# excamera/alfalfa

Hardware: NVIDIA H100
Metric: decode_throughput (higher is better)
Workload: dtype u8

## Files before the change

alfalfa_b200/csrc/capi.cc:

```cpp
#include <cuda_runtime.h>
#include <stdio.h>
#include <stdlib.h>
#include <string.h>
#include <sys/resource.h>
#include <sys/syscall.h>
#include <unistd.h>

#include <algorithm>
#include <atomic>
#include <condition_variable>
#include <deque>
#include <memory>
#include <mutex>
#include <string>
#include <chrono>
#include <thread>
#include <unordered_map>
#include <vector>

#include "../../include/vp8gpu.h"
#include "engine.hpp"
#include "hostpool.h"
#include "parser.h"
#include "serializer.h"

using vp8::Engine;
using vp8::HostJob;
using vp8::ParsedFrame;
using vp8::State;

struct vp8gpu_parsed;
struct vp8gpu_ctx {
  Engine* engine = nullptr;
  std::string create_error;
  std::atomic<int> next_lane{0};
  std::mutex pool_mu;
  std::vector<vp8gpu_parsed*> pinned_pool;
  double stats[8] = {0, 0, 0, 0, 0, 0, 0, 0};
  std::atomic<int> device_tokens{1};
  std::mutex scratch_mu;
  vp8::TokenRing* scratch_ring = nullptr;
  std::vector<struct ivf_worker_kit*> kit_pool;
  std::mutex tok_mu;
  std::condition_variable tok_cv;
  int tok_permits = 0, tok_capacity = 0;
};
struct TokRelease {
  vp8gpu_ctx* ctx;
  int n;
};
static void CUDART_CB tok_release_cb(void* p) {
  TokRelease* r = static_cast<TokRelease*>(p);
  {
    std::lock_guard<std::mutex> lk(r->ctx->tok_mu);
    r->ctx->tok_permits += r->n;
  }
  r->ctx->tok_cv.notify_all();
  delete r;
}
struct vp8gpu_state {
  State s;
  vp8gpu_state(int w, int h) : s(w, h) {}
  explicit vp8gpu_state(const State& o) : s(o) {}
};
struct vp8gpu_parsed {
  ParsedFrame f;
  uint32_t n_intra = 0, n_filtered = 0;
  cudaEvent_t consumed = nullptr;
  bool busy = false;
  explicit vp8gpu_parsed(const vp8::Allocator& a) : f(a) {}
};
constexpr int kTokSlots = 96;
constexpr int kTokChunk = 32;
constexpr int kTokStreams = 4;
struct ivf_worker_kit {
  vp8::TokenRing* ring = nullptr;
  cudaStream_t copy_stream = nullptr;
  cudaStream_t kstream[kTokStreams] = {};
  int next_kstream = 0;
  vp8gpu_parsed* parsed[kTokSlots] = {};
  cudaEvent_t staged[kTokSlots] = {}, ready[kTokSlots] = {}, finished[kTokSlots] = {};
  bool busy[kTokSlots] = {};
};
struct vp8gpu_resident_batch {
  Engine::Resident* r = nullptr;
};

namespace {

constexpr unsigned kWaitableEvent = cudaEventDisableTiming | cudaEventBlockingSync;

void* pinned_alloc(size_t n) {
  void* p = nullptr;
  return cudaHostAlloc(&p, n, cudaHostAllocDefault) == cudaSuccess ? p : nullptr;
}
void pinned_free(void* p) { cudaFreeHost(p); }
const vp8::Allocator kPinned = {&pinned_alloc, &pinned_free};

size_t ring_bytes_for(size_t n) { return n + n / 4 + 4096; }

void count_mbs(vp8gpu_parsed* p) {
  const vp8gpu_frame_desc& d = p->f.desc;
  const size_t n = (size_t)d.mb_cols * d.mb_rows;
  const vp8gpu_mb* m = p->f.mbs.data();
  uint32_t ni = 0, nf = 0;
  for (size_t i = 0; i < n; i++) {
    ni += m[i].ref_frame == VP8GPU_REF_CURRENT;
    nf += m[i].lf_level != 0;
  }
  p->n_intra = ni;
  p->n_filtered = nf;
}

}

extern "C" {

Engine* vp8gpu_ctx_engine(vp8gpu_ctx* ctx) { return ctx->engine; }
int vp8gpu_ctx_next_lane(vp8gpu_ctx* ctx) { return ctx->next_lane.fetch_add(1) % vp8::kMaxLanes; }
const vp8::ParsedFrame* vp8gpu_parsed_frame(const vp8gpu_parsed* p) { return p ? &p->f : nullptr; }

int vp8gpu_ctx_create(int device, int width, int height, int max_frames, vp8gpu_ctx** out) {
  if (!out) return VP8GPU_ERR_LOGIC;
  *out = nullptr;
  setenv("CUDA_DEVICE_MAX_CONNECTIONS", "32", 0);
  vp8gpu_ctx* c = new vp8gpu_ctx();
  const int rc = Engine::create(device, width, height, max_frames, &c->engine, &c->create_error);
  if (rc != VP8GPU_OK) {
    delete c;
    return rc;
  }
  *out = c;
  return VP8GPU_OK;
}
extern "C" void vp8gpu_encoder_pool_purge(Engine* e);
void vp8gpu_ctx_destroy(vp8gpu_ctx* ctx) {
  if (!ctx) return;
  for (vp8gpu_parsed* p : ctx->pinned_pool) vp8gpu_parsed_destroy(p);
  ctx->engine->sync_all();
  if (ctx->scratch_ring) ctx->engine->token_ring_free(ctx->scratch_ring);
  for (ivf_worker_kit* k : ctx->kit_pool) {
    ctx->engine->token_ring_free(k->ring);
    if (k->copy_stream) cudaStreamDestroy(k->copy_stream);
    for (cudaStream_t st : k->kstream)
      if (st) cudaStreamDestroy(st);
    for (int i = 0; i < kTokSlots; i++) {
      if (k->parsed[i]) vp8gpu_parsed_destroy(k->parsed[i]);
      if (k->staged[i]) cudaEventDestroy(k->staged[i]);
      if (k->ready[i]) cudaEventDestroy(k->ready[i]);
    }
    delete k;
  }
  vp8gpu_encoder_pool_purge(ctx->engine);
  delete ctx->engine;
  delete ctx;
}
const char* vp8gpu_last_error(const vp8gpu_ctx* ctx) { return ctx && ctx->engine ? ctx->engine->last_error() : ""; }

int vp8gpu_frame_alloc(vp8gpu_ctx* ctx, vp8gpu_frame_id* out) { return ctx->engine->frame_alloc(out); }
int vp8gpu_frame_retain(vp8gpu_ctx* ctx, vp8gpu_frame_id id) { return ctx->engine->frame_retain(id); }
int vp8gpu_frame_release(vp8gpu_ctx* ctx, vp8gpu_frame_id id) { return ctx->engine->frame_release(id); }
int vp8gpu_frame_upload(vp8gpu_ctx* ctx, vp8gpu_frame_id id, const uint8_t* y, size_t ys, const uint8_t* u,
                        const uint8_t* v, size_t cs) {
  return ctx->engine->frame_upload(id, y, ys, u, v, cs);
}
int vp8gpu_frame_download(vp8gpu_ctx* ctx, vp8gpu_frame_id id, uint8_t* y, size_t ys, uint8_t* u, uint8_t* v,
                          size_t cs) {
  return ctx->engine->frame_download(id, y, ys, u, v, cs);
}
int vp8gpu_frame_download_display(vp8gpu_ctx* ctx, vp8gpu_frame_id id, uint8_t* dst, size_t dst_size) {
  return ctx->engine->frame_download_display(id, 0, dst, dst_size, true);
}
int vp8gpu_frame_download_display_async(vp8gpu_ctx* ctx, vp8gpu_frame_id id, uint8_t* dst, size_t dst_size) {
  return ctx->engine->frame_download_display(id, 0, dst, dst_size, false);
}
int vp8gpu_frame_hash(vp8gpu_ctx* ctx, vp8gpu_frame_id id, uint64_t* out) { return ctx->engine->frame_hash(id, 0, out); }
int vp8gpu_frame_ssim(vp8gpu_ctx* ctx, vp8gpu_frame_id a, vp8gpu_frame_id b, double* out) {
  if (!ctx || !out) return VP8GPU_ERR_LOGIC;
  return ctx->engine->frames_ssim(a, b, 0, out);
}
size_t vp8gpu_frame_bytes(const vp8gpu_ctx* ctx) { return ctx->engine->geom().frame_bytes; }
int vp8gpu_frame_export(vp8gpu_ctx* ctx, vp8gpu_frame_id id, void* dst, size_t bytes) {
  return ctx->engine->frame_copy_raw(id, dst, bytes, false);
}
int vp8gpu_frame_import(vp8gpu_ctx* ctx, vp8gpu_frame_id id, const void* src, size_t bytes) {
  return ctx->engine->frame_copy_raw(id, const_cast<void*>(src), bytes, true);
}
int vp8gpu_ctx_sync(vp8gpu_ctx* ctx) { return ctx->engine->sync_all(); }
int vp8gpu_host_alloc(void** out, size_t bytes) {
  return cudaHostAlloc(out, bytes, cudaHostAllocDefault) == cudaSuccess ? VP8GPU_OK : VP8GPU_ERR_NOMEM;
}
void vp8gpu_host_free(void* p) {
  if (p) cudaFreeHost(p);
}
uint64_t vp8gpu_launch_count(const vp8gpu_ctx* ctx) { return ctx->engine->launches(); }
int vp8gpu_frames_in_use(const vp8gpu_ctx* ctx) { return ctx->engine->frames_in_use(); }
int vp8gpu_serialize_frame_ex(const vp8gpu_encode_header* hdr, const vp8gpu_encode_features* ft, const vp8gpu_mb* mbs,
                              const vp8gpu_token* tokens, const vp8gpu_split_mvs* split, uint8_t* out, size_t cap,
                              size_t* size) {
  if (!hdr || !mbs || !size) return VP8GPU_ERR_LOGIC;
  vp8::EncodeHeader h;
  h.key_frame = hdr->key_frame;
  h.show_frame = hdr->show_frame;
  h.width = hdr->width;
  h.height = hdr->height;
  h.y_ac_qi = hdr->y_ac_qi;
  h.loop_filter_level = hdr->loop_filter_level;
  h.sharpness = hdr->sharpness;
  h.optimize_token_probs = hdr->optimize_token_probs;
  vp8::EncodeFeatures x;
  if (ft) {
    x.log2_partitions = ft->log2_partitions;
    x.segmentation_enabled = ft->segmentation_enabled;
    x.update_mb_segmentation_map = ft->update_mb_segmentation_map;
    x.update_segment_feature_data = ft->update_segment_feature_data;
    x.segment_feature_absolute = ft->segment_feature_absolute;
    for (int i = 0; i < 4; i++) {
      x.segment_quant[i] = ft->segment_quant[i];
      x.segment_lf[i] = ft->segment_lf[i];
      x.ref_lf_delta[i] = ft->ref_lf_delta[i];
      x.mode_lf_delta[i] = ft->mode_lf_delta[i];
    }
    for (int i = 0; i < 3; i++) x.segment_tree_probs[i] = ft->segment_tree_probs[i];
    x.lf_delta_enabled = ft->lf_delta_enabled;
    x.lf_delta_update = ft->lf_delta_update;
    x.y_dc_delta = ft->y_dc_delta;
    x.y2_dc_delta = ft->y2_dc_delta;
    x.y2_ac_delta = ft->y2_ac_delta;
    x.uv_dc_delta = ft->uv_dc_delta;
    x.uv_ac_delta = ft->uv_ac_delta;
    x.refresh_golden = ft->refresh_golden;
    x.refresh_alternate = ft->refresh_alternate;
    x.refresh_last = ft->refresh_last;
    x.refresh_entropy_probs = ft->refresh_entropy_probs;
    x.copy_to_golden = ft->copy_to_golden;
    x.copy_to_alternate = ft->copy_to_alternate;
    x.sign_bias_golden = ft->sign_bias_golden;
    x.sign_bias_alternate = ft->sign_bias_alternate;
    x.saved_coef_probs = ft->saved_coef_probs;
  }
  const std::vector<uint8_t> bytes = vp8::serialize_frame(h, mbs, tokens, split, ft ? &x : nullptr);
  if (bytes.empty()) return VP8GPU_ERR_UNSUPPORTED;
  *size = bytes.size();
  if (!out || cap < bytes.size()) return VP8GPU_ERR_NOMEM;
  memcpy(out, bytes.data(), bytes.size());
  return VP8GPU_OK;
}
int vp8gpu_serialize_frame(const vp8gpu_encode_header* hdr, const vp8gpu_mb* mbs, const vp8gpu_token* tokens,
                           const vp8gpu_split_mvs* split, uint8_t* out, size_t cap, size_t* size) {
  return vp8gpu_serialize_frame_ex(hdr, nullptr, mbs, tokens, split, out, cap, size);
}
void vp8gpu_decode_ivf_stats(const vp8gpu_ctx* ctx, double out[8]) { memcpy(out, ctx->stats, sizeof(ctx->stats)); }

static HostJob to_host_job(const vp8gpu_job& j) {
  HostJob h;
  h.desc = j.desc;
  h.mbs = j.mbs;
  h.tokens = j.tokens;
  h.split = j.split;
  memcpy(h.refs, j.refs, sizeof(h.refs));
  h.out = j.out;
  return h;
}

int vp8gpu_decode_batch(vp8gpu_ctx* ctx, int lane, const vp8gpu_job* jobs, int n) {
  if (!ctx || !jobs || n < 0) return VP8GPU_ERR_LOGIC;
  std::vector<HostJob> hj;
  hj.reserve(n);
  for (int i = 0; i < n; i++) {
    if (!jobs[i].desc || !jobs[i].mbs) return ctx->engine->fail(VP8GPU_ERR_LOGIC, "decode_batch: null records");
    if (jobs[i].desc->mb_cols != ctx->engine->geom().mb_cols || jobs[i].desc->mb_rows != ctx->engine->geom().mb_rows)
      return ctx->engine->fail(VP8GPU_ERR_LOGIC, "decode_batch: frame size does not match the context");
    hj.push_back(to_host_job(jobs[i]));
  }
  const int rc = ctx->engine->submit(lane, hj.data(), n, nullptr);
  if (rc != VP8GPU_OK) return rc;
  cudaError_t e = cudaStreamSynchronize(ctx->engine->stream(lane));
  return e == cudaSuccess ? VP8GPU_OK : ctx->engine->cuda_fail(e, "decode_batch sync");
}

int vp8gpu_decode_parsed(vp8gpu_ctx* ctx, int lane, const vp8gpu_frame_desc* desc, const vp8gpu_mb* mbs,
                         const vp8gpu_token* tokens, const vp8gpu_split_mvs* split, const vp8gpu_frame_id refs[3],
                         vp8gpu_frame_id out) {
  vp8gpu_job j;
  j.desc = desc;
  j.mbs = mbs;
  j.tokens = tokens;
  j.split = split;
  for (int i = 0; i < 3; i++) j.refs[i] = refs ? refs[i] : -1;
  j.out = out;
  return vp8gpu_decode_batch(ctx, lane, &j, 1);
}

int vp8gpu_batch_upload(vp8gpu_ctx* ctx, const vp8gpu_job* jobs, int n, vp8gpu_resident_batch** out) {
  std::vector<HostJob> hj;
  for (int i = 0; i < n; i++) hj.push_back(to_host_job(jobs[i]));
  vp8gpu_resident_batch* b = new vp8gpu_resident_batch();
  const int rc = ctx->engine->resident_upload(hj.data(), n, &b->r);
  if (rc != VP8GPU_OK) {
    delete b;
    return rc;
  }
// ... 502 lines not shown
    j.n_intra = (int)ps[i]->n_intra;
    j.n_filtered = (int)ps[i]->n_filtered;
    j.consumed = ps[i]->consumed;
    jobs.push_back(j);
    which.push_back(i);
  }
  const int rc = e->submit(lane < 0 ? ds[0]->lane : lane, jobs.data(), (int)jobs.size(), nullptr);
  for (size_t k = 0; k < jobs.size(); k++) {
    const int i = which[k];
    if (rc == VP8GPU_OK) {
      ps[i]->busy = true;
      copy_to_references(ds[i], *jobs[k].desc, jobs[k].out);
    } else {
      rcs[i] = rc;
    }
    e->frame_release(jobs[k].out);
  }
  for (int i = 0; i < n; i++)
    if (rcs[i] != VP8GPU_OK) return rcs[i];
  return VP8GPU_OK;
}

int vp8gpu_decoder_decode_parsed(vp8gpu_decoder* d, const vp8gpu_parsed* parsed, int* shown, vp8gpu_frame_id* out) {
  if (!d || !parsed) return VP8GPU_ERR_LOGIC;
  cudaSetDevice(d->ctx->engine->device());
  return decode_parsed_impl(d, const_cast<vp8gpu_parsed*>(parsed), false, shown, out);
}

vp8gpu_state* vp8gpu_decoder_state(vp8gpu_decoder* d) { return &d->state; }
int vp8gpu_decoder_references(const vp8gpu_decoder* d, vp8gpu_frame_id refs[3]) {
  memcpy(refs, d->refs, sizeof(d->refs));
  return VP8GPU_OK;
}
int vp8gpu_decoder_lane(const vp8gpu_decoder* d) { return d->lane; }

int vp8gpu_decoder_hash(vp8gpu_decoder* d, uint64_t* out) {
  if (!d || !out) return VP8GPU_ERR_LOGIC;
  uint64_t h = d->state.s.hash();
  for (int i = 0; i < 3; i++) {
    uint64_t r = 0;
    const int rc = d->ctx->engine->frame_hash(d->refs[i], d->lane, &r);
    if (rc != VP8GPU_OK) return rc;
    h = (h ^ r) * 0x9E3779B97F4A7C15ull + (h >> 29) + i;
  }
  *out = h;
  return VP8GPU_OK;
}

int vp8gpu_decoder_equal(vp8gpu_decoder* a, vp8gpu_decoder* b, int* equal) {
  if (!a || !b || !equal || a->ctx != b->ctx) return VP8GPU_ERR_LOGIC;
  *equal = 0;
  if (!(a->state.s == b->state.s)) return VP8GPU_OK;
  for (int i = 0; i < 3; i++) {
    int eq = 0;
    const int rc = a->ctx->engine->frames_equal(a->refs[i], b->refs[i], a->lane, &eq);
    if (rc != VP8GPU_OK) return rc;
    if (!eq) return VP8GPU_OK;
  }
  *equal = 1;
  return VP8GPU_OK;
}

struct CachedFirstPartition {
  vp8gpu_frame_desc desc;
  std::vector<vp8gpu_mb> mbs;
  std::vector<vp8gpu_split_mvs> split;
  vp8::TokenWork tw;
  size_t bits_delta = 0;
};
std::mutex g_parse_cache_mu;
std::unordered_map<uint64_t, std::shared_ptr<CachedFirstPartition>> g_parse_cache;
uint64_t frame_key(const uint8_t* p, size_t n) {
  uint64_t h = 1469598103934665603ull ^ n;
  auto mix = [&](const uint8_t* q, size_t k) {
    for (size_t i = 0; i < k; i++) h = (h ^ q[i]) * 1099511628211ull;
  };
  mix(p, n < 64 ? n : 64);
  if (n > 64) mix(p + n - 64, 64);
  return h;
}
int parse_first_partition_cached(vp8::State& state, const uint8_t* data, size_t len, vp8::ParsedFrame& out) {
  const uint64_t key = frame_key(data, len);
  std::shared_ptr<CachedFirstPartition> c;
  {
    std::lock_guard<std::mutex> lk(g_parse_cache_mu);
    auto it = g_parse_cache.find(key);
    if (it != g_parse_cache.end()) c = it->second;
  }
  if (!c) {
    const int rc = vp8::parse_frame(state, data, len, out, true);
    if (rc != VP8GPU_OK) return rc;
    c = std::make_shared<CachedFirstPartition>();
    c->desc = out.desc;
    const size_t n = (size_t)out.desc.mb_cols * out.desc.mb_rows;
    c->mbs.assign(out.mbs.data(), out.mbs.data() + n);
    c->split.assign(out.split.data(), out.split.data() + out.desc.n_split);
    c->tw = out.tw;
    c->bits_delta = (size_t)(out.tw.bits - data);
    std::lock_guard<std::mutex> lk(g_parse_cache_mu);
    g_parse_cache[key] = c;
    return VP8GPU_OK;
  }
  out.desc = c->desc;
  if (!out.mbs.reserve(c->mbs.size(), 0) || !out.split.reserve(c->split.size() + 1, 0)) return VP8GPU_ERR_NOMEM;
  memcpy(out.mbs.data(), c->mbs.data(), c->mbs.size() * sizeof(vp8gpu_mb));
  if (!c->split.empty()) memcpy(out.split.data(), c->split.data(), c->split.size() * sizeof(vp8gpu_split_mvs));
  out.tw = c->tw;
  out.tw.bits = data + c->bits_delta;
  return VP8GPU_OK;
}

struct IvfKnobs {
  int tok_slots = -1;
  int tok_chunk = -1;
  int tok_inflight = -1;
  int tok_arena = -1;
  int dispatchers = -1;
  int worker_nice = -1;
  bool trace = false;
  bool parse_cache = false;
  static int num(const char* name) {
    const char* v = getenv(name);
    return v ? atoi(v) : -1;
  }
  IvfKnobs()
      : tok_slots(num("VP8GPU_TOK_SLOTS")), tok_chunk(num("VP8GPU_TOK_CHUNK")), tok_inflight(num("VP8GPU_TOK_INFLIGHT")),
        tok_arena(num("VP8GPU_TOK_ARENA")), dispatchers(num("VP8GPU_DISPATCHERS")), worker_nice(num("VP8GPU_WORKER_NICE")),
        trace(getenv("VP8GPU_TRACE") != nullptr), parse_cache(getenv("VP8GPU_PARSE_CACHE") != nullptr) {}
};

class IvfDecode {
 public:
  IvfDecode(vp8gpu_ctx* ctx_, const uint8_t* ivf_, size_t len_, int threads_, uint8_t* dst_, size_t dst_size_)
      : ctx(ctx_), e(ctx_->engine), ivf(ivf_), len(len_), threads(threads_), dst(dst_), dst_size(dst_size_) {}
  int parse_container();
  void plan();
  int run(uint32_t* n_decoded, uint32_t* n_shown);

 private:
  struct Item {
    const uint8_t* p;
    uint32_t n;
    int64_t out_off;
  };
  static constexpr int kSlots = 4;
  enum SlotState { kFree = 0, kQueued = 1 };
  struct Pending {
    vp8gpu_parsed* slot;
    int refs[3];
    int out;
    int64_t out_off;
    int* slot_state;
    int tid = 0;
    const vp8::TokenRing* ring = nullptr;
    int ring_slot = 0;
    cudaEvent_t ready = nullptr;
    cudaEvent_t* finished = nullptr;
  };

  vp8gpu_ctx* const ctx;
  Engine* const e;
  const IvfKnobs knobs;
  const uint8_t* const ivf;
  const size_t len;
  int threads;
  uint8_t* const dst;
  const size_t dst_size;
  int w = 0, h = 0;
  std::vector<Item> items;
  std::vector<uint32_t> gop_start;
  uint32_t shown_total = 0, max_frame_bytes = 0;
  int n_gops = 0;
  int tok_slots = 0, tok_chunk = 1, n_disp = 1, worker_nice = 5;
  size_t arena_tokens = 0;
  bool device_tokens = false;
  std::mutex mu;
  std::vector<std::condition_variable> cv_worker, cv_disp;
  std::vector<std::deque<Pending>> queues;
  std::vector<int> running;
  std::atomic<int> next_gop{0};
  std::atomic<int> first_error{VP8GPU_OK};
  std::mutex stats_mu;
  double st_parse = 0, st_wait_slot = 0, st_wait_dma = 0, st_submit = 0, st_download = 0, st_disp_idle = 0;
  double st_batches = 0, st_jobs = 0;

  void set_error(int rc) {
    int ok = VP8GPU_OK;
    first_error.compare_exchange_strong(ok, rc);
  }
  static double now() { return std::chrono::duration<double>(std::chrono::steady_clock::now().time_since_epoch()).count(); }
  static void advance_refs(Engine* e, int refs[3], const vp8gpu_frame_desc& desc, int out) {
    if (desc.key_frame) {
      set_ref(e, &refs[0], out);
      set_ref(e, &refs[1], out);
      set_ref(e, &refs[2], out);
    } else {
      if (desc.copy_to_alternate == 1) set_ref(e, &refs[2], refs[0]);
      else if (desc.copy_to_alternate == 2) set_ref(e, &refs[2], refs[1]);
      if (desc.copy_to_golden == 1) set_ref(e, &refs[1], refs[0]);
      else if (desc.copy_to_golden == 2) set_ref(e, &refs[1], refs[2]);
      if (desc.refresh_golden) set_ref(e, &refs[1], out);
      if (desc.refresh_alternate) set_ref(e, &refs[2], out);
      if (desc.refresh_last) set_ref(e, &refs[0], out);
    }
  }
  void worker_host(int tid);
  ivf_worker_kit* acquire_kit();
  void worker_device(int tid);
  void dispatcher(int di);
};

int IvfDecode::parse_container() {
  if (len < 32 || memcmp(ivf, "DKIF", 4) != 0) return e->fail(VP8GPU_ERR_INVALID, "missing IVF file header");
  if ((ivf[4] | (ivf[5] << 8)) != 0) return e->fail(VP8GPU_ERR_UNSUPPORTED, "not an IVF version 0 file");
  if ((ivf[6] | (ivf[7] << 8)) != 32) return e->fail(VP8GPU_ERR_UNSUPPORTED, "unsupported IVF header length");
  if (memcmp(ivf + 8, "VP80", 4) != 0) return e->fail(VP8GPU_ERR_UNSUPPORTED, "not a VP8 file");
  w = ivf[12] | (ivf[13] << 8), h = ivf[14] | (ivf[15] << 8);
  if (w != e->width() || h != e->height()) return e->fail(VP8GPU_ERR_UNSUPPORTED, "IVF size does not match the context");
  const uint32_t count = ivf[24] | (ivf[25] << 8) | (ivf[26] << 16) | ((uint32_t)ivf[27] << 24);
  const size_t frame_bytes = (size_t)w * h + 2 * (size_t)((w + 1) / 2) * ((h + 1) / 2);
  size_t pos = 32, out_off = 0;
  for (uint32_t i = 0; i < count; i++) {
    if (pos + 12 > len) return e->fail(VP8GPU_ERR_INVALID, "IVF file truncated");
    const uint32_t n = ivf[pos] | (ivf[pos + 1] << 8) | (ivf[pos + 2] << 16) | ((uint32_t)ivf[pos + 3] << 24);
    if (pos + 12 + n > len) return e->fail(VP8GPU_ERR_INVALID, "IVF file truncated");
    const uint8_t* p = ivf + pos + 12;
    pos += 12 + n;
    const bool key = n > 0 && !(p[0] & 1);
    if (items.empty() && !key) continue;
    if (key) gop_start.push_back((uint32_t)items.size());
    const bool shown = n > 0 && ((p[0] >> 4) & 1);
    Item it = {p, n, shown ? (int64_t)out_off : -1};
    if (shown) {
      out_off += frame_bytes;
      shown_total++;
    }
    items.push_back(it);
  }
  if (dst && dst_size < out_off) return e->fail(VP8GPU_ERR_LOGIC, "decode_ivf: destination too small");
  gop_start.push_back((uint32_t)items.size());
  n_gops = (int)gop_start.size() - 1;
  for (const Item& it : items) max_frame_bytes = it.n > max_frame_bytes ? it.n : max_frame_bytes;
  return VP8GPU_OK;
}

void IvfDecode::plan() {
  if (threads < 1) threads = 1;
  if (threads > 512) threads = 512;
  if (threads > n_gops) threads = n_gops > 0 ? n_gops : 1;
  if (ctx->device_tokens.load()) {
    tok_slots = e->frames_free() / threads - 4;
    size_t free_mem = 0, total_mem = (size_t)80 << 30;
    if (cudaSetDevice(e->device()) != cudaSuccess || cudaMemGetInfo(&free_mem, &total_mem) != cudaSuccess) total_mem = (size_t)80 << 30;
    const size_t ring_budget = total_mem / 2;
    const size_t worst = e->token_cap_for(max_frame_bytes), worst_bytes = worst * sizeof(vp8gpu_token);
    const size_t stride = e->token_ring_layout(ring_bytes_for(max_frame_bytes), true).stride;
    const size_t per_worker = ring_budget / (size_t)threads;
    int want = per_worker > 2 * worst_bytes ? (int)std::min<size_t>((per_worker - 2 * worst_bytes) / (stride + worst_bytes / 2), kTokSlots) : 0;
    if (knobs.tok_slots >= 0) want = knobs.tok_slots;
    if (want > kTokSlots) want = kTokSlots;
    if (tok_slots > want) tok_slots = want;
    if (tok_slots < 4) tok_slots = 0;
    if (tok_slots > 0) {
      const size_t room = per_worker > (size_t)tok_slots * stride ? (per_worker - (size_t)tok_slots * stride) / sizeof(vp8gpu_token) : 0;
      arena_tokens = std::max(std::min(room, (size_t)tok_slots * worst), (size_t)(tok_slots / 2 + 2) * worst);
      if (knobs.tok_arena >= 0) arena_tokens = std::max((size_t)knobs.tok_arena * worst, (size_t)(tok_slots / 2 + 2) * worst);
    }
  }
  device_tokens = tok_slots > 0;
  if (!device_tokens) {
    const int fit = e->frames_free() / 8;
    if (threads > fit) threads = fit > 0 ? fit : 1;
  }
  if (device_tokens) {
    int sms = 132;
    cudaDeviceGetAttribute(&sms, cudaDevAttrMultiProcessorCount, e->device());
    int cap = 0;
    (void)sms;
    if (knobs.tok_inflight >= 0) cap = knobs.tok_inflight;
    std::lock_guard<std::mutex> lk(ctx->tok_mu);
    ctx->tok_capacity = cap;
    ctx->tok_permits = cap;
  }
  tok_chunk = tok_slots / 3 > kTokChunk ? kTokChunk : (tok_slots / 3 > 0 ? tok_slots / 3 : 1);
  if (knobs.tok_chunk >= 0) {
    const int c = knobs.tok_chunk;
    if (c >= 1 && c <= tok_slots / 2) tok_chunk = c;
  }
  n_disp = device_tokens ? (threads >= 32 ? 4 : (threads >= 8 ? 2 : 1)) : 1;
  if (knobs.dispatchers >= 0) {
    const int n = knobs.dispatchers;
    if (n >= 1 && n <= 16 && n <= threads) n_disp = n;
  }
  if (knobs.worker_nice >= 0) worker_nice = knobs.worker_nice;
  cv_worker = std::vector<std::condition_variable>(threads);
  cv_disp = std::vector<std::condition_variable>(n_disp);
  queues.assign(threads, {});
  running.assign(n_disp, 0);
  for (int t = 0; t < threads; t++) running[t % n_disp]++;
}

void IvfDecode::worker_host(int tid) {
  cudaSetDevice(e->device());
  double t_parse = 0, t_slot = 0, t_dma = 0;
  State state(w, h);
  int refs[3] = {-1, -1, -1};
  vp8gpu_parsed* slots[kSlots] = {};
  int slot_state[kSlots] = {};
  int next_slot = 0;
  int rc = VP8GPU_OK;
  for (;;) {
    const int g = next_gop.fetch_add(1);
    if (g >= n_gops || first_error.load() != VP8GPU_OK) break;
    for (uint32_t i = gop_start[g]; i < gop_start[g + 1] && rc == VP8GPU_OK; i++) {
      const int si = next_slot;
      next_slot = (next_slot + 1) % kSlots;
      if (!slots[si]) {
        {
          std::lock_guard<std::mutex> lk(ctx->pool_mu);
          if (!ctx->pinned_pool.empty()) {
            slots[si] = ctx->pinned_pool.back();
            ctx->pinned_pool.pop_back();
          }
        }
        if (!slots[si]) {
          slots[si] = new vp8gpu_parsed(kPinned);
          cudaEventCreateWithFlags(&slots[si]->consumed, kWaitableEvent);
          const size_t n_mbs = (size_t)e->geom().mb_cols * e->geom().mb_rows;
          slots[si]->f.mbs.reserve(n_mbs, 0);
          slots[si]->f.tokens.reserve(n_mbs * 32 + 1024, 0);
          slots[si]->f.split.reserve(256, 0);
        }
      }
      vp8gpu_parsed* p = slots[si];
      const double t0 = now();
      {
        std::unique_lock<std::mutex> lk(mu);
        cv_worker[tid].wait(lk, [&] { return slot_state[si] == kFree; });
      }
      const double t1 = now();
      if (p->busy) {
        cudaEventSynchronize(p->consumed);
        p->busy = false;
      }
      const double t2 = now();
      rc = vp8::parse_frame(state, items[i].p, items[i].n, p->f);
      if (rc != VP8GPU_OK) break;
      count_mbs(p);
      t_slot += t1 - t0;
      t_dma += t2 - t1;
      t_parse += now() - t2;
      const vp8gpu_frame_desc& desc = p->f.desc;
      Pending job;
      job.slot = p;
      job.slot_state = &slot_state[si];
      job.out_off = (dst && desc.show_frame) ? items[i].out_off : -1;
      rc = e->frame_alloc(&job.out);
      if (rc != VP8GPU_OK) break;
      for (int k = 0; k < 3; k++) {
        job.refs[k] = desc.key_frame ? -1 : refs[k];
        if (job.refs[k] >= 0) e->frame_retain(job.refs[k]);
      }
      advance_refs(e, refs, desc, job.out);
      {
        std::lock_guard<std::mutex> lk(mu);
        slot_state[si] = kQueued;
        job.tid = tid;
        queues[tid].push_back(job);
      }
      cv_disp[tid % n_disp].notify_one();
    }
    if (rc != VP8GPU_OK) {
      set_error(rc);
      break;
    }
  }
  {
    std::unique_lock<std::mutex> lk(mu);
    cv_worker[tid].wait(lk, [&] {
      for (int k = 0; k < kSlots; k++)
        if (slot_state[k] != kFree) return false;
      return true;
    });
    running[tid % n_disp]--;
  }
  cv_disp[tid % n_disp].notify_one();
  {
    std::lock_guard<std::mutex> lk(stats_mu);
    st_parse += t_parse;
    st_wait_slot += t_slot;
    st_wait_dma += t_dma;
  }
  for (int k = 0; k < 3; k++)
    if (refs[k] >= 0) e->frame_release(refs[k]);
  for (auto* p : slots)
    if (p) {
      if (p->busy) {
        cudaEventSynchronize(p->consumed);
        p->busy = false;
      }
      std::lock_guard<std::mutex> lk(ctx->pool_mu);
      ctx->pinned_pool.push_back(p);
    }
}

ivf_worker_kit* IvfDecode::acquire_kit() {
  ivf_worker_kit* k = nullptr;
  {
    std::lock_guard<std::mutex> lk(ctx->pool_mu);
    for (size_t i = 0; i < ctx->kit_pool.size(); i++)
      if (ctx->kit_pool[i]->ring->bits_cap >= max_frame_bytes + 16 && ctx->kit_pool[i]->ring->nslots >= tok_slots &&
          ctx->kit_pool[i]->ring->arena_cap >= arena_tokens) {
        k = ctx->kit_pool[i];
        ctx->kit_pool.erase(ctx->kit_pool.begin() + i);
        break;
      }
  }
  if (k) return k;
  k = new ivf_worker_kit();
  bool ok = e->token_ring_create(tok_slots, ring_bytes_for(max_frame_bytes), &k->ring, arena_tokens) == VP8GPU_OK &&
            cudaStreamCreateWithFlags(&k->copy_stream, cudaStreamNonBlocking) == cudaSuccess;
  for (cudaStream_t& st : k->kstream) ok = ok && cudaStreamCreateWithFlags(&st, cudaStreamNonBlocking) == cudaSuccess;
  if (!ok) {
    if (k->ring) e->token_ring_free(k->ring);
    if (k->copy_stream) cudaStreamDestroy(k->copy_stream);
    for (cudaStream_t st : k->kstream)
      if (st) cudaStreamDestroy(st);
    delete k;
    return nullptr;
  }
  const size_t n_mbs = (size_t)e->geom().mb_cols * e->geom().mb_rows;
  for (int i = 0; i < tok_slots; i++) {
    k->parsed[i] = new vp8gpu_parsed(kPinned);
    k->parsed[i]->f.mbs.reserve(n_mbs, 0);
    k->parsed[i]->f.split.reserve(256, 0);
    cudaEventCreateWithFlags(&k->staged[i], cudaEventDisableTiming);
    cudaEventCreateWithFlags(&k->ready[i], cudaEventDisableTiming);
  }
  return k;
}

void IvfDecode::worker_device(int tid) {
  if (worker_nice > 0) setpriority(PRIO_PROCESS, (id_t)syscall(SYS_gettid), worker_nice);
  cudaSetDevice(e->device());
  double t_parse = 0, t_slot = 0, t_dma = 0;
  State state(w, h);
  int refs[3] = {-1, -1, -1};
  int slot_state[kTokSlots] = {};
  int next_slot = 0;
  int launches_done = 0;
  int rc = VP8GPU_OK;
  ivf_worker_kit* kit = acquire_kit();
  if (!kit) rc = e->fail(VP8GPU_ERR_NOMEM, "decode_ivf: token ring allocation failed");
  std::deque<int> live;
  size_t head = 0, a_start[kTokSlots] = {};
  bool held[kTokSlots] = {};
  long n_takes = 0, n_wraps = 0, n_waits = 0;
  struct ChunkTrace {
    cudaEvent_t ev[3];
    int frames;
  };
  std::vector<ChunkTrace> chunk_trace;
  auto arena_take = [&](int si, size_t need, auto in_chunk, vp8gpu_token** out) {
    const size_t cap = arena_tokens;
    if (held[si]) {
      live.erase(std::find(live.begin(), live.end(), si));
      held[si] = false;
    }
    for (;;) {
      size_t at = SIZE_MAX;
      if (live.empty()) {
        at = need <= cap ? 0 : SIZE_MAX;
      } else {
        const size_t tail = a_start[live.front()];
        if (head > tail) {
          if (cap - head >= need) at = head;
          else if (tail >= need) at = 0;
        } else if (tail - head >= need) {
          at = head;
        }
      }
      if (at != SIZE_MAX) {
        n_takes++;
        if (at == 0 && head > 0) n_wraps++;
        a_start[si] = at;
        head = at + need;
        held[si] = true;
        live.push_back(si);
        *out = kit->ring->arena + at;
        return VP8GPU_OK;
      }
      if (live.empty() || in_chunk(live.front())) return e->fail(VP8GPU_ERR_LOGIC, "decode_ivf: token arena too small");
      const int s = live.front();
      n_waits++;
      {
        std::unique_lock<std::mutex> lk(mu);
        cv_worker[tid].wait(lk, [&] { return slot_state[s] == kFree; });
      }
      if (kit->busy[s]) {
        if (kit->finished[s]) cudaEventSynchronize(kit->finished[s]);
        kit->busy[s] = false;
      }
      live.pop_front();
      held[s] = false;
    }
  };
  while (rc == VP8GPU_OK) {
    const int g = next_gop.fetch_add(1);
    if (g >= n_gops || first_error.load() != VP8GPU_OK) break;
    uint32_t i = gop_start[g];
    while (i < gop_start[g + 1] && rc == VP8GPU_OK) {
      const uint32_t left = gop_start[g + 1] - i;
      int want = tok_chunk;
      if (launches_done < 3 && (2 << launches_done) < want) want = 2 << launches_done;
      launches_done++;
      const int n = (int)left < want ? (int)left : want;
      const int first_slot = next_slot;
      int staged = 0, permits_taken = 0;
      for (int c = 0; c < n && rc == VP8GPU_OK; c++) {
        const int si = (first_slot + c) % tok_slots;
        const double t0 = now();
        {
          std::unique_lock<std::mutex> lk(mu);
          cv_worker[tid].wait(lk, [&] { return slot_state[si] == kFree; });
        }
        const double t1 = now();
        if (kit->busy[si]) {
          if (kit->finished[si]) cudaEventSynchronize(kit->finished[si]);
          kit->busy[si] = false;
        }
        const double t2 = now();
        vp8gpu_parsed* p = kit->parsed[si];
        rc = knobs.parse_cache ? parse_first_partition_cached(state, items[i + c].p, items[i + c].n, p->f)
                               : vp8::parse_frame(state, items[i + c].p, items[i + c].n, p->f, true);
        if (rc != VP8GPU_OK) break;
        count_mbs(p);
        vp8gpu_token* tokens = nullptr;
        rc = arena_take(si, e->token_cap_for(p->f.tw.bits_len), [&](int s) {
          return (s - first_slot + tok_slots) % tok_slots < c;
        }, &tokens);
        if (rc != VP8GPU_OK) break;
        rc = e->token_ring_stage(kit->ring, si, p->f, kit->copy_stream, tokens);
        if (rc != VP8GPU_OK) break;
        staged++;
        t_slot += t1 - t0;
        t_dma += t2 - t1;
        t_parse += now() - t2;
      }
      if (rc != VP8GPU_OK) break;
      cudaStream_t ks = kit->kstream[kit->next_kstream];
      kit->next_kstream = (kit->next_kstream + 1) % kTokStreams;
      cudaEventRecord(kit->staged[first_slot], kit->copy_stream);
      cudaStreamWaitEvent(ks, kit->staged[first_slot], 0);
      ChunkTrace ctr{{nullptr, nullptr, nullptr}, staged};
      if (knobs.trace) {
        for (cudaEvent_t& ev : ctr.ev) cudaEventCreate(&ev);
        cudaEventRecord(ctr.ev[0], kit->copy_stream);
        cudaEventRecord(ctr.ev[1], ks);
      }
      if (ctx->tok_capacity > 0) {
        std::unique_lock<std::mutex> lk(ctx->tok_mu);
        const int need = staged < ctx->tok_capacity ? staged : ctx->tok_capacity;
        ctx->tok_cv.wait(lk, [&] { return ctx->tok_permits >= need; });
        ctx->tok_permits -= need;
        permits_taken = need;
      }
      const int until_wrap = tok_slots - first_slot;
      rc = e->token_ring_launch(kit->ring, first_slot, staged < until_wrap ? staged : until_wrap, ks);
      if (rc == VP8GPU_OK && staged > until_wrap) rc = e->token_ring_launch(kit->ring, 0, staged - until_wrap, ks);
      if (rc == VP8GPU_OK)
        cudaEventRecord(kit->ready[first_slot], ks);
      if (knobs.trace) {
        cudaEventRecord(ctr.ev[2], ks);
        chunk_trace.push_back(ctr);
      }
      if (permits_taken && cudaLaunchHostFunc(ks, tok_release_cb, new TokRelease{ctx, permits_taken}) != cudaSuccess) {
        std::lock_guard<std::mutex> lk(ctx->tok_mu);
        ctx->tok_permits += permits_taken;
      }
      if (rc != VP8GPU_OK) break;
      for (int c = 0; c < staged && rc == VP8GPU_OK; c++) {
        const int si = (first_slot + c) % tok_slots;
        vp8gpu_parsed* p = kit->parsed[si];
        const vp8gpu_frame_desc& desc = p->f.desc;
        Pending job;
        job.slot = p;
        job.slot_state = &slot_state[si];
        job.out_off = (dst && desc.show_frame) ? items[i + c].out_off : -1;
        job.ring = kit->ring;
        job.ring_slot = si;
        job.ready = kit->ready[first_slot];
        job.finished = &kit->finished[si];
        rc = e->frame_alloc(&job.out);
        if (rc != VP8GPU_OK) break;
        for (int k = 0; k < 3; k++) {
          job.refs[k] = desc.key_frame ? -1 : refs[k];
          if (job.refs[k] >= 0) e->frame_retain(job.refs[k]);
        }
        advance_refs(e, refs, desc, job.out);
        kit->busy[si] = true;
        {
          std::lock_guard<std::mutex> lk(mu);
          slot_state[si] = kQueued;
          job.tid = tid;
        queues[tid].push_back(job);
        }
        cv_disp[tid % n_disp].notify_one();
      }
      next_slot = (first_slot + staged) % tok_slots;
      i += (uint32_t)staged;
    }
    if (rc != VP8GPU_OK) break;
  }
  if (rc != VP8GPU_OK) set_error(rc);
  {
    std::unique_lock<std::mutex> lk(mu);
    cv_worker[tid].wait(lk, [&] {
      for (int k = 0; k < kTokSlots; k++)
        if (slot_state[k] != kFree) return false;
      return true;
    });
    running[tid % n_disp]--;
  }
  cv_disp[tid % n_disp].notify_one();
  {
    std::lock_guard<std::mutex> lk(stats_mu);
    st_parse += t_parse;
    st_wait_slot += t_slot;
    st_wait_dma += t_dma;
  }
  for (int k = 0; k < 3; k++)
    if (refs[k] >= 0) e->frame_release(refs[k]);
  if (kit) {
    for (int k = 0; k < kTokSlots; k++)
      if (kit->busy[k]) {
        if (kit->finished[k]) cudaEventSynchronize(kit->finished[k]);
        kit->busy[k] = false;
      }
    cudaStreamSynchronize(kit->copy_stream);
    for (cudaStream_t st : kit->kstream) cudaStreamSynchronize(st);
    uint32_t res[kTokSlots][2];
    if (cudaMemcpy2D(res, 8, kit->ring->dev + kit->ring->result_off, kit->ring->stride, 8, (size_t)kit->ring->nslots,
                     cudaMemcpyDeviceToHost) == cudaSuccess) {
      bool cleared = false;
      for (int k = 0; k < kit->ring->nslots && k < tok_slots; k++)
        if (res[k][1]) {
          set_error(e->fail(VP8GPU_ERR_LOGIC, "device token pool overflow"));
          cleared = e->token_ring_clear_result(kit->ring, k, kit->copy_stream) == VP8GPU_OK || cleared;
        }
      if (cleared) cudaStreamSynchronize(kit->copy_stream);
    }
    if (knobs.trace) {
      fprintf(stderr, "decode_ivf arena: worker %d takes %ld wraps %ld waits %ld cap %zu slots %d chunk %d\n", tid, n_takes, n_wraps,
              n_waits, arena_tokens, tok_slots, tok_chunk);
      std::vector<float> lat, kern;
      long frames = 0;
      for (ChunkTrace& c : chunk_trace) {
        float ms = 0;
        if (cudaEventElapsedTime(&ms, c.ev[0], c.ev[2]) == cudaSuccess) lat.push_back(ms);
        if (cudaEventElapsedTime(&ms, c.ev[1], c.ev[2]) == cudaSuccess) kern.push_back(ms);
        frames += c.frames;
        for (cudaEvent_t ev : c.ev) cudaEventDestroy(ev);
      }
      auto pct = [](std::vector<float>& v, double q) {
        if (v.empty()) return 0.0;
        std::sort(v.begin(), v.end());
        return (double)v[std::min(v.size() - 1, (size_t)(q * (v.size() - 1) + 0.5))];
      };
      fprintf(stderr, "[trace] worker %d chunks: %zu (%ld frames); staged -> ready ms p10 %.2f p50 %.2f p90 %.2f max %.2f; "
              "k_tokens start -> ready ms p50 %.2f p90 %.2f max %.2f\n", tid, chunk_trace.size(), frames, pct(lat, 0.1), pct(lat, 0.5),
              pct(lat, 0.9), pct(lat, 1.0), pct(kern, 0.5), pct(kern, 0.9), pct(kern, 1.0));
    }
    std::lock_guard<std::mutex> lk(ctx->pool_mu);
    ctx->kit_pool.push_back(kit);
  }
}

void IvfDecode::dispatcher(int di) {
  cudaSetDevice(e->device());
  std::vector<Pending> batch;
  std::vector<HostJob> hj;
  std::vector<int> dl_ids;
  std::vector<uint8_t*> dl_dst;
  int round = 0;
  double t_idle = 0, t_submit = 0, t_download = 0, n_batches = 0, n_jobs = 0;
  struct Trace {
    cudaEvent_t a, b;
    int lane, n;
    double host_t;
    cudaEvent_t mid[4] = {nullptr, nullptr, nullptr, nullptr};
  };
  std::vector<Trace> trace;
  const bool tracing = knobs.trace;
  for (;;) {
    batch.clear();
    const double ti = now();
    {
      std::unique_lock<std::mutex> lk(mu);
      auto eligible = [&](std::deque<Pending>& q) {
        if (q.empty()) return false;
        Pending& f = q.front();
        if (!f.ready) return true;
        if (cudaEventQuery(f.ready) != cudaSuccess) return false;
        const cudaEvent_t fired = f.ready;
        for (Pending& p : q) {
          if (p.ready != fired) break;
          p.ready = nullptr;
        }
        return true;
      };
      auto ready = [&] {
        int n = 0;
        for (int t = di; t < threads; t += n_disp) n += eligible(queues[t]);
        return n;
      };
      auto queued = [&] {
        for (int t = di; t < threads; t += n_disp)
          if (!queues[t].empty()) return true;
        return false;
      };
      while (!(running[di] == 0 && !queued()) && ready() == 0) {
        if (queued()) cv_disp[di].wait_for(lk, std::chrono::microseconds(100));
        else cv_disp[di].wait(lk);
      }
      const auto deadline = std::chrono::steady_clock::now() + std::chrono::microseconds(1500);
      while (running[di] > 0 && ready() < (running[di] * 3 + 3) / 4) {
        if (device_tokens) {
          if (std::chrono::steady_clock::now() >= deadline) break;
          cv_disp[di].wait_for(lk, std::chrono::microseconds(100));
        } else if (cv_disp[di].wait_until(lk, deadline) == std::cv_status::timeout) {
          break;
        }
      }
      for (int t = di; t < threads; t += n_disp)
        if (eligible(queues[t])) {
          batch.push_back(queues[t].front());
          queues[t].pop_front();
        }
      if (batch.empty() && running[di] == 0 && !queued()) break;
    }
    if (batch.empty()) continue;
    const double ts = now();
    t_idle += ts - ti;
    n_batches += 1;
    n_jobs += batch.size();
    const int lane = 2 * di + (round++ & 1);
    hj.clear();
    for (const Pending& b : batch) {
      HostJob j;
      j.desc = &b.slot->f.desc;
      j.mbs = b.slot->f.mbs.data();
      j.tokens = b.slot->f.tokens.data();
      j.split = b.slot->f.split.data();
      memcpy(j.refs, b.refs, sizeof(j.refs));
      j.out = b.out;
      j.n_intra = (int)b.slot->n_intra;
      j.n_filtered = (int)b.slot->n_filtered;
      j.consumed = b.slot->consumed;
      if (b.ring) {
        j.ring = b.ring;
        j.ring_slot = b.ring_slot;
        j.ready = nullptr;
        j.finished = b.finished;
        j.consumed = nullptr;
      }
      hj.push_back(j);
    }
    Trace tr{nullptr, nullptr, lane, (int)batch.size(), ts};
    if (tracing) {
      e->ensure_lane(lane);
      cudaEventCreate(&tr.a);
      cudaEventCreate(&tr.b);
      for (cudaEvent_t& m : tr.mid) cudaEventCreate(&m);
      cudaEventRecord(tr.a, e->stream(lane));
    }
    int rc = e->submit(lane, hj.data(), (int)hj.size(), nullptr, tracing ? tr.mid + 1 : nullptr);
    if (tracing) {
      cudaEventRecord(tr.b, e->stream(lane));
      trace.push_back(tr);
    }
    const double td = now();
    t_submit += td - ts;
    if (rc == VP8GPU_OK) {
      dl_ids.clear();
      dl_dst.clear();
      for (const Pending& b : batch) {
        if (!b.ring) b.slot->busy = true;
        if (b.out_off >= 0) {
          dl_ids.push_back(b.out);
          dl_dst.push_back(dst + b.out_off);
        }
      }
      if (!dl_ids.empty()) rc = e->frames_download_display(dl_ids.data(), dl_dst.data(), (int)dl_ids.size(), lane);
    }
    for (const Pending& b : batch) {
      for (int k = 0; k < 3; k++)
        if (b.refs[k] >= 0) e->frame_release(b.refs[k]);
      e->frame_release(b.out);
    }
    if (rc != VP8GPU_OK) set_error(rc);
    t_download += now() - td;
    {
      std::lock_guard<std::mutex> lk(mu);
      for (const Pending& b : batch) *b.slot_state = kFree;
    }
    for (const Pending& b : batch) cv_worker[b.tid].notify_one();
  }
  e->sync_lane(2 * di);
  e->sync_lane(2 * di + 1);
  if (tracing && !trace.empty()) {
    double sum_ms = 0, sum_gap = 0, first_host = trace.front().host_t, last_host = trace.back().host_t;
    double sum_intra = 0, sum_lf = 0, sum_inter = 0, sum_pre = 0, sum_turn = 0;
    float ms = 0;
    for (size_t i = 0; i < trace.size(); i++) {
      if (cudaEventElapsedTime(&ms, trace[i].mid[3], trace[i].mid[1]) == cudaSuccess) sum_inter += ms;
      if (cudaEventElapsedTime(&ms, trace[i].a, trace[i].mid[3]) == cudaSuccess) sum_pre += ms;
      if (cudaEventElapsedTime(&ms, trace[i].mid[1], trace[i].mid[2]) == cudaSuccess) sum_intra += ms;
      if (cudaEventElapsedTime(&ms, trace[i].mid[2], trace[i].b) == cudaSuccess) sum_lf += ms;
      cudaEventElapsedTime(&ms, trace[i].a, trace[i].b);
      sum_ms += ms;
      if (i) {
        cudaEventElapsedTime(&ms, trace[i - 1].b, trace[i].b);
        sum_gap += ms;
        if (cudaEventElapsedTime(&ms, trace[i - 1].b, trace[i].mid[3]) == cudaSuccess) sum_turn += ms;
      }
    }
    fprintf(stderr, "[trace] dispatcher %d: %zu batches, avg %.2f frames, device %.3f ms per batch, end-to-end period %.3f ms, "
            "host span %.1f ms; per batch: waits + upload %.3f ms, k_inter %.3f ms, k_intra %.3f ms, k_loopfilter %.3f ms, turn-around %.3f ms\n", di,
            trace.size(), n_jobs / n_batches, sum_ms / trace.size(), trace.size() > 1 ? sum_gap / (trace.size() - 1) : 0.0,
            (last_host - first_host) * 1e3, sum_pre / trace.size(), sum_inter / trace.size(), sum_intra / trace.size(),
            sum_lf / trace.size(), trace.size() > 1 ? sum_turn / (trace.size() - 1) : 0.0);
    for (Trace& t : trace) {
      cudaEventDestroy(t.a);
      cudaEventDestroy(t.b);
      for (cudaEvent_t m : t.mid)
        if (m) cudaEventDestroy(m);
    }
  }
  std::lock_guard<std::mutex> lk(stats_mu);
  st_disp_idle += t_idle;
  st_submit += t_submit;
  st_download += t_download;
  st_batches += n_batches;
  st_jobs += n_jobs;
}

int IvfDecode::run(uint32_t* n_decoded, uint32_t* n_shown) {
  std::vector<std::thread> pool;
  for (int t = 0; t < threads; t++) {
    if (device_tokens) pool.emplace_back(&IvfDecode::worker_device, this, t);
    else pool.emplace_back(&IvfDecode::worker_host, this, t);
  }
  std::vector<std::thread> dispatchers;
  for (int d = 1; d < n_disp; d++) dispatchers.emplace_back(&IvfDecode::dispatcher, this, d);
  dispatcher(0);
  for (auto& t : dispatchers) t.join();
  for (auto& t : pool) t.join();
  ctx->stats[0] = st_parse;
  ctx->stats[1] = st_wait_slot;
  ctx->stats[2] = st_wait_dma;
  ctx->stats[3] = st_submit;
  ctx->stats[4] = st_download;
  ctx->stats[5] = st_disp_idle;
  ctx->stats[6] = st_batches;
  ctx->stats[7] = st_jobs;
  if (n_decoded) *n_decoded = (uint32_t)items.size();
  if (n_shown) *n_shown = shown_total;
  return first_error.load();
}

int vp8gpu_decode_ivf(vp8gpu_ctx* ctx, const uint8_t* ivf, size_t len, int threads, uint8_t* dst, size_t dst_size,
                      uint32_t* n_decoded, uint32_t* n_shown) {
  if (!ctx || !ivf) return VP8GPU_ERR_LOGIC;
  IvfDecode job(ctx, ivf, len, threads, dst, dst_size);
  const int rc = job.parse_container();
  if (rc != VP8GPU_OK) return rc;
  job.plan();
  return job.run(n_decoded, n_shown);
}

}
```

alfalfa_b200/csrc/engine.cu:

```cuda
#include "engine.hpp"

#include <cuda.h>
#include <stdlib.h>
#include <string.h>

namespace vp8 {

int launch_compare(const uint8_t* a, const uint8_t* b, const Geom& g, int* d_flag, void* stream);
int launch_hash(const uint8_t* a, const Geom& g, unsigned long long* d_out, void* stream);

namespace {
inline size_t align_up(size_t v, size_t a) { return (v + a - 1) / a * a; }

std::mutex g_tmap_mu;
struct TmapChunk {
  uint8_t* base;
  size_t used, cap;
};
std::vector<TmapChunk> g_tmap_chunks[64];
uint8_t* tmap_arena_alloc(int device, size_t bytes) {
  std::lock_guard<std::mutex> lk(g_tmap_mu);
  if (device < 0 || device >= 64) return nullptr;
  auto& chunks = g_tmap_chunks[device];
  if (chunks.empty() || chunks.back().used + bytes > chunks.back().cap) {
// ... 362 lines not shown
    if (!cmp_scratch_) CU(cudaMalloc(&cmp_scratch_, 1024));
    flag = reinterpret_cast<int*>(cmp_scratch_ + 640 + 4 * lane);
    if (int rc = wait_for(frames_[a], lane, s, false)) return rc;
    if (int rc = wait_for(frames_[b], lane, s, false)) return rc;
    CU(cudaMemsetAsync(flag, 0, sizeof(int), s));
    if (int e = launch_compare(frames_[a].dev, frames_[b].dev, g_, flag, s)) return cuda_fail((cudaError_t)e, "compare");
    launches_++;
    if (int rc = touch(frames_[a], lane, false)) return rc;
    if (int rc = touch(frames_[b], lane, false)) return rc;
  }
  int h = 0;
  CU(cudaMemcpyAsync(&h, flag, sizeof(int), cudaMemcpyDeviceToHost, s));
  CU(cudaStreamSynchronize(s));
  *equal = h == 0;
  return VP8GPU_OK;
}

int Engine::frames_ssim(int a, int b, int lane, double* out) {
  if (int rc = ensure_lane(lane)) return rc;
  cudaStream_t s = lanes_[lane];
  const int n = (g_.W / 4 - 1) * (g_.H / 4 - 1);
  if (n <= 0) {
    *out = 0.0;
    return VP8GPU_OK;
  }
  {
    std::lock_guard<std::mutex> lk(mu_);
    for (int id : {a, b})
      if (id < 0 || id >= (int)frames_.size() || frames_[id].refcnt <= 0) return fail(VP8GPU_ERR_LOGIC, "ssim: bad frame id");
    if (!ssim_dev_[lane]) {
      CU(cudaSetDevice(device_));
      CU(cudaMalloc(&ssim_dev_[lane], (size_t)n * sizeof(float)));
      CU(cudaHostAlloc(&ssim_host_[lane], (size_t)n * sizeof(float), cudaHostAllocDefault));
    }
    if (int rc = wait_for(frames_[a], lane, s, false)) return rc;
    if (int rc = wait_for(frames_[b], lane, s, false)) return rc;
    if (int e = launch_ssim(frames_[a].dev, frames_[b].dev, g_, ssim_dev_[lane], s)) return cuda_fail((cudaError_t)e, "ssim");
    launches_++;
    if (int rc = touch(frames_[a], lane, false)) return rc;
    if (int rc = touch(frames_[b], lane, false)) return rc;
  }
  CU(cudaMemcpyAsync(ssim_host_[lane], ssim_dev_[lane], (size_t)n * sizeof(float), cudaMemcpyDeviceToHost, s));
  CU(cudaStreamSynchronize(s));
  float total = 0.0f;
  const float* v = ssim_host_[lane];
  for (int i = 0; i < n; i++) total += v[i];
  *out = total / n;
  return VP8GPU_OK;
}

int Engine::frame_hash(int id, int lane, uint64_t* out) {
  if (int rc = ensure_lane(lane)) return rc;
  unsigned long long* d;
  cudaStream_t s = lanes_[lane];
  {
    std::lock_guard<std::mutex> lk(mu_);
    if (id < 0 || id >= (int)frames_.size() || frames_[id].refcnt <= 0) return fail(VP8GPU_ERR_LOGIC, "hash: bad frame id");
    if (!cmp_scratch_) CU(cudaMalloc(&cmp_scratch_, 1024));
    d = reinterpret_cast<unsigned long long*>(cmp_scratch_ + 64 + 8 * lane);
    if (int rc = wait_for(frames_[id], lane, s, false)) return rc;
    CU(cudaMemsetAsync(d, 0, sizeof(unsigned long long), s));
    if (int e = launch_hash(frames_[id].dev, g_, d, s)) return cuda_fail((cudaError_t)e, "hash");
    launches_++;
    if (int rc = touch(frames_[id], lane, false)) return rc;
  }
  unsigned long long h = 0;
  CU(cudaMemcpyAsync(&h, d, sizeof(h), cudaMemcpyDeviceToHost, s));
  CU(cudaStreamSynchronize(s));
  *out = h;
  return VP8GPU_OK;
}

int Engine::count_jobs(const HostJob& j, uint32_t* n_intra, uint32_t* n_inter, uint32_t* n_filtered) const {
  const size_t n = (size_t)g_.mb_cols * g_.mb_rows;
  uint32_t ni = 0, nf = 0;
  if (j.n_intra >= 0 && j.n_filtered >= 0) {
    ni = (uint32_t)j.n_intra;
    nf = (uint32_t)j.n_filtered;
  } else {
    for (size_t i = 0; i < n; i++) {
      ni += j.mbs[i].ref_frame == VP8GPU_REF_CURRENT;
      nf += j.mbs[i].lf_level != 0;
    }
  }
  *n_intra = ni;
  *n_inter = (uint32_t)n - ni;
  *n_filtered = j.desc->loop_filter_level ? nf : 0;
  return VP8GPU_OK;
}

namespace {
struct Layout {
  size_t jobs_off, sync_off, sync_bytes, total;
  std::vector<size_t> mbs_off, tok_off, split_off;
};
Layout plan(const Geom& g, const HostJob* jobs, int n) {
  Layout L;
  L.jobs_off = 0;
  L.sync_off = align_up(sizeof(DevJob) * n, 256);
  L.sync_bytes = sizeof(int) * (kSyncHeaderInts + (size_t)n * 2 * g.mb_rows);
  size_t off = align_up(L.sync_off + L.sync_bytes, 256);
  const size_t n_mbs = (size_t)g.mb_cols * g.mb_rows;
  for (int i = 0; i < n; i++) {
    if (jobs[i].ring) {
      L.mbs_off.push_back(0);
      L.tok_off.push_back(0);
      L.split_off.push_back(0);
      continue;
    }
    L.mbs_off.push_back(off);
    off = align_up(off + n_mbs * sizeof(vp8gpu_mb), 256);
    L.tok_off.push_back(off);
    off = align_up(off + (size_t)jobs[i].desc->n_tokens * sizeof(vp8gpu_token) + 4, 256);
    L.split_off.push_back(off);
    off = align_up(off + (size_t)jobs[i].desc->n_split * sizeof(vp8gpu_split_mvs) + 4, 256);
  }
  L.total = off;
  return L;
}
}

int Engine::build_and_launch(int lane, const DevJob* d_jobs, int* d_sync, int n, bool any_inter, bool any_intra,
                             bool any_lf, cudaEvent_t* between) {
  cudaStream_t s = lanes_[lane];
  if (between) CU(cudaEventRecord(between[2], s));
  if (any_inter) {
    if (int e = launch_inter(d_jobs, n, g_, s)) return cuda_fail((cudaError_t)e, "k_inter launch");
    launches_++;
  }
  if (between) CU(cudaEventRecord(between[0], s));
  if (any_intra) {
    if (int e = launch_intra(d_jobs, n, g_, d_sync + 0, next_epoch(1), s)) return cuda_fail((cudaError_t)e, "k_intra launch");
    launches_++;
  }
  if (between) CU(cudaEventRecord(between[1], s));
  if (any_lf) {
    if (int e = launch_loopfilter(d_jobs, n, g_, d_sync + 32, next_epoch(2), lf_band(), s)) return cuda_fail((cudaError_t)e, "k_loopfilter launch");
    launches_++;
  }
  return VP8GPU_OK;
}

uint32_t Engine::token_cap_for(size_t bits) const {
  const size_t by_bytes = align_up(bits + 16, 256) * 9 + 1024, by_blocks = (size_t)g_.mb_cols * g_.mb_rows * 400;
  return (uint32_t)(by_bytes < by_blocks ? by_bytes : by_blocks);
}

TokenRing Engine::token_ring_layout(size_t max_frame_bytes, bool arena) const {
  const size_t n_mbs = (size_t)g_.mb_cols * g_.mb_rows;
  TokenRing r;
  r.bits_cap = (uint32_t)align_up(max_frame_bytes + 16, 256);
  r.split_cap = (uint32_t)n_mbs;
  r.tok_cap = token_cap_for(max_frame_bytes);
  size_t off = 256;
  r.probs_off = off;
  off += 1280;
  r.info_off = off;
  off = align_up(off + 4 * ((n_mbs + 15) / 16 + 1), 256);
  r.bits_off = off;
  off = align_up(off + r.bits_cap, 256);
  r.host_stride = off;
  r.result_off = off;
  off += 256;
  r.above_off = off;
  off = align_up(off + 2 * (size_t)g_.mb_cols, 256);
  r.mbs_off = off;
  off = align_up(off + n_mbs * sizeof(vp8gpu_mb), 256);
  r.split_off = off;
  off = align_up(off + (size_t)r.split_cap * sizeof(vp8gpu_split_mvs), 256);
  r.tok_off = off;
  if (!arena) off = align_up(off + (size_t)r.tok_cap * sizeof(vp8gpu_token), 256);
  r.stride = off;
  return r;
}

int Engine::token_ring_create(int nslots, size_t max_frame_bytes, TokenRing** out, size_t arena_tokens) {
  CU(cudaSetDevice(device_));
  TokenRing* r = new TokenRing(token_ring_layout(max_frame_bytes, arena_tokens > 0));
  r->nslots = nslots;
  r->slot_tokens.assign(nslots, nullptr);
  r->arena_cap = arena_tokens;
  if (cudaMalloc(&r->dev, r->stride * nslots) != cudaSuccess ||
      (arena_tokens && cudaMalloc(&r->arena, arena_tokens * sizeof(vp8gpu_token)) != cudaSuccess) ||
      cudaHostAlloc(&r->host, r->host_stride * nslots, cudaHostAllocDefault) != cudaSuccess) {
    token_ring_free(r);
    return fail(VP8GPU_ERR_NOMEM, "token ring allocation failed");
  }
  CU(cudaMemset2D(r->dev + r->result_off, r->stride, 0, 8, (size_t)nslots));
  *out = r;
  return VP8GPU_OK;
}

void Engine::token_ring_free(TokenRing* r) {
  if (!r) return;
  cudaSetDevice(device_);
  if (r->dev) cudaFree(r->dev);
  if (r->arena) cudaFree(r->arena);
  if (r->host) cudaFreeHost(r->host);
  delete r;
}

int Engine::token_ring_stage(TokenRing* r, int slot, const ParsedFrame& f, cudaStream_t s, vp8gpu_token* tokens) {
  const TokenWork& tw = f.tw;
  if (!tw.deferred) return fail(VP8GPU_ERR_LOGIC, "token_ring_stage: frame was not parsed with defer_tokens");
  if (tw.bits_len > r->bits_cap || f.desc.n_split > r->split_cap)
    return fail(VP8GPU_ERR_NOMEM, "token_ring_stage: frame larger than the ring was sized for");
  if ((r->arena != nullptr) != (tokens != nullptr)) return fail(VP8GPU_ERR_LOGIC, "token_ring_stage: token area");
  uint8_t* h = r->host_slot(slot);
  uint8_t* d = r->dev_slot(slot);
  TokJob* j = reinterpret_cast<TokJob*>(h);
  j->mbs = reinterpret_cast<vp8gpu_mb*>(d + r->mbs_off);
  j->tokens = tokens ? tokens : reinterpret_cast<vp8gpu_token*>(d + r->tok_off);
  r->slot_tokens[slot] = j->tokens;
  j->bits = d + r->bits_off;
  j->coef_probs = d + r->probs_off;
  j->result = reinterpret_cast<uint32_t*>(d + r->result_off);
  j->above = reinterpret_cast<uint16_t*>(d + r->above_off);
  j->mbinfo = reinterpret_cast<const uint32_t*>(d + r->info_off);
  memcpy(j->part_off, tw.part_off, sizeof(j->part_off));
  memcpy(j->part_len, tw.part_len, sizeof(j->part_len));
  j->nparts = tw.nparts;
  j->tok_cap = tokens ? token_cap_for(tw.bits_len) : r->tok_cap;
  memcpy(h + r->probs_off, tw.coef_probs, 1056);
  memcpy(h + r->bits_off, tw.bits, tw.bits_len);
  const size_t n_mbs = (size_t)g_.mb_cols * g_.mb_rows;
  {
    uint32_t* info = reinterpret_cast<uint32_t*>(h + r->info_off);
    const vp8gpu_mb* m = f.mbs.data();
    for (size_t w = 0; w < (n_mbs + 15) / 16; w++) {
      uint32_t v = 0;
      const size_t n = n_mbs - 16 * w < 16 ? n_mbs - 16 * w : 16;
      for (size_t k = 0; k < n; k++) v |= (uint32_t)(m[16 * w + k].flags & 3u) << (2 * k);
      info[w] = v;
    }
  }
  CU(cudaMemcpyAsync(d, h, r->bits_off + align_up(tw.bits_len, 16), cudaMemcpyHostToDevice, s));
  CU(cudaMemcpyAsync(d + r->mbs_off, f.mbs.data(), n_mbs * sizeof(vp8gpu_mb), cudaMemcpyHostToDevice, s));
  if (f.desc.n_split)
    CU(cudaMemcpyAsync(d + r->split_off, f.split.data(), (size_t)f.desc.n_split * sizeof(vp8gpu_split_mvs),
                       cudaMemcpyHostToDevice, s));
  return VP8GPU_OK;
}

int Engine::token_ring_launch(TokenRing* r, int first, int count, cudaStream_t s) {
  if (count <= 0) return VP8GPU_OK;
  if (int e = launch_tokens(r->dev, r->stride, first, count, r->nslots, g_, s)) return cuda_fail((cudaError_t)e, "k_tokens launch");
  launches_++;
  return VP8GPU_OK;
}

int Engine::token_ring_clear_result(TokenRing* r, int slot, cudaStream_t s) {
  CU(cudaMemsetAsync(r->dev_slot(slot) + r->result_off, 0, 8, s));
  return VP8GPU_OK;
}

int Engine::token_ring_result(TokenRing* r, int slot, cudaStream_t s, uint32_t result[2]) {
  CU(cudaMemcpyAsync(result, r->dev_slot(slot) + r->result_off, 8, cudaMemcpyDeviceToHost, s));
  CU(cudaStreamSynchronize(s));
  return VP8GPU_OK;
}

int Engine::submit(int lane, const HostJob* jobs, int n, cudaEvent_t consumed, cudaEvent_t* between) {
  if (n <= 0) return VP8GPU_OK;
  if (int rc = ensure_lane(lane)) return rc;
  CU(cudaSetDevice(device_));
  cudaStream_t s = lanes_[lane];
  const Layout L = plan(g_, jobs, n);
  Staging& st = staging_[lane][staging_next_[lane]];
  staging_next_[lane] = (staging_next_[lane] + 1) % kStagingDepth;
  if (st.in_flight) {
    CU(cudaEventSynchronize(st.done));
    st.in_flight = false;
  }
  if (!st.done) CU(cudaEventCreateWithFlags(&st.done, cudaEventDisableTiming | cudaEventBlockingSync));
  const size_t hdr_bytes = align_up(L.sync_off + L.sync_bytes, 256);
  if (st.host_cap < hdr_bytes) {
    if (st.host) CU(cudaFreeHost(st.host));
    st.host_cap = hdr_bytes * 2;
    CU(cudaHostAlloc(&st.host, st.host_cap, cudaHostAllocMapped));
    CU(cudaHostGetDevicePointer(reinterpret_cast<void**>(&st.host_dev), st.host, 0));
  }
  if (st.dev_cap < L.total) {
    if (st.dev) CU(cudaFree(st.dev));
    st.dev_cap = L.total + L.total / 2;
    CU(cudaMalloc(&st.dev, st.dev_cap));
  }
  memset(st.host, 0, hdr_bytes);
  DevJob* hj = reinterpret_cast<DevJob*>(st.host);
  int* d_sync = reinterpret_cast<int*>(st.dev + L.sync_off);
  bool any_inter = false, any_intra = false, any_lf = false;
  std::vector<cudaEvent_t> waits;
  {
    std::lock_guard<std::mutex> lk(mu_);
    for (int i = 0; i < n; i++) {
      const HostJob& j = jobs[i];
      if (j.out < 0 || j.out >= (int)frames_.size() || frames_[j.out].refcnt <= 0)
        return fail(VP8GPU_ERR_LOGIC, "submit: bad output frame");
      DevJob& d = hj[i];
      if (j.ring) {
        const uint8_t* slot = j.ring->dev_slot(j.ring_slot);
        d.mbs = reinterpret_cast<const vp8gpu_mb*>(slot + j.ring->mbs_off);
        d.tokens = j.ring->slot_tokens[j.ring_slot];
        d.split = reinterpret_cast<const vp8gpu_split_mvs*>(slot + j.ring->split_off);
      } else {
        d.mbs = reinterpret_cast<const vp8gpu_mb*>(st.dev + L.mbs_off[i]);
        d.tokens = reinterpret_cast<const vp8gpu_token*>(st.dev + L.tok_off[i]);
        d.split = reinterpret_cast<const vp8gpu_split_mvs*>(st.dev + L.split_off[i]);
      }
      d.out = frames_[j.out].dev;
      for (int r = 0; r < 3; r++) {
        d.ref[r] = nullptr;
        d.ref_tmap[r] = nullptr;
        if (!j.desc->key_frame) {
          if (j.refs[r] < 0 || j.refs[r] >= (int)frames_.size() || frames_[j.refs[r]].refcnt <= 0)
            return fail(VP8GPU_ERR_LOGIC, "submit: bad reference frame");
          d.ref[r] = frames_[j.refs[r]].dev;
          d.ref_tmap[r] = frame_tmaps(j.refs[r]);
        }
      }
      d.intra_progress = d_sync + kSyncHeaderInts + (size_t)(2 * i) * g_.mb_rows;
      d.lf_progress = d_sync + kSyncHeaderInts + (size_t)(2 * i + 1) * g_.mb_rows;
      memcpy(d.quant, j.desc->quant, sizeof(d.quant));
      d.key_frame = j.desc->key_frame;
      d.sharpness = j.desc->sharpness;
      uint32_t n_filtered;
      count_jobs(j, &d.n_intra, &d.n_inter, &n_filtered);
      d.lf_enabled = n_filtered != 0;
      any_inter |= d.n_inter != 0;
      any_intra |= d.n_intra != 0;
      any_lf |= d.lf_enabled != 0;
    }
    for (int i = 0; i < n; i++) {
      collect_waits(frames_[jobs[i].out], lane, true, waits);
      if (!jobs[i].desc->key_frame)
        for (int r = 0; r < 3; r++) collect_waits(frames_[jobs[i].refs[r]], lane, false, waits);
    }
  }
  for (cudaEvent_t ev : waits) CU(cudaStreamWaitEvent(s, ev, 0));
  if (int ce = launch_fetch_header(st.dev, st.host_dev, hdr_bytes, s)) return cuda_fail((cudaError_t)ce, "header fetch");
  launches_++;
  const size_t n_mbs = (size_t)g_.mb_cols * g_.mb_rows;
  for (int i = 0; i < n; i++) {
    const HostJob& j = jobs[i];
    if (j.ring) {
      if (j.ready) CU(cudaStreamWaitEvent(s, j.ready, 0));
      continue;
    }
    CU(cudaMemcpyAsync(st.dev + L.mbs_off[i], j.mbs, n_mbs * sizeof(vp8gpu_mb), cudaMemcpyHostToDevice, s));
    if (j.desc->n_tokens)
      CU(cudaMemcpyAsync(st.dev + L.tok_off[i], j.tokens, (size_t)j.desc->n_tokens * sizeof(vp8gpu_token),
                         cudaMemcpyHostToDevice, s));
    if (j.desc->n_split)
      CU(cudaMemcpyAsync(st.dev + L.split_off[i], j.split, (size_t)j.desc->n_split * sizeof(vp8gpu_split_mvs),
                         cudaMemcpyHostToDevice, s));
    if (j.consumed) CU(cudaEventRecord(j.consumed, s));
  }
  if (consumed) CU(cudaEventRecord(consumed, s));
  if (int rc = build_and_launch(lane, reinterpret_cast<const DevJob*>(st.dev), d_sync, n, any_inter, any_intra, any_lf, between))
    return rc;
  {
    std::lock_guard<std::mutex> lk(mu_);
    cudaEvent_t ev = next_event(lane);
    if (!ev) return fail(VP8GPU_ERR_CUDA, "event creation failed");
    CU(cudaEventRecord(ev, s));
    for (int i = 0; i < n; i++) {
      touch(frames_[jobs[i].out], lane, true, ev);
      if (!jobs[i].desc->key_frame)
        for (int r = 0; r < 3; r++) touch(frames_[jobs[i].refs[r]], lane, false, ev);
      if (jobs[i].finished) *jobs[i].finished = ev;
    }
  }
  CU(cudaEventRecord(st.done, s));
  st.in_flight = true;
  return VP8GPU_OK;
}

struct Engine::Resident {
  uint8_t* dev = nullptr;
  size_t sync_off = 0, sync_bytes = 0;
  int n = 0;
  bool any_inter = false, any_intra = false, any_lf = false;
  std::vector<int> outs, refs;
  cudaEvent_t t0 = nullptr, t1 = nullptr;
};

int Engine::resident_upload(const HostJob* jobs, int n, Resident** out) {
  if (n <= 0) return fail(VP8GPU_ERR_LOGIC, "empty batch");
  if (int rc = ensure_lane(0)) return rc;
  CU(cudaSetDevice(device_));
  const Layout L = plan(g_, jobs, n);
  Resident* r = new Resident();
  r->n = n;
  r->sync_off = L.sync_off;
  r->sync_bytes = L.sync_bytes;
  cudaError_t e = cudaMalloc(&r->dev, L.total);
  if (e != cudaSuccess) {
    delete r;
    return cuda_fail(e, "cudaMalloc(resident batch)");
  }
  std::vector<uint8_t> hdr(align_up(L.sync_off + L.sync_bytes, 256), 0);
  DevJob* hj = reinterpret_cast<DevJob*>(hdr.data());
  int* d_sync = reinterpret_cast<int*>(r->dev + L.sync_off);
  {
    std::lock_guard<std::mutex> lk(mu_);
    for (int i = 0; i < n; i++) {
      const HostJob& j = jobs[i];
      DevJob& d = hj[i];
      d.mbs = reinterpret_cast<const vp8gpu_mb*>(r->dev + L.mbs_off[i]);
      d.tokens = reinterpret_cast<const vp8gpu_token*>(r->dev + L.tok_off[i]);
      d.split = reinterpret_cast<const vp8gpu_split_mvs*>(r->dev + L.split_off[i]);
      if (j.out < 0 || j.out >= (int)frames_.size() || frames_[j.out].refcnt <= 0) {
        cudaFree(r->dev);
        delete r;
        return fail(VP8GPU_ERR_LOGIC, "resident: bad output frame");
      }
      d.out = frames_[j.out].dev;
      r->outs.push_back(j.out);
      for (int k = 0; k < 3; k++) {
        d.ref[k] = nullptr;
        d.ref_tmap[k] = nullptr;
        if (!j.desc->key_frame) {
          if (j.refs[k] < 0 || j.refs[k] >= (int)frames_.size() || frames_[j.refs[k]].refcnt <= 0) {
            cudaFree(r->dev);
            delete r;
            return fail(VP8GPU_ERR_LOGIC, "resident: bad reference frame");
          }
          d.ref[k] = frames_[j.refs[k]].dev;
          d.ref_tmap[k] = frame_tmaps(j.refs[k]);
          r->refs.push_back(j.refs[k]);
        }
      }
      d.intra_progress = d_sync + kSyncHeaderInts + (size_t)(2 * i) * g_.mb_rows;
      d.lf_progress = d_sync + kSyncHeaderInts + (size_t)(2 * i + 1) * g_.mb_rows;
      memcpy(d.quant, j.desc->quant, sizeof(d.quant));
      d.key_frame = j.desc->key_frame;
      d.sharpness = j.desc->sharpness;
      uint32_t n_filtered;
      count_jobs(j, &d.n_intra, &d.n_inter, &n_filtered);
      d.lf_enabled = n_filtered != 0;
      r->any_inter |= d.n_inter != 0;
      r->any_intra |= d.n_intra != 0;
      r->any_lf |= d.lf_enabled != 0;
    }
  }
  const size_t n_mbs = (size_t)g_.mb_cols * g_.mb_rows;
  CU(cudaMemcpy(r->dev, hdr.data(), hdr.size(), cudaMemcpyHostToDevice));
  for (int i = 0; i < n; i++) {
    CU(cudaMemcpy(r->dev + L.mbs_off[i], jobs[i].mbs, n_mbs * sizeof(vp8gpu_mb), cudaMemcpyHostToDevice));
    if (jobs[i].desc->n_tokens)
      CU(cudaMemcpy(r->dev + L.tok_off[i], jobs[i].tokens, (size_t)jobs[i].desc->n_tokens * 4, cudaMemcpyHostToDevice));
    if (jobs[i].desc->n_split)
      CU(cudaMemcpy(r->dev + L.split_off[i], jobs[i].split, (size_t)jobs[i].desc->n_split * 64, cudaMemcpyHostToDevice));
  }
  CU(cudaEventCreate(&r->t0));
  CU(cudaEventCreate(&r->t1));
  *out = r;
  return VP8GPU_OK;
}

int Engine::resident_run(int lane, Resident* r, float* ms) {
  if (int rc = ensure_lane(lane)) return rc;
  CU(cudaSetDevice(device_));
  cudaStream_t s = lanes_[lane];
  {
    std::lock_guard<std::mutex> lk(mu_);
    for (int id : r->outs) {
      if (int rc = wait_for(frames_[id], lane, s)) return rc;
    }
    for (int id : r->refs)
      if (int rc = wait_for(frames_[id], lane, s)) return rc;
  }
  CU(cudaMemsetAsync(r->dev + r->sync_off, 0, r->sync_bytes, s));
  if (ms) CU(cudaEventRecord(r->t0, s));
  if (int rc = build_and_launch(lane, reinterpret_cast<const DevJob*>(r->dev), reinterpret_cast<int*>(r->dev + r->sync_off),
                                r->n, r->any_inter, r->any_intra, r->any_lf))
    return rc;
  if (ms) CU(cudaEventRecord(r->t1, s));
  {
    std::lock_guard<std::mutex> lk(mu_);
    cudaEvent_t ev = next_event(lane);
    if (!ev) return fail(VP8GPU_ERR_CUDA, "event creation failed");
    CU(cudaEventRecord(ev, s));
    for (int id : r->refs) touch(frames_[id], lane, false, ev);
    for (int id : r->outs) touch(frames_[id], lane, true, ev);
  }
  if (ms) {
    CU(cudaEventSynchronize(r->t1));
    CU(cudaEventElapsedTime(ms, r->t0, r->t1));
  }
  return VP8GPU_OK;
}

int Engine::resident_run_many(int lane, Resident* const* rs, int n, float* total_ms) {
  if (n <= 0) return VP8GPU_OK;
  if (int rc = ensure_lane(lane)) return rc;
  cudaStream_t s = lanes_[lane];
  if (total_ms) CU(cudaEventRecord(rs[0]->t0, s));
  for (int i = 0; i < n; i++)
    if (int rc = resident_run(lane, rs[i], nullptr)) return rc;
  if (total_ms) {
// ... 84 lines not shown
```

alfalfa_b200/csrc/engine.h:

```cpp
#pragma once
#include <stdint.h>

#include "../../include/vp8gpu.h"

#ifdef VP8GPU_SIMT_EMUL
#define VP8_LAUNCH(kern, grid, block, smem, stream) ::simt::make_launch((grid), (block), (smem), [](auto... a_) { kern(a_...); })
#else
#define VP8_LAUNCH(kern, grid, block, smem, stream) kern<<<(grid), (block), (smem), (stream)>>>
#endif

namespace vp8 {

struct Geom {
  int mb_cols, mb_rows;
  int W, H;
  int y_pitch, c_pitch;
  uint32_t u_off, v_off;
  uint32_t frame_bytes;
  uint32_t msg_lf_off, msg_intra_off;
  uint32_t alloc_bytes;
};

struct DevJob {
  const vp8gpu_mb* mbs;
  const vp8gpu_token* tokens;
  const vp8gpu_split_mvs* split;
  uint8_t* out;
  const uint8_t* ref[3];
  const void* ref_tmap[3];
  int* intra_progress;
  int* lf_progress;
  vp8gpu_quant quant[4];
  uint8_t key_frame, sharpness, lf_enabled;
  uint8_t lf_force;
  uint32_t n_intra;
  uint32_t n_inter;
  uint32_t pad2;
};

struct EncTables;
struct TrellisTables;
struct EncJob {
  const uint8_t* src;
  const uint8_t* ref;
  uint8_t* out;
  vp8gpu_mb* mbs;
  vp8gpu_token* tokens;
  uint32_t* tok_counter;
  uint32_t tok_cap;
  int* progress;
  const EncTables* tab;
  vp8gpu_quant q;
  uint32_t rate_mult, dist_mult;
  uint16_t cols, rows;
  uint8_t sub;
  uint8_t key_frame, lf_level;
  uint8_t sad_per_bit;
  uint8_t realtime;
  uint8_t mv_costs_zero;
  uint8_t mv_sad_zero;
  uint8_t pad[1];
  const TrellisTables* trellis;
  const uint8_t* y2_prev;
};

struct ReencJob {
  const uint8_t* target;
  uint8_t* recon;
  const vp8gpu_mb* mbs_in;
  vp8gpu_mb* mbs_out;
  vp8gpu_token* tokens;
  uint32_t* tok_counter;
  uint32_t tok_cap;
  int* progress;
  vp8gpu_quant q;
  uint16_t cols, rows;
};

struct TokJob {
  vp8gpu_mb* mbs;
  vp8gpu_token* tokens;
  const uint8_t* bits;
  const uint8_t* coef_probs;
  uint32_t* result;
  uint16_t* above;
  const uint32_t* mbinfo;
  uint32_t part_off[8], part_len[8];
  uint32_t nparts;
  uint32_t tok_cap;
};

int launch_inter(const DevJob* jobs, int njobs, const Geom& g, void* stream);
int launch_enc_rd_trellis(const EncJob* job, int rows, const Geom& g, int* ticket, void* stream);
int launch_reenc_inter(const ReencJob* jobs, int njobs, int n_mbs, const Geom& g, void* stream);
int launch_reenc_intra(const ReencJob* jobs, int njobs, int rows, const Geom& g, int* ticket, void* stream);
int launch_intra(const DevJob* jobs, int njobs, const Geom& g, int* ticket, uint32_t epoch, void* stream);
int launch_loopfilter(const DevJob* jobs, int njobs, const Geom& g, int* ticket, uint32_t epoch, bool band, void* stream);
int launch_tokens(const uint8_t* ring, size_t stride, int first, int count, int nslots, const Geom& g, void* stream);
int launch_fetch_header(void* dst, const void* src_host_devptr, size_t bytes, void* stream);
int launch_ssim(const uint8_t* a, const uint8_t* b, const Geom& g, float* d_windows, void* stream);
int launch_enc_rd(const EncJob* jobs, int njobs, int rows, const Geom& g, int* ticket, void* stream);

}
```

alfalfa_b200/csrc/engine.hpp:

```cpp
#pragma once
#include <cuda_runtime.h>
#include <stdint.h>

#include <atomic>
#include <mutex>
#include <string>
#include <vector>

#include "engine.h"
#include "parser.h"

namespace vp8 {

constexpr int kMaxLanes = 32;
constexpr int kStagingDepth = 3;

struct TokenRing {
  int nslots = 0;
  uint8_t* dev = nullptr;
  uint8_t* host = nullptr;
  size_t stride = 0, host_stride = 0;
  size_t probs_off = 0, info_off = 0, bits_off = 0, result_off = 0, above_off = 0, mbs_off = 0, split_off = 0, tok_off = 0;
  uint32_t bits_cap = 0, split_cap = 0, tok_cap = 0;
  vp8gpu_token* arena = nullptr;
  size_t arena_cap = 0;
  std::vector<vp8gpu_token*> slot_tokens;
  uint8_t* dev_slot(int i) const { return dev + (size_t)i * stride; }
  uint8_t* host_slot(int i) const { return host + (size_t)i * host_stride; }
};

struct HostJob {
  const vp8gpu_frame_desc* desc;
  const vp8gpu_mb* mbs;
  const vp8gpu_token* tokens;
  const vp8gpu_split_mvs* split;
  int refs[3];
  int out;
  int n_intra = -1;
  int n_filtered = -1;
  cudaEvent_t consumed = nullptr;
  const TokenRing* ring = nullptr;
  int ring_slot = 0;
  cudaEvent_t ready = nullptr;
  cudaEvent_t* finished = nullptr;
};

class Engine {
 public:
  static int create(int device, int width, int height, int max_frames, Engine** out, std::string* err);
  ~Engine();

  const Geom& geom() const { return g_; }
  int width() const { return width_; }
  int height() const { return height_; }
  int device() const { return device_; }

  int frame_alloc(int* id);
  int frame_retain(int id);
  int frame_release(int id);
  int frames_free();
  int frames_in_use() {
    std::lock_guard<std::mutex> lk(mu_);
    int n = 0;
    for (const Frame& f : frames_) n += f.refcnt > 0;
    return n;
  }
  uint32_t next_epoch(int kernel_bit = 3) {
    if (!(ll_mask_ & kernel_bit)) return 0;
    uint32_t e = ++epoch_;
    if (e == 0) e = ++epoch_;
    return e;
  }
  bool lf_band() const { return ll_mask_ & 4; }
  int frame_upload(int id, const uint8_t* y, size_t ys, const uint8_t* u, const uint8_t* v, size_t cs);
  int frame_download(int id, uint8_t* y, size_t ys, uint8_t* u, uint8_t* v, size_t cs);
  int frame_download_display(int id, int lane, uint8_t* dst, size_t dst_size, bool wait);
  int frames_download_display(const int* ids, uint8_t* const* dsts, int n, int lane);
  int frame_clear(int id, int lane);
  int frame_copy(int dst, int src, int lane);
  int frame_copy_raw(int id, void* buf, size_t bytes, bool into_frame);
  int frames_equal(int a, int b, int lane, int* equal);
  int frame_hash(int id, int lane, uint64_t* out);
  int frames_ssim(int a, int b, int lane, double* out);

  int submit(int lane, const HostJob* jobs, int n, cudaEvent_t consumed, cudaEvent_t* between = nullptr);

  TokenRing token_ring_layout(size_t max_frame_bytes, bool arena = false) const;
  uint32_t token_cap_for(size_t bits) const;
  int token_ring_create(int nslots, size_t max_frame_bytes, TokenRing** out, size_t arena_tokens = 0);
  void token_ring_free(TokenRing* r);
  int token_ring_stage(TokenRing* r, int slot, const ParsedFrame& f, cudaStream_t s, vp8gpu_token* tokens = nullptr);
  int token_ring_launch(TokenRing* r, int first, int count, cudaStream_t s);
  int token_ring_clear_result(TokenRing* r, int slot, cudaStream_t s);
  int token_ring_result(TokenRing* r, int slot, cudaStream_t s, uint32_t result[2]);

  struct Resident;
  int resident_upload(const HostJob* jobs, int n, Resident** out);
  int resident_run(int lane, Resident* r, float* ms);
  int resident_run_many(int lane, Resident* const* rs, int n, float* total_ms);
  int resident_run_timed(int lane, Resident* r, float ms[3]);
  void resident_free(Resident* r);

  uint8_t* frame_dev(int id) { return frames_[id].dev; }
  const void* frame_tmaps(int id) const { return tmaps_ ? tmaps_ + (size_t)id * 384 : nullptr; }
  int acquire_frames(int lane, const int* ids, int n, uint32_t write_mask = ~0u);
  int mark_frames(int lane, const int* ids, int n, uint32_t write_mask = ~0u);
  void count_launches(int n) { launches_ += n; }

  int ensure_lane(int lane);
  int sync_all();
  int sync_lane(int lane);
  cudaStream_t stream(int lane) const { return lanes_[lane]; }
  uint64_t launches() const { return launches_.load(); }
  const char* last_error() const { return err_.c_str(); }
  int fail(int code, const std::string& what);
  int cuda_fail(cudaError_t e, const char* what);
  static std::string& thread_error();

 private:
  Engine() = default;
  struct Frame {
    uint8_t* dev = nullptr;
    int refcnt = 0;
    uint64_t pending = 0;
    cudaEvent_t ev[2 * kMaxLanes] = {};
    int wslot = -1;
    cudaEvent_t wev = nullptr;
  };
  struct Staging {
    uint8_t* dev = nullptr;
    size_t dev_cap = 0;
    uint8_t* host = nullptr;
    uint8_t* host_dev = nullptr;
    size_t host_cap = 0;
    cudaEvent_t done = nullptr;
    bool in_flight = false;
  };
  static constexpr int kEventRing = 2048;
  cudaEvent_t next_event(int slot);
  int touch(Frame& f, int slot, bool write = true, cudaEvent_t shared = nullptr);
  void collect_waits(const Frame& f, int slot, bool write, std::vector<cudaEvent_t>& out) const;
  int wait_for(Frame& f, int slot, cudaStream_t s, bool write = true);
  int build_and_launch(int lane, const DevJob* d_jobs, int* d_sync, int n, bool any_inter, bool any_intra,
                       bool any_lf, cudaEvent_t* between = nullptr);
  int count_jobs(const HostJob& j, uint32_t* n_intra, uint32_t* n_inter, uint32_t* n_filtered) const;

  int device_ = 0, width_ = 0, height_ = 0;
  Geom g_{};
  std::mutex mu_;
  std::vector<Frame> frames_;
  std::vector<int> free_;
  cudaStream_t lanes_[2 * kMaxLanes] = {};
  cudaEvent_t ring_[2 * kMaxLanes][kEventRing] = {};
  int ring_next_[2 * kMaxLanes] = {};
  Staging staging_[kMaxLanes][kStagingDepth];
  int staging_next_[kMaxLanes] = {};
  uint8_t* cmp_scratch_ = nullptr;
  float* ssim_dev_[kMaxLanes] = {};
  float* ssim_host_[kMaxLanes] = {};
  uint8_t* tmaps_ = nullptr;
  int make_tensor_maps(int id);
  std::atomic<uint64_t> launches_{0};
  std::string err_;
  std::mutex err_mu_;
  std::atomic<uint32_t> epoch_{0};
  int ll_mask_ = 1 | 4;
};

}
```

alfalfa_b200/csrc/kernels.cu:

```cuda
#include <cuda_runtime.h>
#include <stdint.h>

#include "enc_costs.h"
#include "engine.h"
#include "vp8_math.cuh"

namespace vp8 {
namespace {

#define VP8_LUT_QUALIFIER __device__ const
#include "bpred_lut.inc"

__constant__ int16_t c_sixtap[8][6] = {{0, 0, 128, 0, 0, 0},     {0, -6, 123, 12, -1, 0}, {2, -11, 108, 36, -8, 1},
                                      {0, -9, 93, 50, -6, 0},   {3, -16, 77, 77, -16, 3}, {0, -6, 50, 93, -9, 0},
                                      {1, -8, 36, 108, -11, 2}, {0, -1, 12, 123, -6, 0}};

#ifdef VP8_PROFILE
__device__ unsigned long long g_prof[32];
#define PROF_DECL unsigned long long prof_t = clock64(), prof_acc[8] = {0, 0, 0, 0, 0, 0, 0, 0}; unsigned prof_n = 0
#define PROF(i)                                  \
  do {                                           \
    const unsigned long long now_ = clock64();   \
    prof_acc[i] += now_ - prof_t;                \
    prof_t = now_;                               \
// ... 264 lines not shown
  const uint32_t nz = __ballot_sync(0xffffffffu, nonzero);
  __syncwarp();
  return nz;
}

__device__ __forceinline__ void store_mb(const uint8_t* pix, uint8_t* frame, const Geom& g, int col, int row,
                                         int lane) {
  if (lane < 16) {
    const uint4 v = *reinterpret_cast<const uint4*>(pix + lane * 16);
    *reinterpret_cast<uint4*>(frame + (size_t)(16 * row + lane) * g.y_pitch + 16 * col) = v;
  } else {
    const int plane = (lane - 16) >> 3, y = (lane - 16) & 7;
    const uint2 v = *reinterpret_cast<const uint2*>(pix + 256 + plane * 64 + y * 8);
    uint8_t* base = frame + (plane ? g.v_off : g.u_off);
    *reinterpret_cast<uint2*>(base + (size_t)(8 * row + y) * g.c_pitch + 8 * col) = v;
  }
}

constexpr int INTER_WARPS = 4;
constexpr int TSY = 48, TSC = 32;
constexpr uint32_t TILE_Y_BYTES = 21 * TSY, TILE_C_BYTES = 13 * TSC;

__constant__ uint32_t c_taps03[8] = {0x00800000u, 0x0c7bfa00u, 0x246cf502u, 0x325df700u, 0x4d4df003u, 0x5d32fa00u, 0x6c24f801u, 0x7b0cff00u};
__constant__ uint32_t c_taps45[8] = {0x0000u, 0x00ffu, 0x01f8u, 0x00fau, 0x03f0u, 0x00f7u, 0x02f5u, 0x00fau};

struct __align__(128) InterSmem {
  union {
    struct {
      uint8_t y[1024];
      uint8_t u[512];
      uint8_t v[512];
      uint8_t mid_y[21 * 16];
      uint8_t mid_c[2][13 * 8];
    } n;
    struct {
      uint8_t win[24][9][12];
      uint8_t mid[24][9][4];
    } s;
  };
  uint8_t pix[384];
  int16_t coef[COEF_I16];
  unsigned long long bar;
  uint8_t nzlist[24];
};

#ifndef VP8GPU_SIMT_EMUL
__device__ __forceinline__ uint32_t smem_u32(const void* p) { return (uint32_t)__cvta_generic_to_shared(p); }
__device__ __forceinline__ void mbar_init(unsigned long long* bar, int count) {
  asm volatile("mbarrier.init.shared::cta.b64 [%0], %1;" ::"r"(smem_u32(bar)), "r"(count) : "memory");
  asm volatile("fence.mbarrier_init.release.cluster;" ::: "memory");
  asm volatile("fence.proxy.async.shared::cta;" ::: "memory");
}
__device__ __forceinline__ void mbar_expect_tx(unsigned long long* bar, uint32_t bytes) {
  asm volatile("mbarrier.arrive.expect_tx.shared::cta.b64 _, [%0], %1;" ::"r"(smem_u32(bar)), "r"(bytes) : "memory");
}
__device__ __forceinline__ void tma_load_2d(void* dst, const void* tmap, int x, int y, unsigned long long* bar) {
  asm volatile("cp.async.bulk.tensor.2d.shared::cluster.global.tile.mbarrier::complete_tx::bytes [%0], [%1, {%2, %3}], [%4];" ::"r"(
                   smem_u32(dst)),
               "l"(tmap), "r"(x), "r"(y), "r"(smem_u32(bar))
               : "memory");
}
__device__ __forceinline__ void tmap_acquire(const void* tmap) {
#ifdef VP8_TMAP_FENCE
  asm volatile("fence.proxy.tensormap::generic.acquire.sys [%0], 128;" ::"l"(tmap) : "memory");
#else
  (void)tmap;
#endif
}
__device__ __forceinline__ void mbar_wait(unsigned long long* bar, uint32_t parity) {
  uint32_t done;
  do {
    asm volatile(
        "{\n"
        ".reg .pred p;\n"
        "mbarrier.try_wait.parity.shared::cta.b64 p, [%1], %2;\n"
        "selp.u32 %0, 1, 0, p;\n"
        "}"
        : "=r"(done)
        : "r"(smem_u32(bar)), "r"(parity)
        : "memory");
  } while (!done);
}
#else
__device__ __forceinline__ void mbar_init(unsigned long long* bar, int) { *bar = 0; }
__device__ __forceinline__ void mbar_expect_tx(unsigned long long* bar, uint32_t bytes) { *bar = bytes; }
__device__ __forceinline__ void tma_load_2d(void* dst, const void* tmap, int x, int y, unsigned long long* bar) {
  *bar -= simt::tma_copy_2d(dst, tmap, x, y);
  if (*bar == 0) *bar = 1ull << 63;
}
__device__ __forceinline__ void tmap_acquire(const void*) {}
__device__ __forceinline__ void mbar_wait(unsigned long long* bar, uint32_t) {
  while (!(*bar >> 63)) simt::yield();
}
#endif

template <int TS>
__device__ __forceinline__ void stage_clamped(uint8_t* tile, const uint8_t* __restrict__ ref, int pitch, int PW, int PH, int wx,
                                              int wy, int wcols, int wrows, int lane) {
  for (int i = lane; i < wrows * wcols; i += 32) {
    const int r = i / wcols, c = i - r * wcols;
    tile[r * TS + c] = __ldg(ref + (size_t)clampi(wy + r, 0, PH - 1) * pitch + clampi(wx + c, 0, PW - 1));
  }
}

template <int N, int TS, int OS>
__device__ __forceinline__ void hpass2(const uint8_t* tile, int o, int nrows, int mx, uint8_t* out, int lane) {
  constexpr int G = N / 4;
  const uint32_t t03 = c_taps03[mx], t45 = c_taps45[mx];
  const int sh = 8 * (o & 3);
  for (int i = lane; i < nrows * G; i += 32) {
    const int r = i / G, g = i - r * G;
    const uint32_t* w = reinterpret_cast<const uint32_t*>(tile + r * TS) + (o >> 2) + g;
    const uint32_t w0 = w[0], w1 = w[1], w2 = w[2], w3 = w[3];
    *reinterpret_cast<uint32_t*>(out + r * OS + 4 * g) =
        vp8m::sixtap_h4(vp8m::bytes_at(w0, w1, sh), vp8m::bytes_at(w1, w2, sh), vp8m::bytes_at(w2, w3, sh), t03, t45);
  }
}
template <int N, int TS, int OS>
__device__ __forceinline__ void hcopy(const uint8_t* tile, int o, int nrows, uint8_t* out, int lane) {
  constexpr int G = N / 4;
  const int sh = 8 * (o & 3);
  for (int i = lane; i < nrows * G; i += 32) {
    const int r = i / G, g = i - r * G;
    const uint32_t* w = reinterpret_cast<const uint32_t*>(tile + r * TS) + (o >> 2) + g;
    *reinterpret_cast<uint32_t*>(out + r * OS + 4 * g) = vp8m::bytes_at(w[0], w[1], sh);
  }
}
template <int R>
__device__ __forceinline__ void vitem(const uint8_t* s, int ss, const int16_t* t, uint8_t* d, int ds) {
  uint32_t p[R + 5];
#pragma unroll
  for (int k = 0; k < R + 5; k++) p[k] = vp8m::pair_of(*reinterpret_cast<const uint16_t*>(s + k * ss));
#pragma unroll
  for (int j = 0; j < R; j++)
    *reinterpret_cast<uint16_t*>(d + j * ds) = (uint16_t)vp8m::sixtap_v2(p[j], p[j + 1], p[j + 2], p[j + 3], p[j + 4], p[j + 5], t);
}

__device__ __forceinline__ void add_residuals(uint8_t* pix, const int16_t* coef, uint32_t nz, uint8_t* nzlist, int lane) {
  if ((nz >> lane) & 1) nzlist[__popc(nz & ((1u << lane) - 1))] = (uint8_t)lane;
  __syncwarp();
  const int n = 4 * __popc(nz);
  for (int i = lane; i < n; i += 32) {
    const int blk = nzlist[i >> 2], ry = i & 3;
    int off;
    if (blk < 16) off = ((blk >> 2) * 4 + ry) * 16 + (blk & 3) * 4;
    else off = 256 + ((blk - 16) >> 2) * 64 + (((blk >> 1) & 1) * 4 + ry) * 8 + (blk & 1) * 4;
    const uint2 r = *reinterpret_cast<const uint2*>(coef + blk * CS + ry * 4);
    uint32_t* p = reinterpret_cast<uint32_t*>(pix + off);
    *p = vp8m::add_residual4(*p, r.x, r.y);
  }
  __syncwarp();
}

__global__ void __launch_bounds__(INTER_WARPS * 32, 10) k_inter(const DevJob* __restrict__ jobs, Geom g) {
  __shared__ InterSmem s_all[INTER_WARPS];
  const int warp = threadIdx.x >> 5, lane = threadIdx.x & 31;
  const DevJob& J = jobs[blockIdx.y];
  const int mbi = blockIdx.x * INTER_WARPS + warp;
  if (mbi >= g.mb_cols * g.mb_rows) return;
  const MbFields f = load_mb(J.mbs + mbi);
  if (f.ref == VP8GPU_REF_CURRENT) return;
  const int row = mbi / g.mb_cols, col = mbi - row * g.mb_cols;
  InterSmem& S = s_all[warp];
  uint8_t* const pix = S.pix;
  const uint8_t* ref = J.ref[f.ref - 1];
  const uint8_t* refU = ref + g.u_off;
  const uint8_t* refV = ref + g.v_off;
  const int CW = g.W >> 1, CH = g.H >> 1;
  uint32_t nz = 0;

  if (f.y_mode != VP8GPU_SPLITMV) {
    const int mx = f.mv_x & 7, my = f.mv_y & 7;
    const int X = 16 * col + (f.mv_x >> 3) - (mx ? 2 : 0), Y = 16 * row + (f.mv_y >> 3) - (my ? 2 : 0);
    const int ncols = 16 + (mx ? 5 : 0), nrows = 16 + (my ? 5 : 0);
    const bool fastY = X >= 0 && Y >= 0 && X + ncols <= g.W && Y + nrows <= g.H;
    const int cmvx = chroma_component(4 * f.mv_x), cmvy = chroma_component(4 * f.mv_y);
    const int cmx = cmvx & 7, cmy = cmvy & 7;
    const int CX = 8 * col + (cmvx >> 3) - (cmx ? 2 : 0), CY = 8 * row + (cmvy >> 3) - (cmy ? 2 : 0);
    const int cncols = 8 + (cmx ? 5 : 0), cnrows = 8 + (cmy ? 5 : 0);
    const bool fastC = CX >= 0 && CY >= 0 && CX + cncols <= CW && CY + cnrows <= CH;
    const uint32_t tx = (fastY ? TILE_Y_BYTES : 0u) + (fastC ? 2 * TILE_C_BYTES : 0u);
    const int oY = fastY ? (X & 15) : 0, oC = fastC ? (CX & 15) : 0;
    if (lane == 0) mbar_init(&S.bar, 1);
    __syncwarp();
    if (lane == 0 && tx) {
      const uint8_t* maps = static_cast<const uint8_t*>(J.ref_tmap[f.ref - 1]);
      mbar_expect_tx(&S.bar, tx);
      if (fastY) {
        tmap_acquire(maps);
        tma_load_2d(S.n.y, maps, X & ~15, Y, &S.bar);
      }
      if (fastC) {
        tmap_acquire(maps + 128);
        tmap_acquire(maps + 256);
        tma_load_2d(S.n.u, maps + 128, CX & ~15, CY, &S.bar);
        tma_load_2d(S.n.v, maps + 256, CX & ~15, CY, &S.bar);
      }
    }
    if (f.tok_cnt) nz = build_residuals(J, f, S.coef, lane);
    if (!fastY) stage_clamped<TSY>(S.n.y, ref, g.y_pitch, g.W, g.H, X, Y, ncols, nrows, lane);
    if (!fastC) {
      stage_clamped<TSC>(S.n.u, refU, g.c_pitch, CW, CH, CX, CY, cncols, cnrows, lane);
      stage_clamped<TSC>(S.n.v, refV, g.c_pitch, CW, CH, CX, CY, cncols, cnrows, lane);
    }
    if (tx) mbar_wait(&S.bar, 0);
    __syncwarp();

    if (my == 0) {
      if (mx) hpass2<16, TSY, 16>(S.n.y, oY, 16, mx, pix, lane);
      else hcopy<16, TSY, 16>(S.n.y, oY, 16, pix, lane);
    } else {
      if (mx) hpass2<16, TSY, 16>(S.n.y, oY, 21, mx, S.n.mid_y, lane);
      else hcopy<16, TSY, 16>(S.n.y, oY, 21, S.n.mid_y, lane);
      __syncwarp();
      const int cp = lane & 7, rg = lane >> 3;
      vitem<4>(S.n.mid_y + (4 * rg) * 16 + 2 * cp, 16, c_sixtap[my], pix + (4 * rg) * 16 + 2 * cp, 16);
    }
    if (cmy == 0) {
      if (cmx) {
        hpass2<8, TSC, 8>(S.n.u, oC, 8, cmx, pix + 256, lane);
        hpass2<8, TSC, 8>(S.n.v, oC, 8, cmx, pix + 320, lane);
      } else {
        hcopy<8, TSC, 8>(lane < 16 ? S.n.u : S.n.v, oC, 8, pix + (lane < 16 ? 256 : 320), lane & 15);
      }
    } else {
      if (cmx) {
        hpass2<8, TSC, 8>(S.n.u, oC, 13, cmx, S.n.mid_c[0], lane);
        hpass2<8, TSC, 8>(S.n.v, oC, 13, cmx, S.n.mid_c[1], lane);
      } else {
        hcopy<8, TSC, 8>(S.n.u, oC, 13, S.n.mid_c[0], lane);
        hcopy<8, TSC, 8>(S.n.v, oC, 13, S.n.mid_c[1], lane);
      }
      __syncwarp();
      const int plane = lane >> 4, cp = lane & 3, rg = (lane >> 2) & 3;
      vitem<2>(S.n.mid_c[plane] + (2 * rg) * 8 + 2 * cp, 8, c_sixtap[cmy], pix + 256 + 64 * plane + (2 * rg) * 8 + 2 * cp, 8);
    }
    __syncwarp();
  } else {
    if (f.tok_cnt) nz = build_residuals(J, f, S.coef, lane);
    int lmx = 0, lmy = 0;
    if (lane < 16) {
      const uint32_t v = __ldg(reinterpret_cast<const uint32_t*>(J.split + f.split_idx) + lane);
      lmx = (int16_t)(v & 0xFFFF);
      lmy = (int16_t)(v >> 16);
    }
    const int qa = ((lane >> 1) & 1) * 8 + (lane & 1) * 2;
    const int sx = __shfl_sync(0xffffffffu, lmx, qa) + __shfl_sync(0xffffffffu, lmx, qa + 1) + __shfl_sync(0xffffffffu, lmx, qa + 4) +
                   __shfl_sync(0xffffffffu, lmx, qa + 5);
    const int sy = __shfl_sync(0xffffffffu, lmy, qa) + __shfl_sync(0xffffffffu, lmy, qa + 1) + __shfl_sync(0xffffffffu, lmy, qa + 4) +
                   __shfl_sync(0xffffffffu, lmy, qa + 5);
    int bmvx = lmx, bmvy = lmy, bx0 = 16 * col + 4 * (lane & 3), by0 = 16 * row + 4 * ((lane >> 2) & 3);
    if (lane >= 16) {
      bmvx = chroma_component(sx), bmvy = chroma_component(sy);
      bx0 = 8 * col + 4 * (lane & 1), by0 = 8 * row + 4 * ((lane >> 1) & 1);
    }
    const int bX = bx0 + (bmvx >> 3) - 2, bY = by0 + (bmvy >> 3) - 2;
    const int bfx = bmvx & 7, bfy = bmvy & 7;
    for (int it = 0; it < 7; it++) {
      const int i = it * 32 + lane, b = min(i / 9, 23), r = i - 9 * (i / 9);
      const int wx = __shfl_sync(0xffffffffu, bX, b), wy = __shfl_sync(0xffffffffu, bY, b);
      if (i < 216) {
        const uint8_t* plane = b < 16 ? ref : (b < 20 ? refU : refV);
        const int pitch = b < 16 ? g.y_pitch : g.c_pitch, PW = b < 16 ? g.W : CW, PH = b < 16 ? g.H : CH;
        const uint8_t* rowp = plane + (size_t)clampi(wy + r, 0, PH - 1) * pitch;
        uint32_t a0, a1, a2;
        if (wx >= 0 && wx + 9 <= PW) {
          const int o = wx & 3;
          const uint32_t* wp = reinterpret_cast<const uint32_t*>(rowp + (wx - o));
          const uint32_t w0 = __ldg(wp), w1 = __ldg(wp + 1), w2 = __ldg(wp + 2);
          a0 = vp8m::bytes_at(w0, w1, 8 * o), a1 = vp8m::bytes_at(w1, w2, 8 * o), a2 = w2 >> (8 * o);
        } else {
          uint32_t px[9];
#pragma unroll
          for (int k = 0; k < 9; k++) px[k] = __ldg(rowp + clampi(wx + k, 0, PW - 1));
          a0 = px[0] | (px[1] << 8) | (px[2] << 16) | (px[3] << 24);
          a1 = px[4] | (px[5] << 8) | (px[6] << 16) | (px[7] << 24);
          a2 = px[8];
        }
        uint32_t* d = reinterpret_cast<uint32_t*>(S.s.win[b][r]);
        d[0] = a0, d[1] = a1, d[2] = a2;
      }
    }
    __syncwarp();
    for (int it = 0; it < 7; it++) {
      const int i = it * 32 + lane, b = min(i / 9, 23), r = i - 9 * (i / 9);
      const int fx = __shfl_sync(0xffffffffu, bfx, b);
      if (i < 216) {
        const uint32_t* w = reinterpret_cast<const uint32_t*>(S.s.win[b][r]);
        *reinterpret_cast<uint32_t*>(S.s.mid[b][r]) =
            fx ? vp8m::sixtap_h4(w[0], w[1], w[2], c_taps03[fx], c_taps45[fx]) : vp8m::bytes_at(w[0], w[1], 16);
      }
    }
    __syncwarp();
    for (int it = 0; it < 2; it++) {
      const int i = it * 32 + lane, b = min(i >> 1, 23), cp = i & 1;
      const int fy = __shfl_sync(0xffffffffu, bfy, b);
      if (i < 48) {
        uint8_t* d;
        int ds;
        if (b < 16) d = pix + ((b >> 2) * 4) * 16 + (b & 3) * 4 + 2 * cp, ds = 16;
        else d = pix + 256 + 64 * ((b - 16) >> 2) + (((b >> 1) & 1) * 4) * 8 + (b & 1) * 4 + 2 * cp, ds = 8;
        const uint8_t* m = &S.s.mid[b][0][2 * cp];
        if (fy) {
          vitem<4>(m, 4, c_sixtap[fy], d, ds);
        } else {
#pragma unroll
          for (int j = 0; j < 4; j++) *reinterpret_cast<uint16_t*>(d + j * ds) = *reinterpret_cast<const uint16_t*>(m + (j + 2) * 4);
        }
      }
    }
    __syncwarp();
  }

  if (nz) add_residuals(pix, S.coef, nz, S.nzlist, lane);
  store_mb(pix, J.out, g, col, row, lane);
}

#ifndef VP8GPU_SIMT_EMUL
__device__ __forceinline__ int ld_progress(const int* p) {
  int v;
  asm volatile("ld.acquire.gpu.global.s32 %0, [%1];" : "=r"(v) : "l"(p) : "memory");
  return v;
}
__device__ __forceinline__ void st_progress(int* p, int v) {
  asm volatile("st.release.gpu.global.s32 [%0], %1;" ::"l"(p), "r"(v) : "memory");
}
#else
__device__ __forceinline__ int ld_progress(const int* p) {
  simt::yield();
  return *reinterpret_cast<const volatile int*>(p);
}
__device__ __forceinline__ void st_progress(int* p, int v) { *reinterpret_cast<volatile int*>(p) = v; }
#endif
#ifndef VP8GPU_SIMT_EMUL
__device__ __forceinline__ int ld_flag_cta(const int* p) {
  int v;
  asm volatile("ld.acquire.cta.shared::cta.s32 %0, [%1];" : "=r"(v) : "r"((unsigned)__cvta_generic_to_shared(p)) : "memory");
  return v;
}
__device__ __forceinline__ void st_flag_cta(int* p, int v) {
  asm volatile("st.release.cta.shared::cta.s32 [%0], %1;" ::"r"((unsigned)__cvta_generic_to_shared(p)), "r"(v) : "memory");
}
#else
__device__ __forceinline__ int ld_flag_cta(const int* p) {
  simt::yield();
  return *reinterpret_cast<const volatile int*>(p);
}
__device__ __forceinline__ void st_flag_cta(int* p, int v) { *reinterpret_cast<volatile int*>(p) = v; }
#endif
#ifndef VP8GPU_SIMT_EMUL
__device__ __forceinline__ int lane_here() {
  int l;
  asm volatile("mov.u32 %0, %%laneid;" : "=r"(l));
  return l;
}
#else
__device__ __forceinline__ int lane_here() { return threadIdx.x & 31; }
#endif
__device__ __forceinline__ void wait_flag_cta(const int* flag, int need, int lane) {
  if (lane == 0)
    while (ld_flag_cta(flag) < need) __nanosleep(20);
  __syncwarp();
}
__device__ __forceinline__ void wait_row(const int* progress_above, int need, int lane) {
  if (lane == 0) {
    unsigned ns = 20;
    while (ld_progress(progress_above) < need) {
      __nanosleep(ns);
      if (ns < 160) ns += ns;
    }
  }
  __syncwarp();
}
__device__ __forceinline__ void publish_row(int* progress, int value, int lane) {
  __syncwarp();
  if (lane == 0) st_progress(progress, value);
}
__device__ __forceinline__ uint8_t ldcg_u8(const uint8_t* p) { return __ldcg(p); }

__device__ __forceinline__ int next_marked(uint32_t my_word, int from, int nwords) {
  for (int w = from >> 5; w < nwords; w++) {
    uint32_t bits = __shfl_sync(0xffffffffu, my_word, w);
    if (w == (from >> 5)) bits &= 0xffffffffu << (from & 31);
    if (bits) return w * 32 + __ffs(bits) - 1;
  }
  return -1;
}

constexpr int WS = 48;

__device__ __forceinline__ void add_residuals_intra(uint8_t* W, uint8_t* pixc, const int16_t* coef, int lane,
                                                    bool luma_too) {
  for (int g4 = (luma_too ? lane : 64 + lane); g4 < 96; g4 += 32) {
    int blk, ry;
    uint8_t* p;
    if (g4 < 64) {
      const int y = g4 >> 2, x4 = (g4 & 3) * 4;
      blk = (y >> 2) * 4 + (x4 >> 2);
      ry = y & 3;
      p = W + (y + 1) * WS + 16 + x4;
    } else {
      const int c = g4 - 64, plane = c >> 4, cc = c & 15;
      const int y = cc >> 1, x4 = (cc & 1) * 4;
      blk = 16 + plane * 4 + (y >> 2) * 2 + (x4 >> 2);
      ry = y & 3;
      p = pixc + plane * 64 + y * 8 + x4;
    }
    const int16_t* r = coef + blk * CS + ry * 4;
    const uint32_t v = *reinterpret_cast<uint32_t*>(p);
    uint32_t o = 0;
#pragma unroll
    for (int k = 0; k < 4; k++) o |= (uint32_t)vp8m::clamp255((int)((v >> (8 * k)) & 0xFF) + r[k]) << (8 * k);
    *reinterpret_cast<uint32_t*>(p) = o;
  }
  __syncwarp();
}

constexpr int WF_WARPS = 2;

__global__ void __launch_bounds__(32 * WF_WARPS, 24) k_intra(const DevJob* __restrict__ jobs, int njobs, Geom g, int* ticket) {
  __shared__ __align__(16) uint8_t s_W[WF_WARPS][17 * WS];
  __shared__ __align__(16) uint8_t s_pixc[WF_WARPS][128];
  __shared__ __align__(16) int16_t s_coef[WF_WARPS][COEF_I16];
  __shared__ uint8_t s_aboveC[WF_WARPS][2][12];
  __shared__ uint8_t s_leftC[WF_WARPS][2][8];
  __shared__ uint16_t s_lut[WF_WARPS][128];
  const int lane = threadIdx.x & 31, warp = threadIdx.x >> 5;
  uint8_t* const W = s_W[warp];
  uint8_t* const pixc = s_pixc[warp];
  int16_t* const coef = s_coef[warp];
  uint8_t (*const aboveC)[12] = s_aboveC[warp];
  uint8_t (*const leftC)[8] = s_leftC[warp];
  uint16_t* const lut = s_lut[warp];
  for (int i = lane; i < 128; i += 32) lut[i] = k_bpred_lut[i];
  int t = 0;
  if (lane == 0) t = atomicAdd(ticket, 1);
  t = __shfl_sync(0xffffffffu, t, 0);
  const int row = t / njobs, job = t - row * njobs;
  if (row >= g.mb_rows) return;
  const DevJob& J = jobs[job];
  if (J.n_intra == 0) return;
  const int cols = g.mb_cols;
  const vp8gpu_mb* row_mbs = J.mbs + (size_t)row * cols;

  const int nwords = (cols + 31) >> 5;
  uint32_t my_word = 0;
  for (int w = 0; w < nwords; w++) {
    const int c = w * 32 + lane;
    const bool intra = c < cols && (__ldg(reinterpret_cast<const uint32_t*>(row_mbs + c) + 2) & 0xFF) == VP8GPU_REF_CURRENT;
    const uint32_t bits = __ballot_sync(0xffffffffu, intra);
    if (lane == w) my_word = bits;
  }
  uint32_t above_word = 0;
  if (row > 0)
    for (int w = 0; w < nwords; w++) {
      const int c = w * 32 + lane;
      const bool intra = c < cols && (__ldg(reinterpret_cast<const uint32_t*>(row_mbs - cols + c) + 2) & 0xFF) == VP8GPU_REF_CURRENT;
      const uint32_t bits = __ballot_sync(0xffffffffu, intra);
      if (lane == w) above_word = bits;
    }
  int col = next_marked(my_word, 0, nwords);
  int* progress = J.intra_progress + row;
  publish_row(progress, col < 0 ? cols : col, lane);

  uint8_t* const Y = J.out;
  uint8_t* const U = J.out + g.u_off;
  uint8_t* const V = J.out + g.v_off;

  PROF_DECL;
  while (col >= 0) {
    PROF(7);
    const MbFields f = load_mb(row_mbs + col);
    const bool has_res = f.tok_cnt != 0;
    PROF(0);
    if (has_res) build_residuals(J, f, coef, lane);
    PROF(1);
    if (row > 0) {
      int dep = -1;
#pragma unroll
      for (int d = -1; d <= 1; d++) {
        const int c = col + d;
        const uint32_t word = __shfl_sync(0xffffffffu, above_word, (c >> 5) & 31);
        if (c >= 0 && c < cols && ((word >> (c & 31)) & 1)) dep = c;
      }
      if (dep >= 0) wait_row(progress - 1, dep + 1, lane);
    }
    PROF(2);

    {
      const int outside_above = row == 0 ? 127 : 129;
      const uint8_t* pa = Y;
      bool va = false;
      if (lane < 21 && row > 0 && !(lane == 0 && col == 0)) {
        const int x = (lane >= 17 && col == cols - 1) ? 15 : lane - 1;
        pa = Y + (size_t)(16 * row - 1) * g.y_pitch + 16 * col + x;
        va = true;
      }
      const uint8_t* pb = Y;
      if (col > 0) {
        if (lane < 16) pb = Y + (size_t)(16 * row + lane) * g.y_pitch + 16 * col - 1;
        else pb = ((lane & 8) ? V : U) + (size_t)(8 * row + (lane & 7)) * g.c_pitch + 8 * col - 1;
      }
      const uint8_t* pc = Y;
      bool vc = false;
      const int cpl = lane >= 9, ck = lane - 9 * cpl;
      if (lane < 18 && row > 0 && !(ck == 0 && col == 0)) {
        pc = (cpl ? V : U) + (size_t)(8 * row - 1) * g.c_pitch + 8 * col + ck - 1;
        vc = true;
      }
      const int a = va ? (int)ldcg_u8(pa) : outside_above;
      const int b = col > 0 ? (int)ldcg_u8(pb) : 129;
      const int c = vc ? (int)ldcg_u8(pc) : outside_above;
      if (lane < 21) W[15 + lane] = (uint8_t)a;
      if (lane < 16) W[(lane + 1) * WS + 15] = (uint8_t)b;
      else leftC[(lane >> 3) & 1][lane & 7] = (uint8_t)b;
      if (lane < 18) aboveC[cpl][ck] = (uint8_t)c;
    }
    __syncwarp();
    PROF(3);

    {
      const int plane = lane >> 4, y = (lane >> 1) & 7, x4 = (lane & 1) * 4;
      const uint8_t* A = aboveC[plane] + 1;
      const uint8_t* L = leftC[plane];
      uint32_t word;
      if (f.uv_mode == VP8GPU_DC_PRED) {
        int s = 0, n = 0;
        if (row > 0) { for (int k = 0; k < 8; k++) s += A[k]; n += 8; }
        if (col > 0) { for (int k = 0; k < 8; k++) s += L[k]; n += 8; }
        word = (uint32_t)(n == 16 ? (s + 8) >> 4 : (n == 8 ? (s + 4) >> 3 : 128)) * 0x01010101u;
      } else if (f.uv_mode == VP8GPU_V_PRED) {
        word = (uint32_t)A[x4] | ((uint32_t)A[x4 + 1] << 8) | ((uint32_t)A[x4 + 2] << 16) | ((uint32_t)A[x4 + 3] << 24);
      } else if (f.uv_mode == VP8GPU_H_PRED) {
        word = (uint32_t)L[y] * 0x01010101u;
      } else {
        const int base = L[y] - A[-1];
        word = 0;
#pragma unroll
        for (int k = 0; k < 4; k++) word |= (uint32_t)vp8m::clamp255(base + A[x4 + k]) << (8 * k);
      }
      *reinterpret_cast<uint32_t*>(pixc + plane * 64 + y * 8 + x4) = word;
    }

    if (f.y_mode != VP8GPU_B_PRED) {
      const int y = lane >> 1, x8 = (lane & 1) * 8;
      const uint8_t* A = W + 16;
      const int left = W[(y + 1) * WS + 15];
      uint32_t w0, w1;
      if (f.y_mode == VP8GPU_DC_PRED) {
        int s = 0, n = 0;
        if (row > 0) { for (int k = 0; k < 16; k++) s += A[k]; n += 16; }
        if (col > 0) { for (int k = 0; k < 16; k++) s += W[(k + 1) * WS + 15]; n += 16; }
        w0 = w1 = (uint32_t)(n == 32 ? (s + 16) >> 5 : (n == 16 ? (s + 8) >> 4 : 128)) * 0x01010101u;
      } else if (f.y_mode == VP8GPU_V_PRED) {
        w0 = *reinterpret_cast<const uint32_t*>(A + x8);
        w1 = *reinterpret_cast<const uint32_t*>(A + x8 + 4);
      } else if (f.y_mode == VP8GPU_H_PRED) {
        w0 = w1 = (uint32_t)left * 0x01010101u;
      } else {
        const int base = left - W[15];
        w0 = w1 = 0;
#pragma unroll
        for (int k = 0; k < 4; k++) {
          w0 |= (uint32_t)vp8m::clamp255(base + A[x8 + k]) << (8 * k);
          w1 |= (uint32_t)vp8m::clamp255(base + A[x8 + 4 + k]) << (8 * k);
        }
      }
      __syncwarp();
      *reinterpret_cast<uint32_t*>(W + (y + 1) * WS + 16 + x8) = w0;
      *reinterpret_cast<uint32_t*>(W + (y + 1) * WS + 20 + x8) = w1;
      __syncwarp();
      if (has_res) add_residuals_intra(W, pixc, coef, lane, true);
    } else {
      if (lane < 12) W[(4 + 4 * (lane >> 2)) * WS + 32 + (lane & 3)] = W[32 + (lane & 3)];
      __syncwarp();
      if (has_res) add_residuals_intra(W, pixc, coef, lane, false);
      const uint64_t modes = ((uint64_t)f.bm_hi << 32) | f.bm_lo;
      const int x = lane & 3, y = (lane >> 2) & 3;
#pragma unroll
      for (int b = 0; b < 16; b++) {
        const int bx = b & 3, by = b >> 2;
        const int mode = (int)((modes >> (4 * b)) & 15);
        const uint8_t* e0 = W + (4 * by) * WS + 15 + 4 * bx;
        if (lane < 16) {
          int v;
          if (mode == VP8GPU_B_DC_PRED) {
            int s4 = 4;
#pragma unroll
            for (int k = 0; k < 4; k++) s4 += e0[1 + k] + e0[(1 + k) * WS];
            v = s4 >> 3;
          } else if (mode == VP8GPU_B_TM_PRED) {
            v = vp8m::clamp255(e0[(1 + y) * WS] + e0[1 + x] - e0[0]);
          } else {
            const unsigned entry = lut[(mode - 2) * 16 + lane];
            const int ia = entry & 15, ib = (entry >> 4) & 15, ic = (entry >> 8) & 15;
            const int pa = e0[ia < 4 ? (4 - ia) * WS : ia - 4];
            const int pb = e0[ib < 4 ? (4 - ib) * WS : ib - 4];
            const int pc = e0[ic < 4 ? (4 - ic) * WS : ic - 4];
            v = (entry & 0x1000) ? ((pa + 2 * pb + pc + 2) >> 2) : ((pa + pb + 1) >> 1);
          }
          if (has_res) v = vp8m::clamp255(v + coef[b * CS + lane]);
          W[(4 * by + y + 1) * WS + 16 + 4 * bx + x] = (uint8_t)v;
        }
        __syncwarp();
      }
    }
    __syncwarp();
    PROF(4);
    if (lane < 16) {
      *reinterpret_cast<uint4*>(Y + (size_t)(16 * row + lane) * g.y_pitch + 16 * col) =
          *reinterpret_cast<const uint4*>(W + (lane + 1) * WS + 16);
    } else {
      const int plane = (lane - 16) >> 3, yy = lane & 7;
      *reinterpret_cast<uint2*>((plane ? V : U) + (size_t)(8 * row + yy) * g.c_pitch + 8 * col) =
          *reinterpret_cast<const uint2*>(pixc + plane * 64 + yy * 8);
    }
    const int next = next_marked(my_word, col + 1, nwords);
    PROF(5);
    publish_row(progress, next < 0 ? cols : next, lane);
    PROF(6);
    PROF_COUNT();
    col = next;
  }
  PROF_FLUSH(0);
}

__device__ __forceinline__ void filter_edge_at(int* px, int q, const vp8m::LfParams& lp, bool mb_edge) {
  const int mask = vp8m::lf_mask(lp.interior, mb_edge ? lp.mb_edge : lp.sub_edge, px[q - 4], px[q - 3], px[q - 2],
                                 px[q - 1], px[q], px[q + 1], px[q + 2], px[q + 3]);
  if (!mask) return;
  const int hev = vp8m::lf_hev(lp.hev, px[q - 2], px[q - 1], px[q], px[q + 1]);
  if (mb_edge) vp8m::lf_mbedge(mask, hev, px[q - 3], px[q - 2], px[q - 1], px[q], px[q + 1], px[q + 2]);
  else vp8m::lf_inner(mask, hev, px[q - 2], px[q - 1], px[q], px[q + 1]);
}
__device__ __forceinline__ void filter_line(int* px, bool luma, bool do_mb_edge, bool do_inner,
                                            const vp8m::LfParams& lp) {
  if (do_mb_edge) filter_edge_at(px, 4, lp, true);
  if (do_inner) {
    filter_edge_at(px, 8, lp, false);
    if (luma) {
      filter_edge_at(px, 12, lp, false);
      filter_edge_at(px, 16, lp, false);
    }
  }
}

__device__ __forceinline__ void filter_region(uint8_t* ry, uint8_t (*rc)[12 * 12], const DevJob& J, const MbFields& f,
                                              bool left_edge, bool top_edge, int lane) {
  constexpr int YS = 20, CSZ = 12;
  const vp8m::LfParams lp = vp8m::lf_params(J.lf_force ? J.lf_force : f.lf_level, J.sharpness, J.key_frame);
  const bool do_inner = !((f.flags & VP8GPU_MB_HAS_Y2) && f.tok_cnt == 0);
  const bool luma = lane < 16;
  uint8_t* const plane_base = luma ? ry : rc[(lane - 16) >> 3];
  const int stride = luma ? YS : CSZ, idx = luma ? lane : (lane & 7), len = luma ? 20 : 12;
  int px[20];

  {
    const uint32_t* rw = reinterpret_cast<const uint32_t*>(plane_base + (4 + idx) * stride);
#pragma unroll
    for (int k = 0; k < 5; k++) {
      const uint32_t v = (k < 3 || luma) ? rw[k] : 0u;
      px[4 * k] = v & 0xFF, px[4 * k + 1] = (v >> 8) & 0xFF, px[4 * k + 2] = (v >> 16) & 0xFF, px[4 * k + 3] = v >> 24;
    }
    filter_line(px, luma, left_edge, do_inner, lp);
    uint32_t* ww = reinterpret_cast<uint32_t*>(plane_base + (4 + idx) * stride);
#pragma unroll
    for (int k = 0; k < 5; k++)
      if (k < 3 || luma) ww[k] = (uint32_t)px[4 * k] | ((uint32_t)px[4 * k + 1] << 8) | ((uint32_t)px[4 * k + 2] << 16) | ((uint32_t)px[4 * k + 3] << 24);
  }
  __syncwarp();
  {
    uint8_t* cp = plane_base + 4 + idx;
#pragma unroll
    for (int k = 0; k < 20; k++) px[k] = k < len ? cp[k * stride] : 0;
    filter_line(px, luma, top_edge, do_inner, lp);
#pragma unroll
    for (int k = 1; k < 19; k++)
      if (k < len - 1) cp[k * stride] = (uint8_t)px[k];
  }
  __syncwarp();
}

__global__ void __launch_bounds__(32 * WF_WARPS, 16) k_loopfilter(const DevJob* __restrict__ jobs, int njobs, Geom g, int* ticket) {
  constexpr int YS = 20, CSZ = 12;
  __shared__ __align__(16) uint8_t s_ry[WF_WARPS][20 * YS];
  __shared__ __align__(16) uint8_t s_rc[WF_WARPS][2][12 * CSZ];
  const int lane = threadIdx.x & 31, warp = threadIdx.x >> 5;
  uint8_t* const ry = s_ry[warp];
  uint8_t (*const rc)[12 * CSZ] = s_rc[warp];
  int t = 0;
  if (lane == 0) t = atomicAdd(ticket, 1);
  t = __shfl_sync(0xffffffffu, t, 0);
  const int row = t / njobs, job = t - row * njobs;
  if (row >= g.mb_rows) return;
  const DevJob& J = jobs[job];
  if (!J.lf_enabled) return;
  const int cols = g.mb_cols;
  const vp8gpu_mb* row_mbs = J.mbs + (size_t)row * cols;

  const int nwords = (cols + 31) >> 5;
  uint32_t my_word = 0;
  for (int w = 0; w < nwords; w++) {
    const int c = w * 32 + lane;
    const bool filtered = c < cols && (J.lf_force || ((__ldg(reinterpret_cast<const uint32_t*>(row_mbs + c) + 2) >> 16) & 0xFF) != 0);
    const uint32_t bits = __ballot_sync(0xffffffffu, filtered);
    if (lane == w) my_word = bits;
  }
  int col = next_marked(my_word, 0, nwords);
  int* progress = J.lf_progress + row;
  publish_row(progress, col < 0 ? cols : col, lane);

  uint8_t* const Y = J.out;
  uint8_t* const U = J.out + g.u_off;
  uint8_t* const V = J.out + g.v_off;
  const int y_lo = row > 0 ? 0 : 4;

  auto own_ptr = [&](int k, int c, const uint8_t*& gp, uint8_t*& sp) {
    const int w = lane + 32 * k;
    if (w < 64) {
      const int r = w >> 2, wx = w & 3;
      gp = Y + (size_t)(16 * row + r) * g.y_pitch + 16 * c + 4 * wx;
      sp = ry + (4 + r) * YS + 4 + 4 * wx;
    } else {
      const int cw = w - 64, plane = cw >> 4, k2 = cw & 15, r = k2 >> 1, wx = k2 & 1;
      gp = (plane ? V : U) + (size_t)(8 * row + r) * g.c_pitch + 8 * c + 4 * wx;
      sp = rc[plane] + (4 + r) * CSZ + 4 + 4 * wx;
    }
  };
  uint32_t own[3];
  auto prefetch_own = [&](int c) {
#pragma unroll
    for (int k = 0; k < 3; k++) {
      const uint8_t* gp;
      uint8_t* sp;
      own_ptr(k, c, gp, sp);
      own[k] = __ldcg(reinterpret_cast<const uint32_t*>(gp));
    }
  };
  if (col >= 0) prefetch_own(col);
  int prev = -2;

  PROF_DECL;
  while (col >= 0) {
    PROF(7);
    const MbFields f = load_mb(row_mbs + col);
    const bool have_left = prev == col - 1;
    PROF(0);
    if (row > 0) wait_row(progress - 1, min(col + 2, cols), lane);
    PROF(1);

    uint32_t top = 0;
    if (row > 0) {
      if (lane < 16) {
        const int r = lane >> 2, wx = lane & 3;
        top = __ldcg(reinterpret_cast<const uint32_t*>(Y + (size_t)(16 * row - 4 + r) * g.y_pitch + 16 * col + 4 * wx));
      } else {
        const int cw = lane - 16, plane = cw >> 3, k2 = cw & 7, r = k2 >> 1, wx = k2 & 1;
        top = __ldcg(reinterpret_cast<const uint32_t*>((plane ? V : U) + (size_t)(8 * row - 4 + r) * g.c_pitch + 8 * col + 4 * wx));
      }
    }
    uint32_t left0 = 0, left1 = 0;
    if (col > 0) {
      if (have_left) {
        if (lane < 20) left0 = *reinterpret_cast<const uint32_t*>(ry + lane * YS + 16);
        if (lane < 24) left1 = *reinterpret_cast<const uint32_t*>(rc[lane / 12] + (lane % 12) * CSZ + 8);
      } else {
        if (lane < 20 && lane >= y_lo)
          left0 = __ldcg(reinterpret_cast<const uint32_t*>(Y + (size_t)(16 * row - 4 + lane) * g.y_pitch + 16 * col - 4));
        if (lane < 24 && (lane % 12) >= y_lo)
          left1 = __ldcg(reinterpret_cast<const uint32_t*>((lane / 12 ? V : U) + (size_t)(8 * row - 4 + lane % 12) * g.c_pitch + 8 * col - 4));
      }
    }
    __syncwarp();
    if (col > 0) {
      if (lane < 20) *reinterpret_cast<uint32_t*>(ry + lane * YS) = left0;
      if (lane < 24) *reinterpret_cast<uint32_t*>(rc[lane / 12] + (lane % 12) * CSZ) = left1;
    }
    if (row > 0) {
      if (lane < 16) *reinterpret_cast<uint32_t*>(ry + (lane >> 2) * YS + 4 + 4 * (lane & 3)) = top;
      else {
        const int cw = lane - 16, plane = cw >> 3, k2 = cw & 7;
        *reinterpret_cast<uint32_t*>(rc[plane] + (k2 >> 1) * CSZ + 4 + 4 * (k2 & 1)) = top;
      }
    }
#pragma unroll
    for (int k = 0; k < 3; k++) {
      const uint8_t* gp;
      uint8_t* sp;
      own_ptr(k, col, gp, sp);
      *reinterpret_cast<uint32_t*>(sp) = own[k];
    }
    __syncwarp();
    PROF(2);
    const int next = next_marked(my_word, col + 1, nwords);
    if (next >= 0) prefetch_own(next);

    filter_region(ry, rc, J, f, col > 0, row > 0, lane);

    PROF(3);
    const int x_lo = col > 0 ? 0 : 1;
    const bool flush_right = next != col + 1;
    {
      uint8_t* const gy = Y + (size_t)(16 * row - 4) * g.y_pitch + 16 * col - 4;
#pragma unroll
      for (int k = 0; k < 3; k++) {
        const int w = lane + 32 * k, r = w >> 2, wx = w & 3;
        if (w < 80 && r >= y_lo && wx >= x_lo)
          *reinterpret_cast<uint32_t*>(gy + (size_t)r * g.y_pitch + 4 * wx) = *reinterpret_cast<const uint32_t*>(ry + r * YS + 4 * wx);
      }
#pragma unroll
      for (int k = 0; k < 2; k++) {
        const int w = lane + 32 * k, plane = w >= 24, kk = w - 24 * plane, r = kk >> 1, wx = kk & 1;
        if (w < 48 && r >= y_lo && wx >= x_lo)
          *reinterpret_cast<uint32_t*>((plane ? V : U) + (size_t)(8 * row - 4 + r) * g.c_pitch + 8 * col - 4 + 4 * wx) =
              *reinterpret_cast<const uint32_t*>(rc[plane] + r * CSZ + 4 * wx);
      }
      if (flush_right) {
        if (lane < 20 && lane >= y_lo)
          *reinterpret_cast<uint32_t*>(gy + (size_t)lane * g.y_pitch + 16) = *reinterpret_cast<const uint32_t*>(ry + lane * YS + 16);
        if (lane < 24) {
          const int plane = lane >= 12, r = lane - 12 * plane;
          if (r >= y_lo)
            *reinterpret_cast<uint32_t*>((plane ? V : U) + (size_t)(8 * row - 4 + r) * g.c_pitch + 8 * col + 4) =
                *reinterpret_cast<const uint32_t*>(rc[plane] + r * CSZ + 8);
        }
      }
    }
    PROF(4);
    publish_row(progress, next < 0 ? cols : next, lane);
    PROF(5);
    PROF_COUNT();
    prev = col;
    col = next;
  }
  PROF_FLUSH(16);
}

constexpr int LF_BAND = 4, LF_RING = 8;

__global__ void __launch_bounds__(32 * LF_BAND, 32 / LF_BAND) k_loopfilter_band(const DevJob* __restrict__ jobs, int njobs, Geom g, int* ticket) {
  constexpr int YS = 20, CSZ = 12;
  struct Row {
    uint8_t ry[20 * YS];
    uint8_t rc[2][12 * CSZ];
    uint32_t ring[LF_RING][32];
    int done;
    int free;
    int pad[2];
  };
  __shared__ __align__(16) Row s_rows[LF_BAND];
  __shared__ int s_ticket;
  const int lane = threadIdx.x & 31, warp = threadIdx.x >> 5;
  if (threadIdx.x == 0) s_ticket = atomicAdd(ticket, 1);
  if (threadIdx.x < LF_BAND) s_rows[threadIdx.x].done = 0, s_rows[threadIdx.x].free = 0;
  __syncthreads();
  const int band = s_ticket / njobs, job = s_ticket - band * njobs;
  const int row = band * LF_BAND + warp;
  if (row >= g.mb_rows) return;
  const DevJob& J = jobs[job];
  if (!J.lf_enabled) return;
  const int cols = g.mb_cols;
  const vp8gpu_mb* row_mbs = J.mbs + (size_t)row * cols;
  Row* const S = s_rows + warp;
  uint8_t* const ry = S->ry;
  uint8_t (*const rc)[12 * CSZ] = S->rc;
  const bool ring_in = warp > 0;
  const bool ring_out = warp < LF_BAND - 1 && row + 1 < g.mb_rows;

  const int nwords = (cols + 31) >> 5;
  uint32_t my_word = 0, above_word = 0;
  for (int w = 0; w < nwords; w++) {
    const int c = w * 32 + lane;
    const bool filtered = c < cols && (J.lf_force || ((__ldg(reinterpret_cast<const uint32_t*>(row_mbs + c) + 2) >> 16) & 0xFF) != 0);
    const uint32_t bits = __ballot_sync(0xffffffffu, filtered);
    if (lane == w) my_word = bits;
    if (ring_in) {
      const bool fa = c < cols && (J.lf_force || ((__ldg(reinterpret_cast<const uint32_t*>(row_mbs - cols + c) + 2) >> 16) & 0xFF) != 0);
      const uint32_t bits_above = __ballot_sync(0xffffffffu, fa);
      if (lane == w) above_word = bits_above;
    }
  }
  int* const progress = J.lf_progress + row;
  auto publish = [&](int done, int free) {
    __syncwarp();
    if (lane == 0) {
      if (warp == LF_BAND - 1) st_progress(progress, done);
      else st_flag_cta(&S->done, done);
      if (ring_in) st_flag_cta(&S->free, free);
    }
  };
  int col = next_marked(my_word, 0, nwords);
  publish(col < 0 ? cols : col, col < 0 ? cols : col - 1);

  uint8_t* const Y = J.out;
  uint8_t* const U = J.out + g.u_off;
  uint8_t* const V = J.out + g.v_off;
  const int y_lo = row > 0 ? 0 : 4;

  auto own_ptr = [&](int k, int c, const uint8_t*& gp, uint8_t*& sp) {
    const int w = lane_here() + 32 * k;
    if (w < 64) {
      const int r = w >> 2, wx = w & 3;
      gp = Y + (size_t)(16 * row + r) * g.y_pitch + 16 * c + 4 * wx;
      sp = ry + (4 + r) * YS + 4 + 4 * wx;
    } else {
      const int cw = w - 64, plane = cw >> 4, k2 = cw & 15, r = k2 >> 1, wx = k2 & 1;
      gp = (plane ? V : U) + (size_t)(8 * row + r) * g.c_pitch + 8 * c + 4 * wx;
      sp = rc[plane] + (4 + r) * CSZ + 4 + 4 * wx;
    }
  };
  uint32_t own[3];
  auto prefetch_own = [&](int c) {
#pragma unroll
    for (int k = 0; k < 3; k++) {
      const uint8_t* gp;
      uint8_t* sp;
      own_ptr(k, c, gp, sp);
      own[k] = __ldcg(reinterpret_cast<const uint32_t*>(gp));
    }
  };
  if (col >= 0) prefetch_own(col);
  int prev = -2;

  PROF_DECL;
  while (col >= 0) {
    PROF(7);
    const MbFields f = load_mb(row_mbs + col);
    const bool have_left = prev == col - 1;
    uint32_t abits = 0;
    if (ring_in) {
#pragma unroll
      for (int d = -1; d <= 1; d++) {
        const int c = col + d;
        const uint32_t word = __shfl_sync(0xffffffffu, above_word, (c >> 5) & 31);
        if (c >= 0 && c < cols && ((word >> (c & 31)) & 1)) abits |= 1u << (d + 1);
      }
    }
    PROF(0);
    if (ring_in) wait_flag_cta(&S[-1].done, min(col + 2, cols), lane);
    PROF(1);
    if (!ring_in && row > 0) wait_row(progress - 1, min(col + 2, cols), lane);
    PROF(2);

    const int lane = lane_here();
    uint32_t top = 0;
    if (row > 0) {
      const uint8_t* tp;
      bool right;
      if (lane < 16) {
        const int r = lane >> 2, wx = lane & 3;
        tp = Y + (size_t)(16 * row - 4 + r) * g.y_pitch + 16 * col + 4 * wx;
        right = wx == 3;
      } else {
        const int cw = lane - 16, plane = cw >> 3, k2 = cw & 7, r = k2 >> 1, wx = k2 & 1;
        tp = (plane ? V : U) + (size_t)(8 * row - 4 + r) * g.c_pitch + 8 * col + 4 * wx;
        right = wx == 1;
      }
      const bool in_ring = (abits & 2) || (right && (abits & 4));
      top = in_ring ? S[-1].ring[col & (LF_RING - 1)][lane] : __ldcg(reinterpret_cast<const uint32_t*>(tp));
    }
    uint32_t left0 = 0, left1 = 0;
    if (col > 0) {
      if (have_left) {
        if (lane < 20) left0 = *reinterpret_cast<const uint32_t*>(ry + lane * YS + 16);
        if (lane < 24) left1 = *reinterpret_cast<const uint32_t*>(rc[lane / 12] + (lane % 12) * CSZ + 8);
      } else {
        const uint32_t* const corner = S[-1].ring[(col - 1) & (LF_RING - 1)];
        const bool corner_in_ring = (abits & 3) != 0;
        if (lane < 20 && lane >= y_lo)
          left0 = corner_in_ring && lane < 4
                      ? corner[4 * lane + 3]
                      : __ldcg(reinterpret_cast<const uint32_t*>(Y + (size_t)(16 * row - 4 + lane) * g.y_pitch + 16 * col - 4));
        if (lane < 24 && (lane % 12) >= y_lo)
          left1 = corner_in_ring && lane % 12 < 4
                      ? corner[16 + 8 * (lane / 12) + 2 * (lane % 12) + 1]
                      : __ldcg(reinterpret_cast<const uint32_t*>((lane / 12 ? V : U) + (size_t)(8 * row - 4 + lane % 12) * g.c_pitch + 8 * col - 4));
      }
    }
    __syncwarp();
    if (col > 0) {
      if (lane < 20) *reinterpret_cast<uint32_t*>(ry + lane * YS) = left0;
      if (lane < 24) *reinterpret_cast<uint32_t*>(rc[lane / 12] + (lane % 12) * CSZ) = left1;
    }
    if (row > 0) {
      if (lane < 16) *reinterpret_cast<uint32_t*>(ry + (lane >> 2) * YS + 4 + 4 * (lane & 3)) = top;
      else {
        const int cw = lane - 16, plane = cw >> 3, k2 = cw & 7;
        *reinterpret_cast<uint32_t*>(rc[plane] + (k2 >> 1) * CSZ + 4 + 4 * (k2 & 1)) = top;
      }
    }
#pragma unroll
    for (int k = 0; k < 3; k++) {
      const uint8_t* gp;
      uint8_t* sp;
      own_ptr(k, col, gp, sp);
      *reinterpret_cast<uint32_t*>(sp) = own[k];
    }
    __syncwarp();
    PROF(3);
    const int next = next_marked(my_word, col + 1, nwords);
    if (next >= 0) prefetch_own(next);

    filter_region(ry, rc, J, f, col > 0, row > 0, lane);

    PROF(4);
    if (ring_out) wait_flag_cta(&S[1].free, col - LF_RING + 1, lane);
    PROF(5);
    const int x_lo = col > 0 ? 0 : 1;
    const bool flush_right = next != col + 1;
    uint32_t* const slot = S->ring[col & (LF_RING - 1)];
    uint32_t* const slot_left = S->ring[(col - 1) & (LF_RING - 1)];
    {
      const int lane = lane_here();
// ... 1067 lines not shown
```

alfalfa_b200/csrc/tokens.cu:

```cuda
#include <cuda_runtime.h>
#include <stdint.h>
#include <stdlib.h>

#include "engine.h"
#include "tokens_core.cuh"

namespace vp8 {
namespace {

constexpr int kMaxCols = 1024;
template <int kTokWarps>
__global__ void __launch_bounds__(32 * kTokWarps) k_tokens(const uint8_t* ring, size_t stride, int first, int count,
                                                          int nslots, Geom g) {
  __shared__ __align__(16) uint8_t probs_all[kTokWarps][tok::kProbBytes];
  __shared__ uint16_t above_all[kTokWarps][kMaxCols];
  const int warp = kTokWarps == 1 ? 0 : threadIdx.x >> 5, lane = threadIdx.x & 31;
  const int job = blockIdx.x * kTokWarps + warp;
  if (job >= count) return;
  uint8_t* probs = probs_all[warp];
  uint16_t* above_nz = above_all[warp];
  const TokJob& J = *reinterpret_cast<const TokJob*>(ring + static_cast<size_t>((first + job) % nslots) * stride);
  for (int e = lane; e < tok::kProbEntries; e += 32) tok::expand_prob_entry(J.coef_probs, probs, e);
  for (int i = lane; i < g.mb_cols; i += 32) above_nz[i] = 0;
  __syncwarp();
  if (lane != 0) return;
  tok::decode_frame_tokens(J, g, probs, above_nz);
}

__global__ void __launch_bounds__(32) k_tokens_lockstep(const uint8_t* ring, size_t stride, int first, int count,
                                                         int nslots, Geom g) {
#ifdef VP8GPU_SIMT_EMUL
  uint8_t* const dyn = simt::dyn_smem();
#else
  extern __shared__ __align__(16) uint8_t dyn[];
#endif
  __shared__ tok::LockstepTables T;
  uint8_t* const P = dyn;
  uint16_t* const above = reinterpret_cast<uint16_t*>(dyn + 1056 * 32);
  const int lane = threadIdx.x;
  tok::fill_lockstep_tables(T, lane, 32);
  const int job = blockIdx.x * 32 + lane;
  const TokJob* J = job < count ? reinterpret_cast<const TokJob*>(ring + static_cast<size_t>((first + job) % nslots) * stride) : nullptr;
  if (J) {
    const uint32_t* src = reinterpret_cast<const uint32_t*>(J->coef_probs);
    for (int w = 0; w < 264; w++) {
      const uint32_t v = __ldg(src + w);
      P[(4 * w + 0) * 32 + lane] = v & 0xFF;
      P[(4 * w + 1) * 32 + lane] = (v >> 8) & 0xFF;
      P[(4 * w + 2) * 32 + lane] = (v >> 16) & 0xFF;
      P[(4 * w + 3) * 32 + lane] = v >> 24;
    }
  }
  __syncwarp();
  if (!J) return;
  tok::decode_frame_tokens_lockstep<32>(*J, g, T, P + lane, above + lane);
}

}

int launch_tokens(const uint8_t* ring, size_t stride, int first, int count, int nslots, const Geom& g, void* stream) {
  if (g.mb_cols > kMaxCols) return (int)cudaErrorInvalidValue;
  static const int warps = [] {
    const char* v = getenv("VP8GPU_TOK_WARPS");
    return v && atoi(v) == 8 ? 8 : (v && atoi(v) == 32 ? 32 : 1);
  }();
  cudaStream_t s = static_cast<cudaStream_t>(stream);
  if (warps == 32) {
    const size_t smem = 1056 * 32 + (size_t)g.mb_cols * 32 * sizeof(uint16_t);
    static const cudaError_t attr = cudaFuncSetAttribute(k_tokens_lockstep, cudaFuncAttributeMaxDynamicSharedMemorySize, 1056 * 32 + kMaxCols * 64);
    if (attr != cudaSuccess) return (int)attr;
    VP8_LAUNCH(k_tokens_lockstep, (count + 31) / 32, 32, smem, s)(ring, stride, first, count, nslots, g);
  }
  else if (warps == 8) VP8_LAUNCH(k_tokens<8>, (count + 7) / 8, 256, 0, s)(ring, stride, first, count, nslots, g);
  else VP8_LAUNCH(k_tokens<1>, count, 32, 0, s)(ring, stride, first, count, nslots, g);
  return (int)cudaGetLastError();
}

}
```

alfalfa_b200/csrc/wavefront_ll.cuh:

```cuda

struct Msg {
  uint32_t d, f;
};
#ifndef VP8GPU_SIMT_EMUL
__device__ __forceinline__ Msg ld_msg(const unsigned long long* p) {
  unsigned long long v;
  asm volatile("ld.relaxed.gpu.global.u64 %0, [%1];" : "=l"(v) : "l"(p) : "memory");
  Msg m;
  m.d = (uint32_t)v;
  m.f = (uint32_t)(v >> 32);
  return m;
}
__device__ __forceinline__ void st_msg(unsigned long long* p, uint32_t d, uint32_t f) {
  const unsigned long long v = (unsigned long long)d | ((unsigned long long)f << 32);
  asm volatile("st.relaxed.gpu.global.u64 [%0], %1;" ::"l"(p), "l"(v) : "memory");
}
#else
__device__ __forceinline__ Msg ld_msg(const unsigned long long* p) {
  simt::yield();
  const unsigned long long v = *reinterpret_cast<const volatile unsigned long long*>(p);
  Msg m;
  m.d = (uint32_t)v;
  m.f = (uint32_t)(v >> 32);
  return m;
}
__device__ __forceinline__ void st_msg(unsigned long long* p, uint32_t d, uint32_t f) {
  *reinterpret_cast<volatile unsigned long long*>(p) = (unsigned long long)d | ((unsigned long long)f << 32);
}
#endif
__device__ __forceinline__ uint32_t wait_msg(const unsigned long long* p, Msg m, bool need, uint32_t epoch) {
  unsigned ns = 32;
  for (;;) {
    const bool ok = !need || m.f == epoch;
    const unsigned late = __ballot_sync(0xffffffffu, !ok);
    if (!late) break;
    const int watcher = __ffs(late) - 1;
    if ((threadIdx.x & 31) == watcher) {
      for (;;) {
        __nanosleep(ns);
        m = ld_msg(p);
        if (m.f == epoch) break;
        if (ns < 256) ns += ns;
      }
    }
    __syncwarp();
    if (!ok && (threadIdx.x & 31) != watcher) m = ld_msg(p);
  }
  return need ? m.d : 0u;
}

struct MbRaw {
  uint32_t x, y, z, bz, bw;
};
__device__ __forceinline__ MbRaw load_mb_raw(const vp8gpu_mb* p) {
  const uint4* q = reinterpret_cast<const uint4*>(p);
  const uint4 a = __ldg(q);
  const uint2 b = __ldg(reinterpret_cast<const uint2*>(p) + 3);
  MbRaw r;
  r.x = a.x, r.y = a.y, r.z = a.z, r.bz = b.x, r.bw = b.y;
  return r;
}
__device__ __forceinline__ MbFields decode_mb(const MbRaw& r) {
  MbFields f;
  f.tok_off = r.x;
  f.tok_cnt = r.y & 0xFFFF;
  f.y_mode = (r.y >> 16) & 0xFF;
  f.uv_mode = r.y >> 24;
  f.ref = r.z & 0xFF;
  f.segment = (r.z >> 8) & 0xFF;
  f.lf_level = (r.z >> 16) & 0xFF;
  f.flags = r.z >> 24;
  f.mv_x = f.mv_y = 0;
  f.split_idx = 0;
  f.bm_lo = r.bz;
  f.bm_hi = r.bw;
  return f;
}

__global__ void __launch_bounds__(32 * WF_WARPS, 18) k_intra_ll(const DevJob* __restrict__ jobs, int njobs, Geom g, int* ticket,
                                                                 uint32_t epoch) {
  __shared__ __align__(16) uint8_t s_W[WF_WARPS][17 * WS];
  __shared__ __align__(16) uint8_t s_pixc[WF_WARPS][128];
  __shared__ __align__(16) int16_t s_coef[WF_WARPS][COEF_I16];
  __shared__ uint8_t s_aboveC[WF_WARPS][2][12];
  __shared__ uint8_t s_leftC[WF_WARPS][2][8];
  __shared__ uint16_t s_lut[WF_WARPS][128];
  const int lane = threadIdx.x & 31, warp = threadIdx.x >> 5;
  uint8_t* const W = s_W[warp];
  uint8_t* const pixc = s_pixc[warp];
  int16_t* const coef = s_coef[warp];
  uint8_t (*const aboveC)[12] = s_aboveC[warp];
  uint8_t (*const leftC)[8] = s_leftC[warp];
  uint16_t* const lut = s_lut[warp];
  for (int i = lane; i < 128; i += 32) lut[i] = k_bpred_lut[i];
  int t = 0;
  if (lane == 0) t = atomicAdd(ticket, 1);
  t = __shfl_sync(0xffffffffu, t, 0);
  const int row = t / njobs, job = t - row * njobs;
  if (row >= g.mb_rows) return;
  const DevJob& J = jobs[job];
  if (J.n_intra == 0) return;
  const int cols = g.mb_cols;
  const vp8gpu_mb* row_mbs = J.mbs + (size_t)row * cols;

  const int nwords = (cols + 31) >> 5;
  uint32_t my_word = 0, above_word = 0;
  for (int w = 0; w < nwords; w++) {
    const int c = w * 32 + lane;
    const bool intra = c < cols && (__ldg(reinterpret_cast<const uint32_t*>(row_mbs + c) + 2) & 0xFF) == VP8GPU_REF_CURRENT;
    const uint32_t bits = __ballot_sync(0xffffffffu, intra);
    if (lane == w) my_word = bits;
    bool above = false;
    if (row > 0) above = c < cols && (__ldg(reinterpret_cast<const uint32_t*>(row_mbs - cols + c) + 2) & 0xFF) == VP8GPU_REF_CURRENT;
    const uint32_t abits = __ballot_sync(0xffffffffu, above);
    if (lane == w) above_word = abits;
  }
  int col = next_marked(my_word, 0, nwords);

  uint8_t* const Y = J.out;
  uint8_t* const U = J.out + g.u_off;
  uint8_t* const V = J.out + g.v_off;
  unsigned long long* const msg_row = reinterpret_cast<unsigned long long*>(J.out + g.msg_intra_off) + (size_t)row * cols * 8;
  const unsigned long long* const msg_above = msg_row - (size_t)cols * 8;
  const bool sends = row + 1 < g.mb_rows;

  MbRaw raw;
  raw.x = raw.y = raw.z = raw.bz = raw.bw = 0;
  if (col >= 0) raw = load_mb_raw(row_mbs + col);
  int prev = -2;

  PROF_DECL;
  while (col >= 0) {
    PROF(7);
    const int next = next_marked(my_word, col + 1, nwords);
    const MbFields f = decode_mb(raw);
    if (next >= 0) raw = load_mb_raw(row_mbs + next);
    const bool has_res = f.tok_cnt != 0;
    PROF(0);

    bool ia_l = false, ia_c = false, ia_r = false;
    if (row > 0) {
#pragma unroll
      for (int d = -1; d <= 1; d++) {
        const int c = col + d;
        const uint32_t word = __shfl_sync(0xffffffffu, above_word, (c >> 5) & 31);
        const bool bit = c >= 0 && c < cols && ((word >> (c & 31)) & 1);
        if (d == -1) ia_l = bit;
        else if (d == 0) ia_c = bit;
        else ia_r = bit;
      }
    }
    const unsigned long long* mp = msg_above;
    bool need = false;
    if (lane < 8) {
      need = ia_c;
      mp = msg_above + (size_t)col * 8 + lane;
    } else if (lane == 8) {
      need = ia_r;
      mp = msg_above + (size_t)(col + 1) * 8;
    } else if (lane < 12) {
      need = ia_l;
      mp = msg_above + (size_t)(col - 1) * 8 + (2 * (lane - 9) + 3);
    }
    Msg m;
    m.d = 0, m.f = 0;
    if (need) m = ld_msg(mp);

    const int outside_above = row == 0 ? 127 : 129;
    const int ax = (lane >= 17 && col == cols - 1) ? 15 : lane - 1;
    const bool va = lane < 21 && row > 0 && !(lane == 0 && col == 0);
    const bool a_msg = va && (ax < 0 ? ia_l : (ax < 16 ? ia_c : ia_r));
    int a = outside_above;
    if (va && !a_msg) a = (int)ldcg_u8(Y + (size_t)(16 * row - 1) * g.y_pitch + 16 * col + ax);
    const int cpl = lane >= 9, ck = lane - 9 * cpl;
    const bool vc = lane < 18 && row > 0 && !(ck == 0 && col == 0);
    const bool c_msg = vc && (ck == 0 ? ia_l : ia_c);
    int c = outside_above;
    if (vc && !c_msg) c = (int)ldcg_u8((cpl ? V : U) + (size_t)(8 * row - 1) * g.c_pitch + 8 * col + ck - 1);
    int b = 129;
    if (col > 0) {
      if (prev == col - 1) {
        b = lane < 16 ? W[(lane + 1) * WS + 31] : pixc[((lane >> 3) & 1) * 64 + (lane & 7) * 8 + 7];
      } else {
        const uint8_t* pb = lane < 16 ? Y + (size_t)(16 * row + lane) * g.y_pitch + 16 * col - 1
                                      : ((lane & 8) ? V : U) + (size_t)(8 * row + (lane & 7)) * g.c_pitch + 8 * col - 1;
        b = (int)ldcg_u8(pb);
      }
    }
    __syncwarp();

    if (has_res) build_residuals(J, f, coef, lane);
    PROF(1);

    const uint32_t md = wait_msg(mp, m, need, epoch);
    PROF(2);
    {
      const int sl = ax < 0 ? 9 : (ax < 16 ? (ax >> 2) : 8);
      const int sb = ax < 0 ? 3 : (ax & 3);
      const uint32_t w = __shfl_sync(0xffffffffu, md, sl & 31);
      if (a_msg) a = (int)((w >> (8 * sb)) & 0xFF);
      const int cx = ck - 1;
      const int cl = cx < 0 ? 10 + cpl : 4 + 2 * cpl + ((cx >> 2) & 1);
      const int cb = cx < 0 ? 3 : (cx & 3);
      const uint32_t wc = __shfl_sync(0xffffffffu, md, cl & 31);
      if (c_msg) c = (int)((wc >> (8 * cb)) & 0xFF);
    }
    if (lane < 21) W[15 + lane] = (uint8_t)a;
    if (lane < 16) W[(lane + 1) * WS + 15] = (uint8_t)b;
    else leftC[(lane >> 3) & 1][lane & 7] = (uint8_t)b;
    if (lane < 18) aboveC[cpl][ck] = (uint8_t)c;
    __syncwarp();
    PROF(3);

    {
      const int plane = lane >> 4, y = (lane >> 1) & 7, x4 = (lane & 1) * 4;
      const uint8_t* A = aboveC[plane] + 1;
      const uint8_t* L = leftC[plane];
      uint32_t word;
      if (f.uv_mode == VP8GPU_DC_PRED) {
        int s = 0, n = 0;
        if (row > 0) { for (int k = 0; k < 8; k++) s += A[k]; n += 8; }
        if (col > 0) { for (int k = 0; k < 8; k++) s += L[k]; n += 8; }
        word = (uint32_t)(n == 16 ? (s + 8) >> 4 : (n == 8 ? (s + 4) >> 3 : 128)) * 0x01010101u;
      } else if (f.uv_mode == VP8GPU_V_PRED) {
        word = (uint32_t)A[x4] | ((uint32_t)A[x4 + 1] << 8) | ((uint32_t)A[x4 + 2] << 16) | ((uint32_t)A[x4 + 3] << 24);
      } else if (f.uv_mode == VP8GPU_H_PRED) {
        word = (uint32_t)L[y] * 0x01010101u;
      } else {
        const int base = L[y] - A[-1];
        word = 0;
#pragma unroll
        for (int k = 0; k < 4; k++) word |= (uint32_t)vp8m::clamp255(base + A[x4 + k]) << (8 * k);
      }
      *reinterpret_cast<uint32_t*>(pixc + plane * 64 + y * 8 + x4) = word;
    }

    if (f.y_mode != VP8GPU_B_PRED) {
      const int y = lane >> 1, x8 = (lane & 1) * 8;
      const uint8_t* A = W + 16;
      const int left = W[(y + 1) * WS + 15];
      uint32_t w0, w1;
      if (f.y_mode == VP8GPU_DC_PRED) {
        int s = 0, n = 0;
        if (row > 0) { for (int k = 0; k < 16; k++) s += A[k]; n += 16; }
        if (col > 0) { for (int k = 0; k < 16; k++) s += W[(k + 1) * WS + 15]; n += 16; }
        w0 = w1 = (uint32_t)(n == 32 ? (s + 16) >> 5 : (n == 16 ? (s + 8) >> 4 : 128)) * 0x01010101u;
      } else if (f.y_mode == VP8GPU_V_PRED) {
        w0 = *reinterpret_cast<const uint32_t*>(A + x8);
        w1 = *reinterpret_cast<const uint32_t*>(A + x8 + 4);
      } else if (f.y_mode == VP8GPU_H_PRED) {
        w0 = w1 = (uint32_t)left * 0x01010101u;
      } else {
        const int base = left - W[15];
        w0 = w1 = 0;
#pragma unroll
        for (int k = 0; k < 4; k++) {
          w0 |= (uint32_t)vp8m::clamp255(base + A[x8 + k]) << (8 * k);
          w1 |= (uint32_t)vp8m::clamp255(base + A[x8 + 4 + k]) << (8 * k);
        }
      }
      __syncwarp();
      *reinterpret_cast<uint32_t*>(W + (y + 1) * WS + 16 + x8) = w0;
      *reinterpret_cast<uint32_t*>(W + (y + 1) * WS + 20 + x8) = w1;
      __syncwarp();
      if (has_res) add_residuals_intra(W, pixc, coef, lane, true);
    } else {
      if (lane < 12) W[(4 + 4 * (lane >> 2)) * WS + 32 + (lane & 3)] = W[32 + (lane & 3)];
      __syncwarp();
      if (has_res) add_residuals_intra(W, pixc, coef, lane, false);
      const uint64_t modes = ((uint64_t)f.bm_hi << 32) | f.bm_lo;
      const int x = lane & 3, y = (lane >> 2) & 3;
#pragma unroll
      for (int bi = 0; bi < 16; bi++) {
        const int bx = bi & 3, by = bi >> 2;
        const int mode = (int)((modes >> (4 * bi)) & 15);
        const uint8_t* e0 = W + (4 * by) * WS + 15 + 4 * bx;
        if (lane < 16) {
          int v;
          if (mode == VP8GPU_B_DC_PRED) {
            int s4 = 4;
#pragma unroll
            for (int k = 0; k < 4; k++) s4 += e0[1 + k] + e0[(1 + k) * WS];
            v = s4 >> 3;
          } else if (mode == VP8GPU_B_TM_PRED) {
            v = vp8m::clamp255(e0[(1 + y) * WS] + e0[1 + x] - e0[0]);
          } else {
            const unsigned entry = lut[(mode - 2) * 16 + lane];
            const int ia = entry & 15, ib = (entry >> 4) & 15, ic = (entry >> 8) & 15;
            const int pa = e0[ia < 4 ? (4 - ia) * WS : ia - 4];
            const int pb = e0[ib < 4 ? (4 - ib) * WS : ib - 4];
            const int pc = e0[ic < 4 ? (4 - ic) * WS : ic - 4];
            v = (entry & 0x1000) ? ((pa + 2 * pb + pc + 2) >> 2) : ((pa + pb + 1) >> 1);
          }
          if (has_res) v = vp8m::clamp255(v + coef[bi * CS + lane]);
          W[(4 * by + y + 1) * WS + 16 + 4 * bx + x] = (uint8_t)v;
        }
        __syncwarp();
      }
    }
    __syncwarp();
    PROF(4);
    if (sends && lane < 8) {
      const uint32_t d = lane < 4 ? *reinterpret_cast<const uint32_t*>(W + 16 * WS + 16 + 4 * lane)
                                  : *reinterpret_cast<const uint32_t*>(pixc + ((lane - 4) >> 1) * 64 + 56 + 4 * (lane & 1));
      st_msg(msg_row + (size_t)col * 8 + lane, d, epoch);
    }
    if (lane < 16) {
      *reinterpret_cast<uint4*>(Y + (size_t)(16 * row + lane) * g.y_pitch + 16 * col) =
          *reinterpret_cast<const uint4*>(W + (lane + 1) * WS + 16);
    } else {
      const int plane = (lane - 16) >> 3, yy = lane & 7;
      *reinterpret_cast<uint2*>((plane ? V : U) + (size_t)(8 * row + yy) * g.c_pitch + 8 * col) =
          *reinterpret_cast<const uint2*>(pixc + plane * 64 + yy * 8);
    }
    PROF(5);
    PROF(6);
    PROF_COUNT();
    prev = col;
    col = next;
  }
  PROF_FLUSH(0);
}

__global__ void __launch_bounds__(32 * WF_WARPS, 14) k_loopfilter_ll(const DevJob* __restrict__ jobs, int njobs, Geom g, int* ticket,
                                                                      uint32_t epoch) {
  constexpr int YS = 20, CSZ = 12;
  __shared__ __align__(16) uint8_t s_ry[WF_WARPS][20 * YS];
  __shared__ __align__(16) uint8_t s_rc[WF_WARPS][2][12 * CSZ];
  const int lane = threadIdx.x & 31, warp = threadIdx.x >> 5;
  uint8_t* const ry = s_ry[warp];
  uint8_t (*const rc)[12 * CSZ] = s_rc[warp];
  int t = 0;
  if (lane == 0) t = atomicAdd(ticket, 1);
  t = __shfl_sync(0xffffffffu, t, 0);
  const int row = t / njobs, job = t - row * njobs;
  if (row >= g.mb_rows) return;
  const DevJob& J = jobs[job];
  if (!J.lf_enabled) return;
  const int cols = g.mb_cols;
  const vp8gpu_mb* row_mbs = J.mbs + (size_t)row * cols;
  const bool last_row = row == g.mb_rows - 1;

  uint8_t* const Y = J.out;
  uint8_t* const U = J.out + g.u_off;
  uint8_t* const V = J.out + g.v_off;
  const int y_lo = row > 0 ? 0 : 4;
  const int y_hi = last_row ? 20 : 16;
  const int yc_hi = last_row ? 12 : 8;
  auto msg_at = [&](int r, int c) {
    return reinterpret_cast<unsigned long long*>(Y + g.msg_lf_off) + ((size_t)r * (cols + 1) + c) * 32 + lane;
  };

  const bool luma_w = lane < 16;
  const int mj = luma_w ? lane >> 2 : ((lane - 16) & 7) >> 1;
  const int mw = luma_w ? lane & 3 : lane & 1;
  const int mp = luma_w ? 0 : (lane - 16) >> 3;
  const int words = luma_w ? 4 : 2;
  const int line0 = luma_w ? 4 * mj : 16 + 8 * mp + 2 * mj;

  auto own_ptr = [&](int k, int c, const uint8_t*& gp, uint8_t*& sp) {
    const int w = lane + 32 * k;
    if (w < 64) {
      const int r = w >> 2, wx = w & 3;
      gp = Y + (size_t)(16 * row + r) * g.y_pitch + 16 * c + 4 * wx;
      sp = ry + (4 + r) * YS + 4 + 4 * wx;
    } else {
      const int cw = w - 64, plane = cw >> 4, k2 = cw & 15, r = k2 >> 1, wx = k2 & 1;
      gp = (plane ? V : U) + (size_t)(8 * row + r) * g.c_pitch + 8 * c + 4 * wx;
      sp = rc[plane] + (4 + r) * CSZ + 4 + 4 * wx;
    }
  };
  uint32_t own[3];
  auto prefetch_own = [&](int c) {
#pragma unroll
    for (int k = 0; k < 3; k++) {
      const uint8_t* gp;
      uint8_t* sp;
      own_ptr(k, c, gp, sp);
      own[k] = __ldcg(reinterpret_cast<const uint32_t*>(gp));
    }
  };
  prefetch_own(0);
  uint32_t a0 = 0;
  Msg spec;
  spec.d = 0, spec.f = 0;
  if (row > 0) {
    a0 = wait_msg(msg_at(row - 1, 0), ld_msg(msg_at(row - 1, 0)), true, epoch);
    spec = ld_msg(msg_at(row - 1, 1));
  }

  PROF_DECL;
  for (int col = 0; col < cols; col++) {
    PROF(7);
    PROF(0);
    uint32_t top = 0;
    if (row > 0) {
      const uint32_t a1 = wait_msg(msg_at(row - 1, col + 1), spec, true, epoch);
      if (col + 2 <= cols) spec = ld_msg(msg_at(row - 1, col + 2));
      const uint32_t t0 = __shfl_sync(0xffffffffu, a0, (line0 + ((mw + 1) & (words - 1))) & 31);
      const uint32_t t1 = __shfl_sync(0xffffffffu, a1, line0 & 31);
      top = mw == words - 1 ? t1 : t0;
      a0 = a1;
    }
    PROF(1);
    uint32_t left0 = 0, left1 = 0;
    if (col > 0) {
      if (lane < 20) left0 = *reinterpret_cast<const uint32_t*>(ry + lane * YS + 16);
      if (lane < 24) left1 = *reinterpret_cast<const uint32_t*>(rc[lane / 12] + (lane % 12) * CSZ + 8);
    }
    __syncwarp();
    if (col > 0) {
      if (lane < 20) *reinterpret_cast<uint32_t*>(ry + lane * YS) = left0;
      if (lane < 24) *reinterpret_cast<uint32_t*>(rc[lane / 12] + (lane % 12) * CSZ) = left1;
    }
    if (row > 0) {
      if (luma_w) *reinterpret_cast<uint32_t*>(ry + mj * YS + 4 + 4 * mw) = top;
      else *reinterpret_cast<uint32_t*>(rc[mp] + mj * CSZ + 4 + 4 * mw) = top;
    }
#pragma unroll
    for (int k = 0; k < 3; k++) {
      const uint8_t* gp;
      uint8_t* sp;
      own_ptr(k, col, gp, sp);
      *reinterpret_cast<uint32_t*>(sp) = own[k];
    }
    __syncwarp();
    PROF(2);
    if (col + 1 < cols) prefetch_own(col + 1);

    const uint32_t rec_y = __ldg(reinterpret_cast<const uint32_t*>(row_mbs + col) + 1);
    const uint32_t rec_z = __ldg(reinterpret_cast<const uint32_t*>(row_mbs + col) + 2);
    const int mb_tok_cnt = rec_y & 0xFFFF, mb_level = (rec_z >> 16) & 0xFF, mb_flags = rec_z >> 24;
    const int level = J.lf_force ? J.lf_force : mb_level;
    if (level != 0) {
      const vp8m::LfParams lp = vp8m::lf_params(level, J.sharpness, J.key_frame);
      const bool do_inner = !((mb_flags & VP8GPU_MB_HAS_Y2) && mb_tok_cnt == 0);
      const bool luma = lane < 16;
      uint8_t* const plane_base = luma ? ry : rc[(lane - 16) >> 3];
      const int stride = luma ? YS : CSZ, idx = luma ? lane : (lane & 7), len = luma ? 20 : 12;
      int px[20];
      {
        const uint32_t* rw = reinterpret_cast<const uint32_t*>(plane_base + (4 + idx) * stride);
#pragma unroll
        for (int k = 0; k < 5; k++) {
          const uint32_t v = (k < 3 || luma) ? rw[k] : 0u;
          px[4 * k] = v & 0xFF, px[4 * k + 1] = (v >> 8) & 0xFF, px[4 * k + 2] = (v >> 16) & 0xFF, px[4 * k + 3] = v >> 24;
        }
        filter_line(px, luma, col > 0, do_inner, lp);
        uint32_t* ww = reinterpret_cast<uint32_t*>(plane_base + (4 + idx) * stride);
#pragma unroll
        for (int k = 0; k < 5; k++)
          if (k < 3 || luma) ww[k] = (uint32_t)px[4 * k] | ((uint32_t)px[4 * k + 1] << 8) | ((uint32_t)px[4 * k + 2] << 16) | ((uint32_t)px[4 * k + 3] << 24);
      }
      __syncwarp();
      {
        uint8_t* cp = plane_base + 4 + idx;
#pragma unroll
        for (int k = 0; k < 20; k++) px[k] = k < len ? cp[k * stride] : 0;
        filter_line(px, luma, row > 0, do_inner, lp);
#pragma unroll
        for (int k = 1; k < 19; k++)
          if (k < len - 1) cp[k * stride] = (uint8_t)px[k];
      }
      __syncwarp();
    }
    PROF(3);

    const bool last_col = col == cols - 1;
    if (!last_row) {
      const uint8_t* src = luma_w ? ry + (16 + mj) * YS : rc[mp] + (8 + mj) * CSZ;
      st_msg(msg_at(row, col), *reinterpret_cast<const uint32_t*>(src + 4 * mw), epoch);
      if (last_col) st_msg(msg_at(row, cols), *reinterpret_cast<const uint32_t*>(src + (luma_w ? 16 : 8)), epoch);
    }
    const int x_lo = col > 0 ? 0 : 1;
    {
      uint8_t* const gy = Y + (size_t)(16 * row - 4) * g.y_pitch + 16 * col - 4;
#pragma unroll
      for (int k = 0; k < 3; k++) {
        const int w = lane + 32 * k, r = w >> 2, wx = w & 3;
        if (w < 80 && r >= y_lo && r < y_hi && wx >= x_lo)
          *reinterpret_cast<uint32_t*>(gy + (size_t)r * g.y_pitch + 4 * wx) = *reinterpret_cast<const uint32_t*>(ry + r * YS + 4 * wx);
      }
#pragma unroll
      for (int k = 0; k < 2; k++) {
        const int w = lane + 32 * k, plane = w >= 24, kk = w - 24 * plane, r = kk >> 1, wx = kk & 1;
        if (w < 48 && r >= y_lo && r < yc_hi && wx >= x_lo)
          *reinterpret_cast<uint32_t*>((plane ? V : U) + (size_t)(8 * row - 4 + r) * g.c_pitch + 8 * col - 4 + 4 * wx) =
              *reinterpret_cast<const uint32_t*>(rc[plane] + r * CSZ + 4 * wx);
      }
      if (last_col) {
        if (lane < 20 && lane >= y_lo && lane < y_hi)
// ... 16 lines not shown
```

Before: 10950.

## Replace per-chunk ready events with per-frame mapped-memory ready flags

The token kernel now publishes a per-slot epoch to device memory and to a mapped host word once each frame's tokens are decoded. Dispatchers poll these host words instead of calling cudaEventQuery on a per-chunk event, and can take the first ready frame of each GOP rather than waiting on the whole chunk. Reconstruction kernels do an acquire load on the device word in place of a cudaStreamWaitEvent. The ramp-up that launched smaller first chunks is removed, and optional globaltimer stamps are added for tracing. This relies on the host-side ready flag for cross-stream ordering, so correctness now depends on the memory fences, and the dispatcher does more polling and deque erasure.

```diff
diff --git a/alfalfa_b200/csrc/capi.cc b/alfalfa_b200/csrc/capi.cc
--- a/alfalfa_b200/csrc/capi.cc
+++ b/alfalfa_b200/csrc/capi.cc
@@ -79,7 +79,7 @@
   cudaStream_t kstream[kTokStreams] = {};
   int next_kstream = 0;
   vp8gpu_parsed* parsed[kTokSlots] = {};
-  cudaEvent_t staged[kTokSlots] = {}, ready[kTokSlots] = {}, finished[kTokSlots] = {};
+  cudaEvent_t staged[kTokSlots] = {}, finished[kTokSlots] = {};
   bool busy[kTokSlots] = {};
 };
 struct vp8gpu_resident_batch {
@@ -147,7 +147,6 @@
     for (int i = 0; i < kTokSlots; i++) {
       if (k->parsed[i]) vp8gpu_parsed_destroy(k->parsed[i]);
       if (k->staged[i]) cudaEventDestroy(k->staged[i]);
-      if (k->ready[i]) cudaEventDestroy(k->ready[i]);
     }
     delete k;
   }
@@ -956,9 +955,11 @@
     int64_t out_off;
     int* slot_state;
     int tid = 0;
+    int gop = 0;
     const vp8::TokenRing* ring = nullptr;
     int ring_slot = 0;
-    cudaEvent_t ready = nullptr;
+    const volatile uint32_t* ready_word = nullptr;
+    uint32_t epoch = 0;
     cudaEvent_t* finished = nullptr;
   };
 
@@ -1170,6 +1171,7 @@
         std::lock_guard<std::mutex> lk(mu);
         slot_state[si] = kQueued;
         job.tid = tid;
+        job.gop = g;
         queues[tid].push_back(job);
       }
       cv_disp[tid % n_disp].notify_one();
@@ -1239,7 +1241,6 @@
     k->parsed[i]->f.mbs.reserve(n_mbs, 0);
     k->parsed[i]->f.split.reserve(256, 0);
     cudaEventCreateWithFlags(&k->staged[i], cudaEventDisableTiming);
-    cudaEventCreateWithFlags(&k->ready[i], cudaEventDisableTiming);
   }
   return k;
 }
@@ -1252,7 +1253,6 @@
   int refs[3] = {-1, -1, -1};
   int slot_state[kTokSlots] = {};
   int next_slot = 0;
-  int launches_done = 0;
   int rc = VP8GPU_OK;
   ivf_worker_kit* kit = acquire_kit();
   if (!kit) rc = e->fail(VP8GPU_ERR_NOMEM, "decode_ivf: token ring allocation failed");
@@ -1263,8 +1263,16 @@
   struct ChunkTrace {
     cudaEvent_t ev[3];
     int frames;
+    int stamp;
   };
   std::vector<ChunkTrace> chunk_trace;
+  constexpr int kTraceStamps = 1024;
+  const int stamp_row = tok_chunk + 1;
+  unsigned long long* stamps = nullptr;
+  unsigned long long* stamps_dev = nullptr;
+  if (knobs.trace && (cudaHostAlloc(&stamps, sizeof(unsigned long long) * stamp_row * kTraceStamps, cudaHostAllocMapped) != cudaSuccess ||
+                      cudaHostGetDevicePointer(reinterpret_cast<void**>(&stamps_dev), stamps, 0) != cudaSuccess))
+    stamps_dev = nullptr;
   auto arena_take = [&](int si, size_t need, auto in_chunk, vp8gpu_token** out) {
     const size_t cap = arena_tokens;
     if (held[si]) {
@@ -1315,12 +1323,10 @@
     uint32_t i = gop_start[g];
     while (i < gop_start[g + 1] && rc == VP8GPU_OK) {
       const uint32_t left = gop_start[g + 1] - i;
-      int want = tok_chunk;
-      if (launches_done < 3 && (2 << launches_done) < want) want = 2 << launches_done;
-      launches_done++;
-      const int n = (int)left < want ? (int)left : want;
+      const int n = (int)left < tok_chunk ? (int)left : tok_chunk;
       const int first_slot = next_slot;
       int staged = 0, permits_taken = 0;
+      const int stamp = stamps_dev && chunk_trace.size() < (size_t)kTraceStamps ? (int)chunk_trace.size() : -1;
       for (int c = 0; c < n && rc == VP8GPU_OK; c++) {
         const int si = (first_slot + c) % tok_slots;
         const double t0 = now();
@@ -1344,7 +1350,7 @@
           return (s - first_slot + tok_slots) % tok_slots < c;
         }, &tokens);
         if (rc != VP8GPU_OK) break;
-        rc = e->token_ring_stage(kit->ring, si, p->f, kit->copy_stream, tokens);
+        rc = e->token_ring_stage(kit->ring, si, p->f, kit->copy_stream, tokens, stamp >= 0 ? stamps_dev + stamp_row * stamp + 1 + c : nullptr);
         if (rc != VP8GPU_OK) break;
         staged++;
         t_slot += t1 - t0;
@@ -1354,9 +1360,10 @@
       if (rc != VP8GPU_OK) break;
       cudaStream_t ks = kit->kstream[kit->next_kstream];
       kit->next_kstream = (kit->next_kstream + 1) % kTokStreams;
+      if (stamp >= 0) vp8::launch_stamp(stamps_dev + stamp_row * stamp, kit->copy_stream);
       cudaEventRecord(kit->staged[first_slot], kit->copy_stream);
       cudaStreamWaitEvent(ks, kit->staged[first_slot], 0);
-      ChunkTrace ctr{{nullptr, nullptr, nullptr}, staged};
+      ChunkTrace ctr{{nullptr, nullptr, nullptr}, staged, stamp};
       if (knobs.trace) {
         for (cudaEvent_t& ev : ctr.ev) cudaEventCreate(&ev);
         cudaEventRecord(ctr.ev[0], kit->copy_stream);
@@ -1372,8 +1379,6 @@
       const int until_wrap = tok_slots - first_slot;
       rc = e->token_ring_launch(kit->ring, first_slot, staged < until_wrap ? staged : until_wrap, ks);
       if (rc == VP8GPU_OK && staged > until_wrap) rc = e->token_ring_launch(kit->ring, 0, staged - until_wrap, ks);
-      if (rc == VP8GPU_OK)
-        cudaEventRecord(kit->ready[first_slot], ks);
       if (knobs.trace) {
         cudaEventRecord(ctr.ev[2], ks);
         chunk_trace.push_back(ctr);
@@ -1393,7 +1398,8 @@
         job.out_off = (dst && desc.show_frame) ? items[i + c].out_off : -1;
         job.ring = kit->ring;
         job.ring_slot = si;
-        job.ready = kit->ready[first_slot];
+        job.ready_word = kit->ring->host_ready_word(si);
+        job.epoch = kit->ring->slot_epoch[si];
         job.finished = &kit->finished[si];
         rc = e->frame_alloc(&job.out);
         if (rc != VP8GPU_OK) break;
@@ -1407,7 +1413,8 @@
           std::lock_guard<std::mutex> lk(mu);
           slot_state[si] = kQueued;
           job.tid = tid;
-        queues[tid].push_back(job);
+          job.gop = g;
+          queues[tid].push_back(job);
         }
         cv_disp[tid % n_disp].notify_one();
       }
@@ -1457,12 +1464,17 @@
     if (knobs.trace) {
       fprintf(stderr, "decode_ivf arena: worker %d takes %ld wraps %ld waits %ld cap %zu slots %d chunk %d\n", tid, n_takes, n_wraps,
               n_waits, arena_tokens, tok_slots, tok_chunk);
-      std::vector<float> lat, kern;
+      std::vector<float> lat, kern, head, last;
       long frames = 0;
       for (ChunkTrace& c : chunk_trace) {
         float ms = 0;
         if (cudaEventElapsedTime(&ms, c.ev[0], c.ev[2]) == cudaSuccess) lat.push_back(ms);
         if (cudaEventElapsedTime(&ms, c.ev[1], c.ev[2]) == cudaSuccess) kern.push_back(ms);
+        if (c.stamp >= 0) {
+          const unsigned long long* row = stamps + stamp_row * c.stamp;
+          head.push_back((float)((double)(row[1] - row[0]) * 1e-6));
+          last.push_back((float)((double)(*std::max_element(row + 1, row + 1 + c.frames) - row[0]) * 1e-6));
+        }
         frames += c.frames;
         for (cudaEvent_t ev : c.ev) cudaEventDestroy(ev);
       }
@@ -1471,18 +1483,22 @@
         std::sort(v.begin(), v.end());
         return (double)v[std::min(v.size() - 1, (size_t)(q * (v.size() - 1) + 0.5))];
       };
-      fprintf(stderr, "[trace] worker %d chunks: %zu (%ld frames); staged -> ready ms p10 %.2f p50 %.2f p90 %.2f max %.2f; "
-              "k_tokens start -> ready ms p50 %.2f p90 %.2f max %.2f\n", tid, chunk_trace.size(), frames, pct(lat, 0.1), pct(lat, 0.5),
-              pct(lat, 0.9), pct(lat, 1.0), pct(kern, 0.5), pct(kern, 0.9), pct(kern, 1.0));
+      fprintf(stderr, "[trace] worker %d chunks: %zu (%ld frames); staged -> head ready ms p10 %.2f p50 %.2f p90 %.2f max %.2f; "
+              "staged -> last frame ready ms p50 %.2f p90 %.2f max %.2f; events: staged -> ready ms p10 %.2f p50 %.2f p90 %.2f max %.2f; "
+              "k_tokens start -> ready ms p50 %.2f p90 %.2f max %.2f\n", tid, chunk_trace.size(), frames, pct(head, 0.1), pct(head, 0.5),
+              pct(head, 0.9), pct(head, 1.0), pct(last, 0.5), pct(last, 0.9), pct(last, 1.0), pct(lat, 0.1), pct(lat, 0.5), pct(lat, 0.9),
+              pct(lat, 1.0), pct(kern, 0.5), pct(kern, 0.9), pct(kern, 1.0));
     }
     std::lock_guard<std::mutex> lk(ctx->pool_mu);
     ctx->kit_pool.push_back(kit);
   }
+  if (stamps) cudaFreeHost(stamps);
 }
 
 void IvfDecode::dispatcher(int di) {
   cudaSetDevice(e->device());
   std::vector<Pending> batch;
+  std::vector<size_t> take;
   std::vector<HostJob> hj;
   std::vector<int> dl_ids;
   std::vector<uint8_t*> dl_dst;
@@ -1501,21 +1517,18 @@
     const double ti = now();
     {
       std::unique_lock<std::mutex> lk(mu);
-      auto eligible = [&](std::deque<Pending>& q) {
-        if (q.empty()) return false;
-        Pending& f = q.front();
-        if (!f.ready) return true;
-        if (cudaEventQuery(f.ready) != cudaSuccess) return false;
-        const cudaEvent_t fired = f.ready;
-        for (Pending& p : q) {
-          if (p.ready != fired) break;
-          p.ready = nullptr;
+      auto each_eligible = [&](const std::deque<Pending>& q, auto&& fn) {
+        int prev_gop = -1;
+        for (size_t k = 0; k < q.size(); k++) {
+          const Pending& f = q[k];
+          if (f.gop == prev_gop) continue;
+          prev_gop = f.gop;
+          if (!f.ready_word || *f.ready_word == f.epoch) fn(k);
         }
-        return true;
       };
       auto ready = [&] {
         int n = 0;
-        for (int t = di; t < threads; t += n_disp) n += eligible(queues[t]);
+        for (int t = di; t < threads; t += n_disp) each_eligible(queues[t], [&](size_t) { n++; });
         return n;
       };
       auto queued = [&] {
@@ -1536,11 +1549,13 @@
           break;
         }
       }
-      for (int t = di; t < threads; t += n_disp)
-        if (eligible(queues[t])) {
-          batch.push_back(queues[t].front());
-          queues[t].pop_front();
-        }
+      for (int t = di; t < threads; t += n_disp) {
+        std::deque<Pending>& q = queues[t];
+        take.clear();
+        each_eligible(q, [&](size_t k) { take.push_back(k); });
+        for (size_t k : take) batch.push_back(q[k]);
+        for (size_t j = take.size(); j-- > 0;) q.erase(q.begin() + (std::ptrdiff_t)take[j]);
+      }
       if (batch.empty() && running[di] == 0 && !queued()) break;
     }
     if (batch.empty()) continue;
@@ -1564,7 +1579,6 @@
       if (b.ring) {
         j.ring = b.ring;
         j.ring_slot = b.ring_slot;
-        j.ready = nullptr;
         j.finished = b.finished;
         j.consumed = nullptr;
       }
diff --git a/alfalfa_b200/csrc/engine.cu b/alfalfa_b200/csrc/engine.cu
--- a/alfalfa_b200/csrc/engine.cu
+++ b/alfalfa_b200/csrc/engine.cu
@@ -538,6 +538,7 @@
   r.bits_cap = (uint32_t)align_up(max_frame_bytes + 16, 256);
   r.split_cap = (uint32_t)n_mbs;
   r.tok_cap = token_cap_for(max_frame_bytes);
+  static_assert(sizeof(TokJob) <= 256, "a slot's TokJob area");
   size_t off = 256;
   r.probs_off = off;
   off += 1280;
@@ -547,6 +548,7 @@
   off = align_up(off + r.bits_cap, 256);
   r.host_stride = off;
   r.result_off = off;
+  r.ready_off = off + 8;
   off += 256;
   r.above_off = off;
   off = align_up(off + 2 * (size_t)g_.mb_cols, 256);
@@ -565,14 +567,18 @@
   TokenRing* r = new TokenRing(token_ring_layout(max_frame_bytes, arena_tokens > 0));
   r->nslots = nslots;
   r->slot_tokens.assign(nslots, nullptr);
+  r->slot_epoch.assign(nslots, 0);
   r->arena_cap = arena_tokens;
   if (cudaMalloc(&r->dev, r->stride * nslots) != cudaSuccess ||
       (arena_tokens && cudaMalloc(&r->arena, arena_tokens * sizeof(vp8gpu_token)) != cudaSuccess) ||
-      cudaHostAlloc(&r->host, r->host_stride * nslots, cudaHostAllocDefault) != cudaSuccess) {
+      cudaHostAlloc(&r->host, r->host_stride * nslots, cudaHostAllocDefault) != cudaSuccess ||
+      cudaHostAlloc(&r->ready_host, sizeof(uint32_t) * nslots, cudaHostAllocMapped) != cudaSuccess ||
+      cudaHostGetDevicePointer(reinterpret_cast<void**>(&r->ready_host_dev), r->ready_host, 0) != cudaSuccess) {
     token_ring_free(r);
     return fail(VP8GPU_ERR_NOMEM, "token ring allocation failed");
   }
-  CU(cudaMemset2D(r->dev + r->result_off, r->stride, 0, 8, (size_t)nslots));
+  memset(r->ready_host, 0, sizeof(uint32_t) * nslots);
+  CU(cudaMemset2D(r->dev + r->result_off, r->stride, 0, 12, (size_t)nslots));
   *out = r;
   return VP8GPU_OK;
 }
@@ -583,10 +589,12 @@
   if (r->dev) cudaFree(r->dev);
   if (r->arena) cudaFree(r->arena);
   if (r->host) cudaFreeHost(r->host);
+  if (r->ready_host) cudaFreeHost(r->ready_host);
   delete r;
 }
 
-int Engine::token_ring_stage(TokenRing* r, int slot, const ParsedFrame& f, cudaStream_t s, vp8gpu_token* tokens) {
+int Engine::token_ring_stage(TokenRing* r, int slot, const ParsedFrame& f, cudaStream_t s, vp8gpu_token* tokens,
+                             unsigned long long* stamp) {
   const TokenWork& tw = f.tw;
   if (!tw.deferred) return fail(VP8GPU_ERR_LOGIC, "token_ring_stage: frame was not parsed with defer_tokens");
   if (tw.bits_len > r->bits_cap || f.desc.n_split > r->split_cap)
@@ -607,6 +615,10 @@
   memcpy(j->part_len, tw.part_len, sizeof(j->part_len));
   j->nparts = tw.nparts;
   j->tok_cap = tokens ? token_cap_for(tw.bits_len) : r->tok_cap;
+  j->ready = reinterpret_cast<uint32_t*>(d + r->ready_off);
+  j->ready_host = r->ready_host_dev + slot;
+  j->epoch = r->slot_epoch[slot] = fresh_epoch();
+  j->stamp = stamp;
   memcpy(h + r->probs_off, tw.coef_probs, 1056);
   memcpy(h + r->bits_off, tw.bits, tw.bits_len);
   const size_t n_mbs = (size_t)g_.mb_cols * g_.mb_rows;
@@ -688,6 +700,8 @@
         d.mbs = reinterpret_cast<const vp8gpu_mb*>(slot + j.ring->mbs_off);
         d.tokens = j.ring->slot_tokens[j.ring_slot];
         d.split = reinterpret_cast<const vp8gpu_split_mvs*>(slot + j.ring->split_off);
+        d.ready = j.ring->dev_ready_word(j.ring_slot);
+        d.ready_epoch = j.ring->slot_epoch[j.ring_slot];
       } else {
         d.mbs = reinterpret_cast<const vp8gpu_mb*>(st.dev + L.mbs_off[i]);
         d.tokens = reinterpret_cast<const vp8gpu_token*>(st.dev + L.tok_off[i]);
@@ -728,10 +742,7 @@
   const size_t n_mbs = (size_t)g_.mb_cols * g_.mb_rows;
   for (int i = 0; i < n; i++) {
     const HostJob& j = jobs[i];
-    if (j.ring) {
-      if (j.ready) CU(cudaStreamWaitEvent(s, j.ready, 0));
-      continue;
-    }
+    if (j.ring) continue;
     CU(cudaMemcpyAsync(st.dev + L.mbs_off[i], j.mbs, n_mbs * sizeof(vp8gpu_mb), cudaMemcpyHostToDevice, s));
     if (j.desc->n_tokens)
       CU(cudaMemcpyAsync(st.dev + L.tok_off[i], j.tokens, (size_t)j.desc->n_tokens * sizeof(vp8gpu_token),
diff --git a/alfalfa_b200/csrc/engine.h b/alfalfa_b200/csrc/engine.h
--- a/alfalfa_b200/csrc/engine.h
+++ b/alfalfa_b200/csrc/engine.h
@@ -30,12 +30,13 @@
   const void* ref_tmap[3];
   int* intra_progress;
   int* lf_progress;
+  const uint32_t* ready;
   vp8gpu_quant quant[4];
   uint8_t key_frame, sharpness, lf_enabled;
   uint8_t lf_force;
   uint32_t n_intra;
   uint32_t n_inter;
-  uint32_t pad2;
+  uint32_t ready_epoch;
 };
 
 struct EncTables;
@@ -88,6 +89,10 @@
   uint32_t part_off[8], part_len[8];
   uint32_t nparts;
   uint32_t tok_cap;
+  uint32_t* ready;
+  uint32_t* ready_host;
+  uint32_t epoch;
+  unsigned long long* stamp;
 };
 
 int launch_inter(const DevJob* jobs, int njobs, const Geom& g, void* stream);
@@ -97,6 +102,7 @@
 int launch_intra(const DevJob* jobs, int njobs, const Geom& g, int* ticket, uint32_t epoch, void* stream);
 int launch_loopfilter(const DevJob* jobs, int njobs, const Geom& g, int* ticket, uint32_t epoch, bool band, void* stream);
 int launch_tokens(const uint8_t* ring, size_t stride, int first, int count, int nslots, const Geom& g, void* stream);
+int launch_stamp(unsigned long long* dst, void* stream);
 int launch_fetch_header(void* dst, const void* src_host_devptr, size_t bytes, void* stream);
 int launch_ssim(const uint8_t* a, const uint8_t* b, const Geom& g, float* d_windows, void* stream);
 int launch_enc_rd(const EncJob* jobs, int njobs, int rows, const Geom& g, int* ticket, void* stream);
diff --git a/alfalfa_b200/csrc/engine.hpp b/alfalfa_b200/csrc/engine.hpp
--- a/alfalfa_b200/csrc/engine.hpp
+++ b/alfalfa_b200/csrc/engine.hpp
@@ -25,6 +25,12 @@
   vp8gpu_token* arena = nullptr;
   size_t arena_cap = 0;
   std::vector<vp8gpu_token*> slot_tokens;
+  std::vector<uint32_t> slot_epoch;
+  uint32_t* ready_host = nullptr;
+  uint32_t* ready_host_dev = nullptr;
+  size_t ready_off = 0;
+  const volatile uint32_t* host_ready_word(int i) const { return ready_host + i; }
+  const uint32_t* dev_ready_word(int i) const { return reinterpret_cast<const uint32_t*>(dev_slot(i) + ready_off); }
   uint8_t* dev_slot(int i) const { return dev + (size_t)i * stride; }
   uint8_t* host_slot(int i) const { return host + (size_t)i * host_stride; }
 };
@@ -41,7 +47,6 @@
   cudaEvent_t consumed = nullptr;
   const TokenRing* ring = nullptr;
   int ring_slot = 0;
-  cudaEvent_t ready = nullptr;
   cudaEvent_t* finished = nullptr;
 };
 
@@ -65,12 +70,12 @@
     for (const Frame& f : frames_) n += f.refcnt > 0;
     return n;
   }
-  uint32_t next_epoch(int kernel_bit = 3) {
-    if (!(ll_mask_ & kernel_bit)) return 0;
+  uint32_t fresh_epoch() {
     uint32_t e = ++epoch_;
     if (e == 0) e = ++epoch_;
     return e;
   }
+  uint32_t next_epoch(int kernel_bit = 3) { return (ll_mask_ & kernel_bit) ? fresh_epoch() : 0; }
   bool lf_band() const { return ll_mask_ & 4; }
   int frame_upload(int id, const uint8_t* y, size_t ys, const uint8_t* u, const uint8_t* v, size_t cs);
   int frame_download(int id, uint8_t* y, size_t ys, uint8_t* u, uint8_t* v, size_t cs);
@@ -89,7 +94,8 @@
   uint32_t token_cap_for(size_t bits) const;
   int token_ring_create(int nslots, size_t max_frame_bytes, TokenRing** out, size_t arena_tokens = 0);
   void token_ring_free(TokenRing* r);
-  int token_ring_stage(TokenRing* r, int slot, const ParsedFrame& f, cudaStream_t s, vp8gpu_token* tokens = nullptr);
+  int token_ring_stage(TokenRing* r, int slot, const ParsedFrame& f, cudaStream_t s, vp8gpu_token* tokens = nullptr,
+                       unsigned long long* stamp = nullptr);
   int token_ring_launch(TokenRing* r, int first, int count, cudaStream_t s);
   int token_ring_clear_result(TokenRing* r, int slot, cudaStream_t s);
   int token_ring_result(TokenRing* r, int slot, cudaStream_t s, uint32_t result[2]);
diff --git a/alfalfa_b200/csrc/kernels.cu b/alfalfa_b200/csrc/kernels.cu
--- a/alfalfa_b200/csrc/kernels.cu
+++ b/alfalfa_b200/csrc/kernels.cu
@@ -440,12 +440,27 @@
   __syncwarp();
 }
 
+__device__ __forceinline__ void acquire_job(const DevJob& J, int lane) {
+  const uint32_t* w = J.ready;
+  if (!w) return;
+  if (lane == 0) {
+#ifndef VP8GPU_SIMT_EMUL
+    uint32_t v;
+    asm volatile("ld.acquire.gpu.global.u32 %0, [%1];" : "=r"(v) : "l"(w) : "memory");
+#else
+    if (__atomic_load_n(w, __ATOMIC_ACQUIRE) != J.ready_epoch) abort();
+#endif
+  }
+  __syncwarp();
+}
+
 __global__ void __launch_bounds__(INTER_WARPS * 32, 10) k_inter(const DevJob* __restrict__ jobs, Geom g) {
   __shared__ InterSmem s_all[INTER_WARPS];
   const int warp = threadIdx.x >> 5, lane = threadIdx.x & 31;
   const DevJob& J = jobs[blockIdx.y];
   const int mbi = blockIdx.x * INTER_WARPS + warp;
   if (mbi >= g.mb_cols * g.mb_rows) return;
+  acquire_job(J, lane);
   const MbFields f = load_mb(J.mbs + mbi);
   if (f.ref == VP8GPU_REF_CURRENT) return;
   const int row = mbi / g.mb_cols, col = mbi - row * g.mb_cols;
@@ -728,6 +743,7 @@
   if (row >= g.mb_rows) return;
   const DevJob& J = jobs[job];
   if (J.n_intra == 0) return;
+  acquire_job(J, lane);
   const int cols = g.mb_cols;
   const vp8gpu_mb* row_mbs = J.mbs + (size_t)row * cols;
 
@@ -983,6 +999,7 @@
   if (row >= g.mb_rows) return;
   const DevJob& J = jobs[job];
   if (!J.lf_enabled) return;
+  acquire_job(J, lane);
   const int cols = g.mb_cols;
   const vp8gpu_mb* row_mbs = J.mbs + (size_t)row * cols;
 
@@ -1147,6 +1164,7 @@
   if (row >= g.mb_rows) return;
   const DevJob& J = jobs[job];
   if (!J.lf_enabled) return;
+  acquire_job(J, lane);
   const int cols = g.mb_cols;
   const vp8gpu_mb* row_mbs = J.mbs + (size_t)row * cols;
   Row* const S = s_rows + warp;
diff --git a/alfalfa_b200/csrc/tokens.cu b/alfalfa_b200/csrc/tokens.cu
--- a/alfalfa_b200/csrc/tokens.cu
+++ b/alfalfa_b200/csrc/tokens.cu
@@ -9,6 +9,23 @@
 namespace {
 
 constexpr int kMaxCols = 1024;
+
+__device__ __forceinline__ void publish_ready(const TokJob& J) {
+#ifndef VP8GPU_SIMT_EMUL
+  asm volatile("st.release.gpu.global.u32 [%0], %1;" ::"l"(J.ready), "r"(J.epoch) : "memory");
+  asm volatile("fence.acq_rel.sys;" ::: "memory");
+  asm volatile("st.relaxed.sys.global.u32 [%0], %1;" ::"l"(J.ready_host), "r"(J.epoch) : "memory");
+  if (J.stamp) {
+    unsigned long long t;
+    asm volatile("mov.u64 %0, %%globaltimer;" : "=l"(t));
+    *J.stamp = t;
+  }
+#else
+  __atomic_store_n(J.ready, J.epoch, __ATOMIC_RELEASE);
+  __atomic_store_n(J.ready_host, J.epoch, __ATOMIC_RELEASE);
+  if (J.stamp) *J.stamp = 1;
+#endif
+}
 template <int kTokWarps>
 __global__ void __launch_bounds__(32 * kTokWarps) k_tokens(const uint8_t* ring, size_t stride, int first, int count,
                                                           int nslots, Geom g) {
@@ -25,6 +42,7 @@
   __syncwarp();
   if (lane != 0) return;
   tok::decode_frame_tokens(J, g, probs, above_nz);
+  publish_ready(J);
 }
 
 __global__ void __launch_bounds__(32) k_tokens_lockstep(const uint8_t* ring, size_t stride, int first, int count,
@@ -54,8 +72,24 @@
   __syncwarp();
   if (!J) return;
   tok::decode_frame_tokens_lockstep<32>(*J, g, T, P + lane, above + lane);
+  publish_ready(*J);
 }
 
+__global__ void k_stamp(unsigned long long* dst) {
+#ifndef VP8GPU_SIMT_EMUL
+  unsigned long long t;
+  asm volatile("mov.u64 %0, %%globaltimer;" : "=l"(t));
+  *dst = t;
+#else
+  *dst = 0;
+#endif
+}
+
+}
+
+int launch_stamp(unsigned long long* dst, void* stream) {
+  VP8_LAUNCH(k_stamp, 1, 1, 0, static_cast<cudaStream_t>(stream))(dst);
+  return (int)cudaGetLastError();
 }
 
 int launch_tokens(const uint8_t* ring, size_t stride, int first, int count, int nslots, const Geom& g, void* stream) {
diff --git a/alfalfa_b200/csrc/wavefront_ll.cuh b/alfalfa_b200/csrc/wavefront_ll.cuh
--- a/alfalfa_b200/csrc/wavefront_ll.cuh
+++ b/alfalfa_b200/csrc/wavefront_ll.cuh
@@ -100,6 +100,7 @@
   if (row >= g.mb_rows) return;
   const DevJob& J = jobs[job];
   if (J.n_intra == 0) return;
+  acquire_job(J, lane);
   const int cols = g.mb_cols;
   const vp8gpu_mb* row_mbs = J.mbs + (size_t)row * cols;
 
@@ -337,6 +338,7 @@
   if (row >= g.mb_rows) return;
   const DevJob& J = jobs[job];
   if (!J.lf_enabled) return;
+  acquire_job(J, lane);
   const int cols = g.mb_cols;
   const vp8gpu_mb* row_mbs = J.mbs + (size_t)row * cols;
   const bool last_row = row == g.mb_rows - 1;
```

Measured after the change: 11540, median of 6. 5.4% higher.
